# StevenChang5/Canny_Edge

Hardware: AMD Instinct MI355X
Metric: Mpixels/s device-resident Canny (4K gray, frames in HBM, whole pipeline); % HBM roofline on Sobel+NMS in `roofline`; the end-to-end (host->host, PCIe-inclusive) rate is `end_to_end` (higher is better)
Workload: dtype f32+s16; 1 GPU; 128x 3840x2160 gray frames per GPU per step, sigma=1.4, thresholds 50/150, inputs resident in HBM; frames_per_gpu=128, height=2160, width=3840

## Files before the change

### canny_edge_amd/capi.py

```python
from __future__ import annotations

import ctypes as C
import os
import threading
from typing import Optional, Tuple

import numpy as np

_HERE = os.path.dirname(os.path.abspath(__file__))
LIB_PATH = os.environ.get("CANNY_HIP_LIB") or os.path.join(_HERE, "libcanny_hip.so")

OK = 0
STAGE_GAUSSIAN, STAGE_SOBEL_NMS, STAGE_HYST_CLASSIFY, STAGE_HYST_PROPAGATE, STAGE_HYST_FINALIZE, \
    STAGE_SOBEL, STAGE_NMS, STAGE_XY_GRADIENT, STAGE_TO_GRAY = range(9)
STAGE_NAMES = ("gaussian", "sobel_nms", "hyst_classify", "hyst_propagate", "hyst_finalize", "sobel", "nms",
               "xy_gradient", "to_gray")
STAGE_COMPACT = 9

LAYOUT_GRAY8, LAYOUT_BGR8, LAYOUT_RGB8, LAYOUT_BGRA8, LAYOUT_RGBA8 = range(5)
LAYOUT_CHANNELS = {LAYOUT_GRAY8: 1, LAYOUT_BGR8: 3, LAYOUT_RGB8: 3, LAYOUT_BGRA8: 4, LAYOUT_RGBA8: 4}


def layout_of(shape, order: str = "bgr", batch: bool = False) -> int:
    shape = tuple(int(d) for d in shape)
    if order not in ("bgr", "rgb"):
        raise ValueError(f"order must be 'bgr' or 'rgb', not {order!r}")
    nd = len(shape) - (1 if batch else 0)
    if nd == 2:
        return LAYOUT_GRAY8
    if nd == 3 and shape[-1] in (3, 4):
        if shape[-1] == 3:
            return LAYOUT_BGR8 if order == "bgr" else LAYOUT_RGB8
        return LAYOUT_BGRA8 if order == "bgr" else LAYOUT_RGBA8
    raise ValueError(f"expected {'(N, ' if batch else '('}H, W) or {'(N, ' if batch else '('}H, W, 3|4) frames, "
                     f"got shape {shape}")

AUTO_MEDIAN, AUTO_QUANTILE = 1, 2
PIXEL_LDS_TILE, PIXEL_PACKED_I16, PIXEL_F32, PIXEL_F32_FLOOR = 0, 1, 2, 3
WS_DATA, WS_INDEX, WS_CACHE = 0, 1, 2
_AUTO_RULES = {"median": AUTO_MEDIAN, "quantile": AUTO_QUANTILE, AUTO_MEDIAN: AUTO_MEDIAN, AUTO_QUANTILE: AUTO_QUANTILE}


def _rule(rule) -> int:
    if rule not in _AUTO_RULES:
        raise ValueError(f"rule must be 'median', 'quantile', AUTO_MEDIAN or AUTO_QUANTILE, not {rule!r}")
    return _AUTO_RULES[rule]


EXPORTS = (
    "canny_hip_version", "canny_hip_status_string", "canny_hip_device_count", "canny_hip_ctx_create",
    "canny_hip_ctx_destroy", "canny_hip_ctx_set_stream", "canny_hip_ctx_device", "canny_hip_ctx_set_option", "canny_hip_synchronize",
    "canny_hip_last_error", "canny_hip_last_hysteresis_iterations", "canny_hip_malloc", "canny_hip_free",
    "canny_hip_host_alloc", "canny_hip_host_free", "canny_hip_memcpy_h2d", "canny_hip_memcpy_d2h",
    "canny_hip_gaussian_kernel", "canny_hip_gaussian", "canny_hip_xy_gradient", "canny_hip_sobel", "canny_hip_nms",
    "canny_hip_hysteresis", "canny_hip_find_edge_pixels", "canny_hip_canny", "canny_hip_canny_batch",
    "canny_hip_canny_batch_u8", "canny_hip_dev_canny_u8", "canny_hip_canny_multi_gpu", "canny_hip_shard_range", "canny_hip_dev_gaussian", "canny_hip_dev_xy_gradient",
    "canny_hip_dev_sobel", "canny_hip_dev_nms", "canny_hip_dev_sobel_nms", "canny_hip_dev_hysteresis",
    "canny_hip_dev_canny", "canny_hip_dev_canny_stream", "canny_hip_dev_canny_stream_flush", "canny_hip_profile_enable", "canny_hip_profile_reset", "canny_hip_profile_get",
    "canny_hip_selftest_mag_angle", "canny_hip_selftest_sobel_pixel", "canny_hip_selftest_div", "canny_hip_selftest_div_fma",
    "canny_hip_selftest_div_fma_table", "canny_hip_canny_multi_gpu_u8", "canny_hip_multi_gpu_set_option",
    "canny_hip_multi_gpu_release", "canny_hip_device_local_cpus", "canny_hip_selftest_cpulist_count",
    "canny_hip_dev_gaussian_u8", "canny_hip_dev_sobel_nms_u8in", "canny_hip_host_register", "canny_hip_host_unregister",
    "canny_hip_canny_batch_bits", "canny_hip_canny_multi_gpu_bits", "canny_hip_dev_canny_bits",
    "canny_hip_probe_copy", "canny_hip_ctx_get_option", "canny_hip_selftest_expand_bits",
    "canny_hip_selftest_march_order", "canny_hip_to_gray", "canny_hip_dev_to_gray", "canny_hip_dev_gaussian_u8_color",
    "canny_hip_dev_canny_color", "canny_hip_canny_color", "canny_hip_canny_batch_color", "canny_hip_canny_batch_color_u8",
    "canny_hip_canny_batch_color_bits", "canny_hip_auto_thresholds_from_histogram", "canny_hip_dev_canny_thresholds",
    "canny_hip_dev_canny_auto", "canny_hip_canny_batch_thresholds", "canny_hip_canny_batch_auto",
    "canny_hip_dev_canny_points", "canny_hip_dev_points_from_bits", "canny_hip_canny_points",
    "canny_hip_points_from_bits",
    "canny_hip_hough_geometry", "canny_hip_hough_tables", "canny_hip_hough_line_of", "canny_hip_dev_hough_points",
    "canny_hip_dev_hough_bits", "canny_hip_dev_canny_hough", "canny_hip_canny_hough", "canny_hip_hough_profile_get",
    "canny_hip_dev_canny_components", "canny_hip_dev_components_bits", "canny_hip_canny_components",
    "canny_hip_components_from_bits", "canny_hip_components_profile_get",
    "canny_hip_dev_canny_contours", "canny_hip_dev_contours_bits", "canny_hip_canny_contours",
    "canny_hip_contours_from_bits", "canny_hip_contours_profile_get",
    "canny_hip_dev_canny_edt", "canny_hip_dev_edt_bits", "canny_hip_canny_edt", "canny_hip_edt_from_bits",
    "canny_hip_edt_profile_get",
    "canny_hip_hough_segments_from_bits", "canny_hip_dev_hough_segments_bits", "canny_hip_dev_canny_hough_segments",
    "canny_hip_canny_hough_segments", "canny_hip_hough_segments_profile_get",
    "canny_hip_selftest_histogram", "canny_hip_selftest_select", "canny_hip_selftest_workspace",
    "canny_hip_hough_circles_step_of", "canny_hip_hough_circles_from_bits", "canny_hip_dev_hough_circles_bits",
    "canny_hip_dev_canny_hough_circles", "canny_hip_canny_hough_circles", "canny_hip_dev_hough_circles_steps",
    "canny_hip_hough_circles_profile_get",
    "canny_hip_dev_polygons_chains", "canny_hip_dev_canny_polygons", "canny_hip_dev_polygons_bits",
    "canny_hip_canny_polygons", "canny_hip_polygons_from_chains", "canny_hip_polygons_profile_get",
)

_lib: Optional[C.CDLL] = None


class CannyHipError(RuntimeError):
    def __init__(self, status: int, what: str, detail: str = ""):
        self.status = status
        msg = f"{what}: {status_string(status)}"
        if detail:
            msg += f" ({detail})"
        super().__init__(msg)


def load() -> C.CDLL:
    global _lib
    if _lib is not None:
        return _lib
    if not os.path.exists(LIB_PATH):
        raise ImportError(f"{LIB_PATH} is missing: run `python -c 'import __graft_entry__ as g; g.build()'` "
                          "(or `make -C canny_edge_amd/csrc`); there is no CPU fallback")
    os.environ.setdefault("GPU_MAX_HW_QUEUES", "8")
    L = C.CDLL(LIB_PATH)
    i, f, p, sz = C.c_int, C.c_float, C.c_void_p, C.c_size_t
    pp, ip = C.POINTER(C.c_void_p), C.POINTER(C.c_int)
    ull = C.c_ulonglong
    sig = {
        "canny_hip_version": ([], i),
        "canny_hip_status_string": ([i], C.c_char_p),
        "canny_hip_device_count": ([ip], i),
        "canny_hip_ctx_create": ([pp, i], i),
        "canny_hip_ctx_destroy": ([p], None),
        "canny_hip_ctx_set_stream": ([p, p], i),
        "canny_hip_ctx_device": ([p], i),
        "canny_hip_ctx_set_option": ([p, C.c_char_p, i], i),
        "canny_hip_synchronize": ([p], i),
        "canny_hip_last_error": ([p], C.c_char_p),
        "canny_hip_last_hysteresis_iterations": ([p], i),
        "canny_hip_malloc": ([p, pp, sz], i),
        "canny_hip_free": ([p, p], i),
        "canny_hip_host_alloc": ([p, pp, sz], i),
        "canny_hip_host_free": ([p, p], i),
        "canny_hip_host_register": ([p, p, sz], i),
        "canny_hip_host_unregister": ([p, p], i),
        "canny_hip_memcpy_h2d": ([p, p, p, sz], i),
        "canny_hip_memcpy_d2h": ([p, p, p, sz], i),
        "canny_hip_gaussian_kernel": ([f, p, i, ip], i),
        "canny_hip_gaussian": ([p, p, f, i, i, p], i),
        "canny_hip_xy_gradient": ([p, p, i, i, p, p], i),
        "canny_hip_sobel": ([p, p, i, i, p, p], i),
        "canny_hip_nms": ([p, p, p, i, i, p], i),
        "canny_hip_hysteresis": ([p, p, i, i, i, i], i),
        "canny_hip_find_edge_pixels": ([p, p, p, i, i, i, i, i], i),
        "canny_hip_canny": ([p, p, f, i, i, i, i, p], i),
        "canny_hip_canny_batch": ([p, p, i, f, i, i, i, i, p], i),
        "canny_hip_canny_batch_u8": ([p, p, i, f, i, i, i, i, p], i),
        "canny_hip_dev_canny_u8": ([p, p, f, i, i, i, i, i, p], i),
        "canny_hip_dev_canny_bits": ([p, p, f, i, i, i, i, i, p], i),
        "canny_hip_canny_batch_bits": ([p, p, i, f, i, i, i, i, p], i),
        "canny_hip_canny_multi_gpu_bits": ([p, i, f, i, i, i, i, p, i], i),
        "canny_hip_canny_multi_gpu": ([p, i, f, i, i, i, i, p, i], i),
        "canny_hip_canny_multi_gpu_u8": ([p, i, f, i, i, i, i, p, i], i),
        "canny_hip_multi_gpu_set_option": ([C.c_char_p, i], i),
        "canny_hip_multi_gpu_release": ([], i),
        "canny_hip_device_local_cpus": ([i, C.c_char_p, i], i),
        "canny_hip_selftest_cpulist_count": ([C.c_char_p], i),
        "canny_hip_shard_range": ([i, i, i, ip, ip], i),
        "canny_hip_dev_gaussian": ([p, p, f, i, i, i, p], i),
        "canny_hip_dev_xy_gradient": ([p, p, i, i, i, p, p], i),
        "canny_hip_dev_sobel": ([p, p, i, i, i, p, p], i),
        "canny_hip_dev_nms": ([p, p, p, i, i, i, p], i),
        "canny_hip_dev_sobel_nms": ([p, p, i, i, i, p], i),
        "canny_hip_dev_hysteresis": ([p, p, i, i, i, i, i], i),
        "canny_hip_dev_gaussian_u8": ([p, p, f, i, i, i, p], i),
        "canny_hip_dev_sobel_nms_u8in": ([p, p, i, i, i, p], i),
        "canny_hip_dev_canny": ([p, p, f, i, i, i, i, i, p], i),
        "canny_hip_dev_canny_stream": ([p, p, f, i, i, i, i, i, p], i),
        "canny_hip_dev_canny_stream_flush": ([p], i),
        "canny_hip_profile_enable": ([p, i], i),
        "canny_hip_profile_reset": ([p], i),
        "canny_hip_profile_get": ([p, i, C.POINTER(C.c_double), C.POINTER(C.c_long)], i),
        "canny_hip_probe_copy": ([p, p, p, C.c_size_t, i, C.POINTER(C.c_double)], i),
        "canny_hip_ctx_get_option": ([p, C.c_char_p, ip], i),
        "canny_hip_selftest_expand_bits": ([p, i, i, i, p, i], i),
        "canny_hip_selftest_march_order": ([i, i, p], i),
        "canny_hip_selftest_mag_angle": ([p, i, p, p], i),
        "canny_hip_selftest_sobel_pixel": ([p, i, i, p, p], i),
        "canny_hip_selftest_div": ([p, f, C.POINTER(C.c_ulonglong), C.POINTER(C.c_float)], i),
        "canny_hip_selftest_div_fma": ([p, f, f, C.POINTER(C.c_ulonglong), C.POINTER(C.c_float)], i),
        "canny_hip_selftest_div_fma_table": ([i, C.POINTER(C.c_float), C.POINTER(C.c_float)], i),
        "canny_hip_to_gray": ([p, p, i, i, i, p], i),
        "canny_hip_dev_to_gray": ([p, p, i, i, i, i, p], i),
        "canny_hip_dev_gaussian_u8_color": ([p, p, i, f, i, i, i, p], i),
        "canny_hip_dev_canny_color": ([p, p, i, f, i, i, i, i, i, p], i),
        "canny_hip_canny_color": ([p, p, i, f, i, i, i, i, p], i),
        "canny_hip_canny_batch_color": ([p, p, i, i, f, i, i, i, i, p], i),
        "canny_hip_canny_batch_color_u8": ([p, p, i, i, f, i, i, i, i, p], i),
        "canny_hip_canny_batch_color_bits": ([p, p, i, i, f, i, i, i, i, p], i),
        "canny_hip_auto_thresholds_from_histogram": ([p, i, f, f, ip, ip], i),
        "canny_hip_dev_canny_thresholds": ([p, p, f, p, i, i, i, p], i),
        "canny_hip_dev_canny_auto": ([p, p, f, i, f, f, i, i, i, p, p], i),
        "canny_hip_canny_batch_thresholds": ([p, p, i, f, p, i, i, p], i),
        "canny_hip_canny_batch_auto": ([p, p, i, f, i, f, f, i, i, p, p], i),
        "canny_hip_dev_canny_points": ([p, p, f, i, i, i, i, i, p, p, C.c_ulonglong, p], i),
        "canny_hip_dev_points_from_bits": ([p, p, i, i, i, p, C.c_ulonglong, p], i),
        "canny_hip_canny_points": ([p, p, i, f, i, i, i, i, p, C.c_ulonglong, p], i),
        "canny_hip_points_from_bits": ([p, i, i, p, C.c_ulonglong, C.POINTER(C.c_ulonglong)], i),
        "canny_hip_hough_geometry": ([i, i, f, f, f, f, ip, ip], i),
        "canny_hip_hough_tables": ([f, f, f, i, p, p], i),
        "canny_hip_hough_line_of": ([C.c_uint, i, f, f, f, C.POINTER(f), C.POINTER(f)], i),
        "canny_hip_dev_hough_points": ([p, p, p, i, i, i, f, f, i, i, f, f, p, p, p, p, p], i),
        "canny_hip_dev_hough_bits": ([p, p, i, i, i, f, f, i, i, f, f, p, p, p, p, p], i),
        "canny_hip_dev_canny_hough": ([p, p, f, i, i, i, i, i, p, f, f, i, i, f, f, p, p, p, p, p], i),
        "canny_hip_canny_hough": ([p, p, i, f, i, i, i, i, f, f, i, i, f, f, p, p, p, p], i),
        "canny_hip_hough_profile_get": ([p, i, C.POINTER(C.c_double), C.POINTER(C.c_long)], i),
        "canny_hip_dev_canny_components": ([p, p, f, i, i, i, i, i, p, i, p, p, p, C.c_ulonglong, p], i),
        "canny_hip_dev_components_bits": ([p, p, i, i, i, i, p, p, p, C.c_ulonglong, p], i),
        "canny_hip_canny_components": ([p, p, i, f, i, i, i, i, i, p, p, p, C.c_ulonglong, p], i),
        "canny_hip_components_from_bits": ([p, i, i, i, p, p, C.c_ulonglong, C.POINTER(C.c_ulonglong)], i),
        "canny_hip_components_profile_get": ([p, i, C.POINTER(C.c_double), C.POINTER(C.c_long)], i),
        "canny_hip_dev_canny_contours": ([p, p, f, i, i, i, i, i, p, i, p, C.c_ulonglong, p, p, p, C.c_ulonglong, p], i),
        "canny_hip_dev_contours_bits": ([p, p, i, i, i, i, p, C.c_ulonglong, p, p, p, C.c_ulonglong, p], i),
        "canny_hip_canny_contours": ([p, p, i, f, i, i, i, i, i, p, C.c_ulonglong, p, p, p, C.c_ulonglong, p], i),
        "canny_hip_contours_from_bits": ([p, i, i, i, p, C.c_ulonglong, C.POINTER(C.c_ulonglong), p, p, C.c_ulonglong,
                                          C.POINTER(C.c_ulonglong)], i),
        "canny_hip_contours_profile_get": ([p, i, C.POINTER(C.c_double), C.POINTER(C.c_long)], i),
        "canny_hip_dev_canny_edt": ([p, p, f, i, i, i, i, i, p, p, p, p], i),
        "canny_hip_dev_edt_bits": ([p, p, i, i, i, p, p, p], i),
        "canny_hip_canny_edt": ([p, p, i, f, i, i, i, i, p, p, p], i),
        "canny_hip_edt_from_bits": ([p, i, i, p, p, p], i),
        "canny_hip_edt_profile_get": ([p, i, C.POINTER(C.c_double), C.POINTER(C.c_long)], i),
        "canny_hip_hough_segments_from_bits": ([p, i, i, f, f, f, f, p, i, i, i, i, p, i, ip], i),
        "canny_hip_dev_hough_segments_bits": ([p, p, i, i, i, f, f, f, f, p, p, i, i, i, i, p, i, p], i),
        "canny_hip_dev_canny_hough_segments": ([p, p, f, i, i, i, i, i, p, f, f, i, i, f, f, p, p, p, p, p, i, i, i, p, i,
                                                p], i),
        "canny_hip_canny_hough_segments": ([p, p, i, f, i, i, i, i, f, f, i, i, f, f, i, i, i, p, p, p, p, p, i, p], i),
        "canny_hip_hough_segments_profile_get": ([p, i, C.POINTER(C.c_double), C.POINTER(C.c_long)], i),
        "canny_hip_selftest_histogram": ([p, p, i, i, i, i, i, p], i),
        "canny_hip_selftest_select": ([p, p, i, i, f, f, p], i),
        "canny_hip_selftest_workspace": ([p, i, C.POINTER(C.c_char_p), pp, C.POINTER(sz), ip], i),
        "canny_hip_hough_circles_step_of": ([i, i, ip, ip], i),
        "canny_hip_hough_circles_from_bits": ([p, p, p, i, i, i, i, i, i, i, i, i, p, ip, ip, p], i),
        "canny_hip_dev_hough_circles_bits": ([p, p, p, p, i, i, i, i, i, i, i, i, i, i, p, p, p, p], i),
        "canny_hip_dev_canny_hough_circles": ([p, p, f, i, i, i, i, i, p, i, i, i, i, i, i, i, p, p, p, p], i),
        "canny_hip_canny_hough_circles": ([p, p, i, f, i, i, i, i, i, i, i, i, i, i, i, p, p, p], i),
        "canny_hip_dev_hough_circles_steps": ([p, p, p, C.c_size_t, p, p], i),
        "canny_hip_hough_circles_profile_get": ([p, i, C.POINTER(C.c_double), C.POINTER(C.c_long)], i),
        "canny_hip_dev_polygons_chains": ([p, p, i, ull, p, p, ull, i, i, C.c_uint, C.c_uint, p, p, ull, p], i),
        "canny_hip_dev_canny_polygons": ([p, p, f, i, i, i, i, i, p, i, p, ull, p, p, p, ull, p, C.c_uint, C.c_uint, p, p,
                                          ull, p], i),
        "canny_hip_dev_polygons_bits": ([p, p, i, i, i, i, p, ull, p, p, p, ull, p, C.c_uint, C.c_uint, p, p, ull, p], i),
        "canny_hip_canny_polygons": ([p, p, i, f, i, i, i, i, i, p, ull, p, p, p, ull, p, C.c_uint, C.c_uint, p, p, ull,
                                      p], i),
        "canny_hip_polygons_from_chains": ([p, p, ull, ull, i, i, C.c_uint, C.c_uint, p, p, ull, p], i),
        "canny_hip_polygons_profile_get": ([p, i, C.POINTER(C.c_double), C.POINTER(C.c_long)], i),
    }
    for name, (args, res) in sig.items():
        fn = getattr(L, name)
        fn.argtypes = args
        fn.restype = res
    _lib = L
    return L


def status_string(status: int) -> str:
    return load().canny_hip_status_string(status).decode()


def device_count() -> int:
    n = C.c_int(0)
# ... 871 lines not shown
                c[name] = r[:, j]
            out.append(c)
        return out, peaks

    def dev_hough_circles_bits(self, d_bits: int, d_gx: int, d_gy: int, n: int, h: int, w: int, min_radius: int,
                               max_radius: int, cell_shift: int, threshold: int, support_threshold: int, min_dist: int,
                               centres_max: int, d_circles: int, d_counts: int, d_centre_counts: int = 0, d_accum: int = 0):
        v = C.c_void_p
        self._check(self._L.canny_hip_dev_hough_circles_bits(self._h, v(d_bits or None), v(d_gx or None), v(d_gy or None), n,
                                                             h, w, min_radius, max_radius, cell_shift, threshold,
                                                             support_threshold, min_dist, centres_max,
                                                             v(d_circles or None), v(d_counts or None),
                                                             v(d_centre_counts or None), v(d_accum or None)),
                    "dev_hough_circles_bits")

    def dev_canny_hough_circles(self, d_img: int, sigma: float, min_val: int, max_val: int, h: int, w: int, n: int,
                                min_radius: int, max_radius: int, cell_shift: int, threshold: int, support_threshold: int,
                                min_dist: int, centres_max: int, d_circles: int, d_counts: int, d_centre_counts: int = 0,
                                d_accum: int = 0, d_edges: int = 0):
        v = C.c_void_p
        self._check(self._L.canny_hip_dev_canny_hough_circles(self._h, v(d_img or None), sigma, min_val, max_val, h, w, n,
                                                              v(d_edges or None), min_radius, max_radius, cell_shift,
                                                              threshold, support_threshold, min_dist, centres_max,
                                                              v(d_circles or None), v(d_counts or None),
                                                              v(d_centre_counts or None), v(d_accum or None)),
                    "dev_canny_hough_circles")

    def dev_hough_circles_steps(self, d_gx: int, d_gy: int, n: int, d_sx: int, d_sy: int):
        v = C.c_void_p
        self._check(self._L.canny_hip_dev_hough_circles_steps(self._h, v(d_gx or None), v(d_gy or None), n,
                                                              v(d_sx or None), v(d_sy or None)), "dev_hough_circles_steps")

    def hough_circles_profile_get(self, part: int) -> Tuple[float, int]:
        ms, n = C.c_double(0), C.c_long(0)
        self._check(self._L.canny_hip_hough_circles_profile_get(self._h, part, C.byref(ms), C.byref(n)),
                    "hough_circles_profile_get")
        return ms.value, n.value

    def to_gray(self, frame, order: str = "bgr") -> np.ndarray:
        a, lay = _frame(frame, order)
        out = np.empty(a.shape[:2], np.uint8)
        self._check(self._L.canny_hip_to_gray(self._h, _hp(a), lay, a.shape[0], a.shape[1], _hp(out)), "to_gray")
        return out

    def canny_color(self, frame, sigma: float, min_val: int, max_val: int, order: str = "bgr") -> np.ndarray:
        a, lay = _frame(frame, order)
        out = np.empty(a.shape[:2], np.int16)
        self._check(self._L.canny_hip_canny_color(self._h, _hp(a), lay, sigma, min_val, max_val, a.shape[0],
                                                  a.shape[1], _hp(out)), "canny_color")
        return out

    def canny_batch_color(self, imgs, sigma: float, min_val: int, max_val: int, order: str = "bgr",
                          out: Optional[np.ndarray] = None, fmt: str = "s16") -> np.ndarray:
        a, lay = _frame(imgs, order, batch=True)
        if fmt not in ("s16", "u8", "bits"):
            raise ValueError(f"fmt must be 's16', 'u8' or 'bits', not {fmt!r}")
        n, h, w = a.shape[:3]
        dtype = np.int16 if fmt == "s16" else np.uint8
        shape = bits_shape((n, h, w)) if fmt == "bits" else (n, h, w)
        if out is None:
            out = np.empty(shape, dtype)
        elif out.shape != shape or out.dtype != dtype or not out.flags["C_CONTIGUOUS"]:
            raise ValueError(f"out must be a C-contiguous {np.dtype(dtype).name} array of shape {shape}")
        fn = {"s16": self._L.canny_hip_canny_batch_color, "u8": self._L.canny_hip_canny_batch_color_u8,
              "bits": self._L.canny_hip_canny_batch_color_bits}[fmt]
        self._check(fn(self._h, _hp(a), lay, n, sigma, min_val, max_val, h, w, _hp(out)), "canny_batch_color")
        return out

    def selftest_mag_angle(self, lim: int = 1020):
        side = 2 * lim + 1
        mags = np.empty((side, side), np.int16)
        bins = np.empty((side, side), np.uint8)
        self._check(self._L.canny_hip_selftest_mag_angle(self._h, lim, _hp(mags), _hp(bins)), "selftest")
        return mags, bins

    def selftest_sobel_pixel(self, form: int, lim: int = 1020):
        side = 2 * lim + 1
        mags = np.empty((side, side), np.int16)
        bins = np.empty((side, side), np.uint8)
        self._check(self._L.canny_hip_selftest_sobel_pixel(self._h, form, lim, _hp(mags), _hp(bins)),
                    "selftest_sobel_pixel")
        return mags, bins

    def selftest_div(self, divisor: float) -> Tuple[int, float]:
        bad, worst = C.c_ulonglong(0), C.c_float(0.0)
        self._check(self._L.canny_hip_selftest_div(self._h, divisor, C.byref(bad), C.byref(worst)), "selftest_div")
        return bad.value, worst.value

    def selftest_div_fma(self, divisor: float, c: float) -> Tuple[int, float]:
        bad, worst = C.c_ulonglong(0), C.c_float(0.0)
        self._check(self._L.canny_hip_selftest_div_fma(self._h, divisor, c, C.byref(bad), C.byref(worst)),
                    "selftest_div_fma")
        return bad.value, worst.value

    def selftest_histogram(self, d_plane: int, plane_is_u8: bool, kind, h: int, w: int, n: int, d_hist: int):
        self._check(self._L.canny_hip_selftest_histogram(self._h, C.c_void_p(d_plane), int(plane_is_u8), _rule(kind), h,
                                                         w, n, C.c_void_p(d_hist)), "selftest_histogram")

    def selftest_select(self, d_hist: int, n: int, rule, low: float, high: float, d_pairs: int):
        self._check(self._L.canny_hip_selftest_select(self._h, C.c_void_p(d_hist), n, _rule(rule), low, high,
                                                      C.c_void_p(d_pairs)), "selftest_select")

    def selftest_workspaces(self):
        out, index = [], 0
        while True:
            name, ptr, size, kind = C.c_char_p(), C.c_void_p(), C.c_size_t(), C.c_int()
            st = self._L.canny_hip_selftest_workspace(self._h, index, C.byref(name), C.byref(ptr), C.byref(size),
                                                      C.byref(kind))
            if st == 1 and index > 0:
                return out
            self._check(st, "selftest_workspace")
            out.append((name.value.decode(), ptr.value or 0, size.value, kind.value))
            index += 1

    def dev_gaussian(self, d_img: int, sigma: float, h: int, w: int, n: int, d_out: int):
        self._check(self._L.canny_hip_dev_gaussian(self._h, C.c_void_p(d_img), sigma, h, w, n, C.c_void_p(d_out)),
                    "dev_gaussian")

    def dev_xy_gradient(self, d_img: int, h: int, w: int, n: int, d_gx: int, d_gy: int):
        self._check(self._L.canny_hip_dev_xy_gradient(self._h, C.c_void_p(d_img), h, w, n, C.c_void_p(d_gx),
                                                      C.c_void_p(d_gy)), "dev_xy_gradient")

    def dev_sobel(self, d_img: int, h: int, w: int, n: int, d_mag: int, d_ang: int):
        self._check(self._L.canny_hip_dev_sobel(self._h, C.c_void_p(d_img), h, w, n, C.c_void_p(d_mag),
                                                C.c_void_p(d_ang)), "dev_sobel")

    def dev_nms(self, d_mag: int, d_ang: int, h: int, w: int, n: int, d_out: int):
        self._check(self._L.canny_hip_dev_nms(self._h, C.c_void_p(d_mag), C.c_void_p(d_ang), h, w, n,
                                              C.c_void_p(d_out)), "dev_nms")

    def dev_sobel_nms(self, d_smoothed: int, h: int, w: int, n: int, d_out: int):
        self._check(self._L.canny_hip_dev_sobel_nms(self._h, C.c_void_p(d_smoothed), h, w, n, C.c_void_p(d_out)),
                    "dev_sobel_nms")

    def probe_copy(self, d_src: int, d_dst: int, nbytes: int, launches: int = 10) -> float:
        ms = C.c_double(0)
        self._check(self._L.canny_hip_probe_copy(self._h, C.c_void_p(d_src), C.c_void_p(d_dst), nbytes, launches,
                                                 C.byref(ms)), "probe_copy")
        return ms.value

    def dev_gaussian_u8(self, d_img: int, sigma: float, h: int, w: int, n: int, d_out: int):
        self._check(self._L.canny_hip_dev_gaussian_u8(self._h, C.c_void_p(d_img), sigma, h, w, n, C.c_void_p(d_out)),
                    "dev_gaussian_u8")

    def dev_sobel_nms_u8in(self, d_smoothed: int, h: int, w: int, n: int, d_out: int):
        self._check(self._L.canny_hip_dev_sobel_nms_u8in(self._h, C.c_void_p(d_smoothed), h, w, n, C.c_void_p(d_out)),
                    "dev_sobel_nms_u8in")

    def dev_hysteresis(self, d_cand: int, h: int, w: int, n: int, min_val: int, max_val: int):
        self._check(self._L.canny_hip_dev_hysteresis(self._h, C.c_void_p(d_cand), h, w, n, min_val, max_val),
                    "dev_hysteresis")

    def dev_canny(self, d_img: int, sigma: float, min_val: int, max_val: int, h: int, w: int, n: int, d_edges: int):
        self._check(self._L.canny_hip_dev_canny(self._h, C.c_void_p(d_img), sigma, min_val, max_val, h, w, n,
                                                C.c_void_p(d_edges)), "dev_canny")

    def dev_canny_stream(self, d_img: int, sigma: float, min_val: int, max_val: int, h: int, w: int, n: int,
                         d_edges: int):
        self._check(self._L.canny_hip_dev_canny_stream(self._h, C.c_void_p(d_img), sigma, min_val, max_val, h, w, n,
                                                       C.c_void_p(d_edges)), "dev_canny_stream")

    def dev_canny_stream_flush(self):
        self._check(self._L.canny_hip_dev_canny_stream_flush(self._h), "dev_canny_stream_flush")

    def dev_canny_bits(self, d_img: int, sigma: float, min_val: int, max_val: int, h: int, w: int, n: int, d_bits: int):
        self._check(self._L.canny_hip_dev_canny_bits(self._h, C.c_void_p(d_img), sigma, min_val, max_val, h, w, n,
# ... 122 lines not shown
```

### canny_edge_amd/csrc/canny_capi.hip

```cpp
#include "canny_hip.h"
#include "canny_kernels.h"

#include <hip/hip_runtime.h>
#include <sched.h>

#include <algorithm>
#include <atomic>
#include <chrono>
#include <condition_variable>
#include <deque>
#include <memory>
#include <cmath>
#include <cstdint>
#include <cstdio>
#include <cctype>
#include <climits>
#include <cstdlib>
#include <cstring>
#include <mutex>
#include <new>
#include <string>
#include <thread>
#include <vector>
#if defined(__SSE2__)
// ... 209 lines not shown
            }
            run(j);
        }
    }
    void run(const Job &j)
    {
        if (j.copy_bytes) std::memcpy(j.dst, j.bits, j.copy_bytes);
        for (int r = 0; r < (j.copy_bytes ? 0 : j.rows); r++) {
            const uint8_t *src = j.bits + (size_t)r * j.row_bytes;
            const int full = j.width / 8, tail = j.width % 8;
            if (j.to_u8) {
                uint8_t *d = (uint8_t *)j.dst + (size_t)r * j.width;
                for (int b = 0; b < full; b++) std::memcpy(d + 8 * b, lut8_[src[b]], 8);
                if (tail) std::memcpy(d + 8 * full, lut8_[src[full]], tail);
            } else {
                short *d = (short *)j.dst + (size_t)r * j.width;
#if defined(__SSE2__)
                if ((((uintptr_t)d) & 15) == 0) {
                    for (int b = 0; b < full; b++)
                        _mm_stream_si128((__m128i *)(d + 8 * b), _mm_load_si128((const __m128i *)lut16_[src[b]]));
                } else
#endif
                {
                    for (int b = 0; b < full; b++) std::memcpy(d + 8 * b, lut16_[src[b]], 16);
                }
                if (tail) std::memcpy(d + 8 * full, lut16_[src[full]], 2 * tail);
            }
        }
#if defined(__SSE2__)
        _mm_sfence();
#endif
        if (j.left->fetch_sub(1, std::memory_order_acq_rel) == 1) {
            std::lock_guard<std::mutex> lk(mu_);
            cv_done_.notify_all();
        }
    }
    alignas(16) short lut16_[256][8];
    alignas(8) uint8_t lut8_[256][8];
    std::vector<std::thread> threads_;
    std::mutex mu_;
    std::condition_variable cv_job_, cv_done_;
    std::deque<Job> q_;
    bool stop_ = false;
};

struct EventPair {
    hipEvent_t a, b;
};

struct PropLane {
    hipStream_t stream = nullptr;
    uint64_t *S = nullptr;
    const uint64_t *C = nullptr;
    unsigned *sched = nullptr, *flags = nullptr;
    unsigned *host = nullptr, *host_dev = nullptr;
    hipEvent_t event = nullptr;
    HystGeom g{};
    short *edges = nullptr;
    int edge_value = 0;
    int iter = 0;
    unsigned seq = 0;
    bool converged = false;
};

}

struct canny_hip_ctx {
    int device = 0;
    hipStream_t own_stream = nullptr;
    hipStream_t stream = nullptr;
    std::string last_error;
    int last_hyst_iters = 0;
    int gaussian_path = 0;
    int sobel_nms_path = 0;
    int tune_sobel_seg = 0;
    int fuse_classify = 1;
    int smoothed_u8 = 1;
    int last_canny_u8 = 0;
    int gray_rule = 0;
    int fuse_gray = 1;
    int last_fused_gray = 0;
    int hyst_tail = 1;
    int hyst_tail_after = 2;
    bool hyst_iters_async = false;
    int batch_workers = 0;
    int batch_chunk_mb = 0;
    int batch_chunk_frames = 0;
    int batch_pipe_mode = 0;
    int batch_compact = 0;
    int batch_expand_threads = 0;
    std::unique_ptr<ExpandPool> expand_pool;
    struct BatchPipe;
    std::vector<BatchPipe *> batch_pool;

    DevBuf tmp_f32;
    DevBuf smoothed;
    DevBuf edges16;
    DevBuf gray;
    DevBuf hist;
    DevBuf thr;
    DevBuf points;
    DevBuf hough_accum, hough_ws, hough_tab;
    std::vector<float> hough_tab_host;
    float hough_tab_key[3] = {0, 0, 0};
    int hough_tab_n = 0;
    int hough_path = 0;
    int hough_lds_kb = 0;
    DevBuf cc_parent, cc_ws;
    DevBuf ct_ws;
    DevBuf pg_ws, pg_points;
    DevBuf edt_cols, edt_stack;
    DevBuf seg_ws, seg_lines, seg_work;
    DevBuf circ_accum, circ_ws;
    DevBuf plane_s, plane_c, stamps, flags;
    DevBuf io[4];
    std::string ws_name;
    unsigned *host_flags = nullptr;
    unsigned *host_flags_dev = nullptr;
    unsigned publish_seq = 0;
    hipEvent_t flag_event = nullptr;
    int overlap_hysteresis = 0;
    int stream_overlap = 0;
    hipStream_t aux_stream = nullptr;
    hipEvent_t fork_event = nullptr, aux_event = nullptr;
    PropLane pend;
    bool has_pend = false;

    bool prof = false;
    unsigned prof_mask = ~0u;
    unsigned prof_every = 1;
    static constexpr int kProfHough = CANNY_HIP_STAGE_END, kProfComponents = CANNY_HIP_STAGE_END + 3;
    static constexpr int kProfEdt = kProfComponents + CANNY_HIP_CC_PARTS;
    static constexpr int kProfSegments = kProfEdt + CANNY_HIP_EDT_PARTS;
    static constexpr int kProfContours = kProfSegments + CANNY_HIP_SEGMENT_PARTS;
    static constexpr int kProfCircles = kProfContours + CANNY_HIP_CONTOUR_PARTS;
    static constexpr int kProfPolygons = kProfCircles + CANNY_HIP_CIRCLE_PARTS;
    static constexpr int kProfSlots = kProfPolygons + CANNY_HIP_POLYGON_PARTS;
    static constexpr int kProfLastBit = 30;
    static_assert(kProfPolygons == kProfLastBit, "profile_stage_mask has one bit per slot up to the polygon parts");
    unsigned prof_seen[kProfSlots] = {0};
    std::vector<EventPair> pending[kProfSlots];
    std::vector<EventPair> pool;
    double total_ms[kProfSlots] = {0};
    long launches[kProfSlots] = {0};
};

struct canny_hip_ctx::BatchPipe {
    static constexpr int kSlots = 3;
    canny_hip_ctx *sub = nullptr;
    bool owns_sub = false;
    hipStream_t s_h2d = nullptr, s_d2h = nullptr;
    struct Slot {
        DevBuf d_in, d_out, d_out8;
        PinBuf pin_in, pin_out;
        DevBuf d_thr;
        PinBuf pin_thr;
        hipEvent_t ev_h2d = nullptr, ev_comp = nullptr, ev_d2h = nullptr;
        bool d2h_issued = false;
        void *retire_dst = nullptr;
        size_t retire_bytes = 0;
        int retire_frames = 0;
        std::atomic<int> expand_left{0};
    } slot[kSlots];
};

namespace {

int fail(canny_hip_ctx *ctx, hipError_t e, const char *where)
{
    if (ctx) {
        ctx->last_error = std::string(where) + ": " + hipGetErrorString(e);
    }
    (void)hipGetLastError();
    return (e == hipErrorNoDevice || e == hipErrorInvalidDevice) ? CANNY_HIP_ERR_NO_DEVICE : CANNY_HIP_ERR_RUNTIME;
}

#define HIP_TRY(ctx, expr)                                  \
    do {                                                    \
        hipError_t e_ = (expr);                             \
        if (e_ != hipSuccess) return fail((ctx), e_, #expr); \
    } while (0)

int bind(canny_hip_ctx *ctx)
{
    if (!ctx) return CANNY_HIP_ERR_INVALID;
    HIP_TRY(ctx, hipSetDevice(ctx->device));
    return CANNY_HIP_OK;
}

struct StageTimer {
    canny_hip_ctx *ctx;
    int stage;
    EventPair ev{};
    bool on = false;
    hipStream_t stream;
    bool attach;
    StageTimer(canny_hip_ctx *c, int s, hipStream_t on_stream = nullptr, bool attached = false)
// ... 73 lines not shown
    default: return CANNY_HIP_ERR_INVALID;
    }
    const bool bgr = layout == CANNY_HIP_BGR8 || layout == CANNY_HIP_BGRA8;
    ci.rule.k0 = bgr ? w[0] : w[2];
    ci.rule.k1 = w[1];
    ci.rule.k2 = bgr ? w[2] : w[0];
    ci.rule.shift = w[3];
    ci.rule.rnd = 1u << (w[3] - 1);
    return CANNY_HIP_OK;
}

bool gaussian_u8_possible(const canny_hip_ctx *ctx, const GaussTaps &taps, int h, int w)
{
    float min_tap = 1.0f;
    for (int k = 0; k <= 2 * taps.center; k++)
        if (taps.tap[k] > 0.0f && taps.tap[k] < min_tap) min_tap = taps.tap[k];
    return ctx->gaussian_path != 1 && gaussian_march_supported(taps.center, h, w) && min_tap >= 0x1p-48f &&
           gaussian_march_u8_supported(taps) && sobel_nms_u8_input_supported();
}

int dev_gaussian(canny_hip_ctx *ctx, const unsigned char *d_img, float sigma, int h, int w, int n, void *d_out_any,
                 int u8_mode = 0)
{
    short *d_out = (short *)d_out_any;
    GaussTaps taps;
    int rc = make_taps(sigma, taps);
    if (rc) return rc;
    StageTimer tm(ctx, CANNY_HIP_STAGE_GAUSSIAN);
    if (u8_mode) {
        if (!gaussian_u8_possible(ctx, taps, h, w)) return CANNY_HIP_ERR_UNSUPPORTED;
        HIP_TRY(ctx, launch_gaussian_march_u8(d_img, (uint8_t *)d_out_any, h, w, n, taps, ctx->stream));
        return CANNY_HIP_OK;
    }
    float min_tap = 1.0f;
    for (int k = 0; k <= 2 * taps.center; k++)
        if (taps.tap[k] > 0.0f && taps.tap[k] < min_tap) min_tap = taps.tap[k];
    const bool can_march = gaussian_march_supported(taps.center, h, w) && min_tap >= 0x1p-48f;
    if (ctx->gaussian_path == 2 && !can_march) return CANNY_HIP_ERR_UNSUPPORTED;
    if (can_march && ctx->gaussian_path != 1) {
        HIP_TRY(ctx, launch_gaussian_march(d_img, d_out, h, w, n, taps, ctx->stream));
    } else {
        HIP_TRY(ctx, ctx->tmp_f32.ensure(npx(h, w, n) * sizeof(float)));
        HIP_TRY(ctx, launch_gaussian_generic(d_img, (float *)ctx->tmp_f32.p, d_out, h, w, n, taps, ctx->stream));
    }
    return CANNY_HIP_OK;
}

int dev_to_gray(canny_hip_ctx *ctx, const unsigned char *d_src, const ColorIn &ci, int h, int w, int n,
                unsigned char *d_gray)
{
    const size_t px = npx(h, w, n);
    if (ci.ch == 1) {
        if (d_src != d_gray) HIP_TRY(ctx, hipMemcpyAsync(d_gray, d_src, px, hipMemcpyDeviceToDevice, ctx->stream));
        return CANNY_HIP_OK;
    }
    StageTimer tm(ctx, CANNY_HIP_STAGE_TO_GRAY);
    HIP_TRY(ctx, launch_to_gray(d_src, ci.ch, ci.rule, d_gray, px, ctx->stream));
    return CANNY_HIP_OK;
}

bool gaussian_color_fusable(const canny_hip_ctx *ctx, const GaussTaps &taps, const ColorIn &ci, int h, int w)
{
    return ci.ch > 1 && gaussian_u8_possible(ctx, taps, h, w) && gaussian_march_color_supported(taps, w, ci.ch);
}

int dev_gaussian_u8_color(canny_hip_ctx *ctx, const unsigned char *d_src, const ColorIn &ci, float sigma, int h, int w,
                          int n, unsigned char *d_out)
{
    GaussTaps taps;
    int rc = make_taps(sigma, taps);
    if (rc) return rc;
    if (!gaussian_color_fusable(ctx, taps, ci, h, w)) return CANNY_HIP_ERR_UNSUPPORTED;
    StageTimer tm(ctx, CANNY_HIP_STAGE_GAUSSIAN);
    HIP_TRY(ctx, launch_gaussian_march_u8_color(d_src, ci.ch, ci.rule, d_out, h, w, n, taps, ctx->stream));
    return CANNY_HIP_OK;
}

int ensure_hyst(canny_hip_ctx *ctx, const HystGeom &g)
{
    HIP_TRY(ctx, ctx->plane_s.ensure(g.words() * sizeof(uint64_t)));
    HIP_TRY(ctx, ctx->plane_c.ensure(g.words() * sizeof(uint64_t)));
    HIP_TRY(ctx, ctx->stamps.ensure((hyst_sched_words(g) + 4) * sizeof(unsigned)));
    HIP_TRY(ctx, ctx->flags.ensure(4 * sizeof(unsigned)));
    if (!ctx->host_flags) {
        HIP_TRY(ctx, hipHostMalloc((void **)&ctx->host_flags, 8 * sizeof(unsigned), hipHostMallocMapped));
        std::memset(ctx->host_flags, 0, 8 * sizeof(unsigned));
        HIP_TRY(ctx, hipHostGetDevicePointer((void **)&ctx->host_flags_dev, ctx->host_flags, 0));
    }
    if (!ctx->flag_event) HIP_TRY(ctx, hipEventCreateWithFlags(&ctx->flag_event, hipEventDisableTiming));
    return CANNY_HIP_OK;
}

int ensure_aux_stream(canny_hip_ctx *ctx)
{
    if (!ctx->aux_stream) {
        int least = 0, greatest = 0;
        HIP_TRY(ctx, hipDeviceGetStreamPriorityRange(&least, &greatest));
        HIP_TRY(ctx, hipStreamCreateWithPriority(&ctx->aux_stream, hipStreamNonBlocking, greatest));
    }
    if (!ctx->fork_event) HIP_TRY(ctx, hipEventCreateWithFlags(&ctx->fork_event, hipEventDisableTiming));
    if (!ctx->aux_event) HIP_TRY(ctx, hipEventCreateWithFlags(&ctx->aux_event, hipEventDisableTiming));
    return CANNY_HIP_OK;
}

int prepare_hyst(canny_hip_ctx *ctx, const HystGeom &g, bool zero_pad)
{
    HIP_TRY(ctx, launch_hyst_prepare((uint64_t *)ctx->plane_s.p, (uint64_t *)ctx->plane_c.p, g, zero_pad,
                                     (unsigned *)ctx->stamps.p, (unsigned *)ctx->flags.p, ctx->stream));
    return CANNY_HIP_OK;
}

constexpr int kTailMaxTiles = 4096;
constexpr int kSweepChunk = 8;
constexpr int kMaxSweeps = 1 << 22;

int lane_launch_chunk(canny_hip_ctx *ctx, PropLane &L)
{
    {
        StageTimer tm(ctx, CANNY_HIP_STAGE_HYST_PROPAGATE, L.stream);
        for (int k = 0; k < kSweepChunk; k++)
            HIP_TRY(ctx, launch_hyst_propagate(L.S, L.C, L.sched, L.flags, L.iter + k, L.g, L.stream, L.edges,
                                               L.edge_value));
    }
    L.iter += kSweepChunk;
    L.seq = ++ctx->publish_seq;
    HIP_TRY(ctx, launch_hyst_publish(L.flags, L.host_dev, L.seq, L.stream));
    HIP_TRY(ctx, hipEventRecord(L.event, L.stream));
    return CANNY_HIP_OK;
}

int lane_wait(canny_hip_ctx *ctx, PropLane &L)
{
    volatile unsigned *hf = L.host;
    const auto t0 = std::chrono::steady_clock::now();
    unsigned spins = 0;
    while (__atomic_load_n(&hf[2], __ATOMIC_ACQUIRE) != L.seq) {
        __builtin_ia32_pause();
        if ((++spins & 0xfffu) == 0 && std::chrono::steady_clock::now() - t0 > std::chrono::seconds(2)) {
            HIP_TRY(ctx, hipEventSynchronize(L.event));
            if (__atomic_load_n(&hf[2], __ATOMIC_ACQUIRE) != L.seq) return CANNY_HIP_ERR_RUNTIME;
        }
    }
    if (hf[1]) return CANNY_HIP_ERR_DOMAIN;
    L.converged = hf[0] != (unsigned)L.iter;
    if (!L.converged && L.iter >= kMaxSweeps) return CANNY_HIP_ERR_NO_CONVERGE;
    if (L.converged) ctx->last_hyst_iters = std::max(ctx->last_hyst_iters, (int)hf[0] + 1);
    return CANNY_HIP_OK;
}

PropLane main_lane(canny_hip_ctx *ctx, const HystGeom &g, short *edges, int edge_value)
{
    PropLane L;
    L.stream = ctx->stream;
    L.S = (uint64_t *)ctx->plane_s.p;
    L.C = (const uint64_t *)ctx->plane_c.p;
    L.sched = (unsigned *)ctx->stamps.p;
    L.flags = (unsigned *)ctx->flags.p;
    L.host = ctx->host_flags;
    L.host_dev = ctx->host_flags_dev;
    L.event = ctx->flag_event;
    L.g = g;
    L.edges = edges;
    L.edge_value = edge_value;
    return L;
}

// ... 42 lines not shown

int dev_hysteresis(canny_hip_ctx *ctx, short *d_cand, int h, int w, int n, int lo, int hi, const int *pairs = nullptr)
{
    if (pairs) lo = hi = 255;
    if (hysteresis_order_dependent(lo, hi)) return CANNY_HIP_ERR_DOMAIN;
    HystGeom g = make_hyst_geom(h, w, n);
    int rc = finish_pending(ctx);
    if (rc || (rc = ensure_hyst(ctx, g))) return rc;
    if ((rc = prepare_hyst(ctx, g, false))) return rc;
    {
        StageTimer tm(ctx, CANNY_HIP_STAGE_HYST_CLASSIFY);
        HIP_TRY(ctx, launch_hyst_classify(d_cand, (uint64_t *)ctx->plane_s.p, (uint64_t *)ctx->plane_c.p, g, lo, hi,
                                          (unsigned *)ctx->flags.p + 1, ctx->stream, pairs));
    }
    return propagate_and_finalize(ctx, g, d_cand, hi);
}

int dev_sobel_nms(canny_hip_ctx *ctx, const short *d_smoothed, int h, int w, int n, short *d_out)
{
    if (ctx->sobel_nms_path != 1 && sobel_nms_march_supported(h, w)) {
        StageTimer tm(ctx, CANNY_HIP_STAGE_SOBEL_NMS, nullptr, true);
        HIP_TRY(ctx, launch_sobel_nms_march(d_smoothed, d_out, h, w, n, ctx->stream, ctx->tune_sobel_seg,
                                            tm.launch_events()));
    } else {
        StageTimer tm(ctx, CANNY_HIP_STAGE_SOBEL_NMS);
        HIP_TRY(ctx, launch_sobel_nms(d_smoothed, d_out, h, w, n, true, ctx->stream));
    }
    return CANNY_HIP_OK;
}

int dev_canny(canny_hip_ctx *ctx, const unsigned char *d_img, float sigma, int lo, int hi, int h, int w, int n,
              short *d_edges, const ColorIn *color = nullptr, const ThrSpec *thr = nullptr)
{
    if (h < 2 || w < 2) return CANNY_HIP_ERR_UNSUPPORTED;
    if (thr) lo = hi = 255;
    if (hysteresis_order_dependent(lo, hi)) return CANNY_HIP_ERR_DOMAIN;
    int rc = finish_pending(ctx);
    if (rc) return rc;
    HIP_TRY(ctx, ctx->smoothed.ensure(npx(h, w, n) * sizeof(short)));
    short *sm = (short *)ctx->smoothed.p;
    const bool fused = ctx->fuse_classify && ctx->sobel_nms_path != 1 && sobel_nms_classify_supported(h, w, lo);
    int sm_u8 = 0;
    if (fused && ctx->smoothed_u8) {
        GaussTaps taps;
        if ((rc = make_taps(sigma, taps))) return rc;
        if (gaussian_u8_possible(ctx, taps, h, w)) sm_u8 = ctx->smoothed_u8;
    }
    ctx->last_canny_u8 = sm_u8;
    if (color && color->ch > 1) {
        GaussTaps taps;
        if ((rc = make_taps(sigma, taps))) return rc;
        const bool fuse = sm_u8 && color->fuse && gaussian_color_fusable(ctx, taps, *color, h, w);
        ctx->last_fused_gray = fuse;
        if (fuse) {
            StageTimer tm(ctx, CANNY_HIP_STAGE_GAUSSIAN);
            HIP_TRY(ctx, launch_gaussian_march_u8_color(d_img, color->ch, color->rule, (uint8_t *)sm, h, w, n, taps,
                                                        ctx->stream));
        } else {
            HIP_TRY(ctx, ctx->gray.ensure(npx(h, w, n)));
            if ((rc = dev_to_gray(ctx, d_img, *color, h, w, n, (unsigned char *)ctx->gray.p))) return rc;
            if ((rc = dev_gaussian(ctx, (const unsigned char *)ctx->gray.p, sigma, h, w, n, sm, sm_u8))) return rc;
        }
    } else {
        if (color) ctx->last_fused_gray = 0;
        if ((rc = dev_gaussian(ctx, d_img, sigma, h, w, n, sm, sm_u8))) return rc;
    }
    const int *pairs = thr ? thr->pairs : nullptr;
    if (thr && thr->rule) {
        int *out = thr->out;
        if (!out) {
            HIP_TRY(ctx, ctx->thr.ensure((size_t)n * 2 * sizeof(int)));
            out = (int *)ctx->thr.p;
        }
        HIP_TRY(ctx, ctx->hist.ensure((size_t)n * kHistBins * sizeof(uint32_t)));
        uint32_t *hist = (uint32_t *)ctx->hist.p;
        StageTimer tm(ctx, CANNY_HIP_STAGE_HYST_CLASSIFY);
        HIP_TRY(ctx, hipMemsetAsync(hist, 0, (size_t)n * kHistBins * sizeof(uint32_t), ctx->stream));
        HIP_TRY(ctx, thr->rule == kAutoMedian ? launch_hist_intensity(sm, sm_u8 != 0, hist, h, w, n, ctx->stream)
                                              : launch_hist_gradient(sm, sm_u8 != 0, hist, h, w, n, ctx->stream));
        HIP_TRY(ctx, launch_thr_select(hist, n, thr->rule, thr->low, thr->high, out, ctx->stream));
        pairs = out;
    }
    auto fused_sobel = [&](const short *smp, short *edges, uint64_t *S, uint64_t *C, const HystGeom &gg, int ev,
                           const LaunchEvents &le, const int *pp) -> hipError_t {
        return sm_u8 ? launch_sobel_nms_classify_march_u8in((const uint8_t *)smp, edges, S, C, gg, lo, hi, ev,
                                                            ctx->stream, ctx->tune_sobel_seg, le, pp)
                     : launch_sobel_nms_classify_march(smp, edges, S, C, gg, lo, hi, ev, ctx->stream,
                                                       ctx->tune_sobel_seg, le, pp);
    };
    if (fused) {
        HystGeom g = make_hyst_geom(h, w, n);
        if ((rc = ensure_hyst(ctx, g))) return rc;
        uint64_t *S = (uint64_t *)ctx->plane_s.p, *C = (uint64_t *)ctx->plane_c.p;
        const int edge_value = 255 >= hi ? 255 : 0;
        if (ctx->overlap_hysteresis && n >= 16) {
            if ((rc = ensure_aux_stream(ctx))) return rc;
            const int nA = n / 2, nB = n - nA;
            const HystGeom gA = make_hyst_geom(h, w, nA), gB = make_hyst_geom(h, w, nB);
            const size_t px_a = npx(h, w, nA);
            HIP_TRY(ctx, launch_hyst_prepare(S, C, g, true, (unsigned *)ctx->stamps.p,
                                             (unsigned *)ctx->flags.p, ctx->stream, 2));
            PropLane A = main_lane(ctx, gA, d_edges, edge_value), B = main_lane(ctx, gB, d_edges + px_a, edge_value);
            A.stream = ctx->aux_stream;
            A.event = ctx->aux_event;
            B.S += gA.words();
            B.C += gA.words();
            B.sched += hyst_sched_words(gA);
            B.flags += 2;
            B.host += 4;
            B.host_dev += 4;
            {
                StageTimer tm(ctx, CANNY_HIP_STAGE_SOBEL_NMS, nullptr, true);
                HIP_TRY(ctx, fused_sobel(sm, d_edges, A.S, (uint64_t *)A.C, gA, edge_value, tm.launch_events(), pairs));
            }
            HIP_TRY(ctx, hipEventRecord(ctx->fork_event, ctx->stream));
            HIP_TRY(ctx, hipStreamWaitEvent(ctx->aux_stream, ctx->fork_event, 0));
            ctx->last_hyst_iters = 0;
            if ((rc = lane_launch_chunk(ctx, A))) return rc;
            {
                StageTimer tm(ctx, CANNY_HIP_STAGE_SOBEL_NMS, nullptr, true);
                const short *smB = sm_u8 ? (const short *)((const uint8_t *)sm + px_a) : sm + px_a;
                HIP_TRY(ctx, fused_sobel(smB, d_edges + px_a, B.S, (uint64_t *)B.C, gB, edge_value, tm.launch_events(),
                                         pairs ? pairs + 2 * (size_t)nA : nullptr));
            }
            if ((rc = lane_launch_chunk(ctx, B))) return rc;
            for (PropLane *L : {&A, &B}) {
                if ((rc = lane_wait(ctx, *L))) return rc;
                while (!L->converged) {
                    if ((rc = lane_launch_chunk(ctx, *L)) || (rc = lane_wait(ctx, *L))) return rc;
                }
            }
            HIP_TRY(ctx, hipStreamWaitEvent(ctx->stream, A.event, 0));
            return CANNY_HIP_OK;
        }
        if ((rc = prepare_hyst(ctx, g, true))) return rc;
        {
            StageTimer tm(ctx, CANNY_HIP_STAGE_SOBEL_NMS, nullptr, true);
            HIP_TRY(ctx, fused_sobel(sm, d_edges, S, C, g, edge_value, tm.launch_events(), pairs));
        }
        if (ctx->hyst_tail && g.tiles_x * g.tiles_y <= kTailMaxTiles) {
            StageTimer tm(ctx, CANNY_HIP_STAGE_HYST_PROPAGATE);
            unsigned *sched = (unsigned *)ctx->stamps.p, *flags = (unsigned *)ctx->flags.p;
            const int wide = ctx->hyst_tail_after;
            for (int k = 0; k < wide; k++)
                HIP_TRY(ctx, launch_hyst_propagate(S, C, sched, flags, k, g, ctx->stream, d_edges, edge_value,
                                                   true));
            HIP_TRY(ctx, launch_hyst_tail(S, C, sched, flags, wide, g, ctx->stream, d_edges, edge_value));
            ctx->hyst_iters_async = true;
            return CANNY_HIP_OK;
        }
        ctx->hyst_iters_async = false;
        return run_propagation(ctx, g, false, []() -> int { return CANNY_HIP_OK; }, d_edges, edge_value);
    }
    if ((rc = dev_sobel_nms(ctx, sm, h, w, n, d_edges))) return rc;
    return dev_hysteresis(ctx, d_edges, h, w, n, lo, hi, pairs);
}

int finish_pending(canny_hip_ctx *ctx)
{
    if (!ctx->has_pend) return CANNY_HIP_OK;
    ctx->has_pend = false;
    PropLane &L = ctx->pend;
    int rc;
    if ((rc = lane_wait(ctx, L))) return rc;
    while (!L.converged)
        if ((rc = lane_launch_chunk(ctx, L)) || (rc = lane_wait(ctx, L))) return rc;
    if (L.stream != ctx->stream) HIP_TRY(ctx, hipStreamWaitEvent(ctx->stream, L.event, 0));
    return CANNY_HIP_OK;
}

int dev_canny_stream(canny_hip_ctx *ctx, const unsigned char *d_img, float sigma, int lo, int hi, int h, int w, int n,
                     short *d_edges)
{
    if (h < 2 || w < 2) return CANNY_HIP_ERR_UNSUPPORTED;
    if (hysteresis_order_dependent(lo, hi)) return CANNY_HIP_ERR_DOMAIN;
    if (!(ctx->fuse_classify && ctx->sobel_nms_path != 1 && sobel_nms_classify_supported(h, w, lo)) ||
        (ctx->hyst_tail && make_hyst_geom(h, w, n).tiles_x * make_hyst_geom(h, w, n).tiles_y <= kTailMaxTiles)) {
        int rc = finish_pending(ctx);
        return rc ? rc : dev_canny(ctx, d_img, sigma, lo, hi, h, w, n, d_edges);
    }
    HIP_TRY(ctx, ctx->smoothed.ensure(npx(h, w, n) * sizeof(short)));
    short *sm = (short *)ctx->smoothed.p;
    int sm_u8 = 0;
    if (ctx->smoothed_u8) {
        GaussTaps taps;
        int rt = make_taps(sigma, taps);
        if (rt) return rt;
        if (gaussian_u8_possible(ctx, taps, h, w)) sm_u8 = ctx->smoothed_u8;
    }
    ctx->last_canny_u8 = sm_u8;
    int rc = dev_gaussian(ctx, d_img, sigma, h, w, n, sm, sm_u8);
    if (rc) return rc;
    if ((rc = finish_pending(ctx))) return rc;
    HystGeom g = make_hyst_geom(h, w, n);
    if ((rc = ensure_hyst(ctx, g)) || (ctx->stream_overlap && (rc = ensure_aux_stream(ctx)))) return rc;
    const int edge_value = 255 >= hi ? 255 : 0;
    if ((rc = prepare_hyst(ctx, g, true))) return rc;
    {
        StageTimer tm(ctx, CANNY_HIP_STAGE_SOBEL_NMS, nullptr, true);
        if (sm_u8)
            HIP_TRY(ctx, launch_sobel_nms_classify_march_u8in((const uint8_t *)sm, d_edges, (uint64_t *)ctx->plane_s.p,
                                                              (uint64_t *)ctx->plane_c.p, g, lo, hi, edge_value,
                                                              ctx->stream, ctx->tune_sobel_seg, tm.launch_events()));
        else
            HIP_TRY(ctx, launch_sobel_nms_classify_march(sm, d_edges, (uint64_t *)ctx->plane_s.p,
                                                         (uint64_t *)ctx->plane_c.p, g, lo, hi, edge_value, ctx->stream,
                                                         ctx->tune_sobel_seg, tm.launch_events()));
    }
    ctx->pend = main_lane(ctx, g, d_edges, edge_value);
    if (ctx->stream_overlap) {
        HIP_TRY(ctx, hipEventRecord(ctx->fork_event, ctx->stream));
        HIP_TRY(ctx, hipStreamWaitEvent(ctx->aux_stream, ctx->fork_event, 0));
        ctx->pend.stream = ctx->aux_stream;
        ctx->pend.event = ctx->aux_event;
    }
    ctx->last_hyst_iters = 0;
    ctx->hyst_iters_async = false;
    if ((rc = lane_launch_chunk(ctx, ctx->pend))) return rc;
    ctx->has_pend = true;
    return CANNY_HIP_OK;
}

int h2d(canny_hip_ctx *ctx, DevBuf &b, const void *src, size_t bytes)
{
    HIP_TRY(ctx, b.ensure(bytes));
    HIP_TRY(ctx, hipMemcpyAsync(b.p, src, bytes, hipMemcpyHostToDevice, ctx->stream));
    return CANNY_HIP_OK;
}
int d2h_sync(canny_hip_ctx *ctx, void *dst, const void *src, size_t bytes)
// ... 596 lines not shown
        sl.d_out8.release();
        sl.pin_in.release();
        sl.pin_out.release();
        sl.d_thr.release();
        sl.pin_thr.release();
        for (hipEvent_t e : {sl.ev_h2d, sl.ev_comp, sl.ev_d2h})
            if (e) (void)hipEventDestroy(e);
    }
    if (w->s_h2d) (void)hipStreamDestroy(w->s_h2d);
    if (w->s_d2h) (void)hipStreamDestroy(w->s_d2h);
    if (w->owns_sub) canny_hip_ctx_destroy(w->sub);
    delete w;
}

int create_batch_pipe(canny_hip_ctx *ctx, bool first, canny_hip_ctx::BatchPipe **out)
{
    auto *w = new (std::nothrow) canny_hip_ctx::BatchPipe();
    if (!w) return CANNY_HIP_ERR_RUNTIME;
    int st = CANNY_HIP_OK;
    if (first) {
        w->sub = ctx;
    } else {
        st = canny_hip_ctx_create(&w->sub, ctx->device);
        w->owns_sub = st == CANNY_HIP_OK;
    }
    hipError_t e = hipSuccess;
    if (!st) {
        for (auto &sl : w->slot)
            for (hipEvent_t *ev : {&sl.ev_h2d, &sl.ev_comp, &sl.ev_d2h})
                if (e == hipSuccess) e = hipEventCreateWithFlags(ev, hipEventDisableTiming);
        if (e != hipSuccess) st = fail(ctx, e, "batch pipeline events");
    }
    if (st) {
        destroy_batch_pipe(w);
        return st;
    }
    *out = w;
    return CANNY_HIP_OK;
}

int ensure_copy_streams(canny_hip_ctx *ctx, canny_hip_ctx::BatchPipe &w)
{
    if (!w.s_h2d) HIP_TRY(ctx, hipStreamCreateWithFlags(&w.s_h2d, hipStreamNonBlocking));
    if (!w.s_d2h) HIP_TRY(ctx, hipStreamCreateWithFlags(&w.s_d2h, hipStreamNonBlocking));
    return CANNY_HIP_OK;
}

struct WsEntry {
    std::string name;
    const DevBuf *buf;
    int kind;
};

void collect_workspaces(const canny_hip_ctx *c, const std::string &prefix, std::vector<WsEntry> &v)
{
    const int D = CANNY_HIP_WS_DATA, I = CANNY_HIP_WS_INDEX;
    auto add = [&](const char *name, const DevBuf &b, int kind) { v.push_back({prefix + name, &b, kind}); };
    add("tmp_f32", c->tmp_f32, D);
    add("smoothed", c->smoothed, D);
    add("edges16", c->edges16, D);
    add("gray", c->gray, D);
    add("hist", c->hist, D);
    add("thr", c->thr, D);
    add("points", c->points, I);
    add("hough_accum", c->hough_accum, D);
    add("hough_ws", c->hough_ws, I);
    add("hough_tab", c->hough_tab, CANNY_HIP_WS_CACHE);
    add("cc_parent", c->cc_parent, I);
    add("cc_ws", c->cc_ws, I);
    add("ct_ws", c->ct_ws, I);
    add("pg_ws", c->pg_ws, I);
    add("pg_points", c->pg_points, I);
    add("edt_cols", c->edt_cols, I);
    add("edt_stack", c->edt_stack, I);
    add("seg_ws", c->seg_ws, I);
    add("seg_lines", c->seg_lines, I);
    add("seg_work", c->seg_work, D);
    add("circ_accum", c->circ_accum, D);
    add("circ_ws", c->circ_ws, I);
    add("plane_s", c->plane_s, D);
    add("plane_c", c->plane_c, D);
    add("stamps", c->stamps, I);
    add("flags", c->flags, D);
    for (int k = 0; k < 4; k++) add(("io" + std::to_string(k)).c_str(), c->io[k], I);
    for (size_t p = 0; p < c->batch_pool.size(); p++) {
        const canny_hip_ctx::BatchPipe *w = c->batch_pool[p];
        if (!w) continue;
        const std::string pipe = prefix + "pipe" + std::to_string(p) + ".";
        for (int s = 0; s < canny_hip_ctx::BatchPipe::kSlots; s++) {
            const std::string slot = pipe + "slot" + std::to_string(s) + ".";
            v.push_back({slot + "d_in", &w->slot[s].d_in, D});
            v.push_back({slot + "d_out", &w->slot[s].d_out, D});
            v.push_back({slot + "d_out8", &w->slot[s].d_out8, D});
            v.push_back({slot + "d_thr", &w->slot[s].d_thr, D});
        }
        if (w->owns_sub && w->sub) collect_workspaces(w->sub, pipe, v);
    }
}

}

extern "C" {

int canny_hip_version(void) { return CANNY_HIP_VERSION; }

const char *canny_hip_status_string(int status)
{
    switch (status) {
    case CANNY_HIP_OK: return "ok";
    case CANNY_HIP_ERR_INVALID: return "invalid argument";
    case CANNY_HIP_ERR_UNSUPPORTED: return "unsupported size or window";
    case CANNY_HIP_ERR_NO_DEVICE: return "no usable HIP device (there is no CPU fallback)";
    case CANNY_HIP_ERR_RUNTIME: return "HIP runtime error";
    case CANNY_HIP_ERR_DOMAIN: return "input outside the documented numeric domain";
    case CANNY_HIP_ERR_NO_CONVERGE: return "hysteresis propagation did not converge";
    default: return "unknown status";
    }
}

int canny_hip_device_count(int *count)
{
    if (!count) return CANNY_HIP_ERR_INVALID;
    int n = 0;
    hipError_t e = hipGetDeviceCount(&n);
    if (e != hipSuccess) {
        (void)hipGetLastError();
        *count = 0;
        return CANNY_HIP_ERR_NO_DEVICE;
    }
    *count = n;
    return CANNY_HIP_OK;
}

int canny_hip_ctx_create(canny_hip_ctx **out, int device)
{
    if (!out) return CANNY_HIP_ERR_INVALID;
    *out = nullptr;
    int n = 0;
    if (hipGetDeviceCount(&n) != hipSuccess || n < 1) {
        (void)hipGetLastError();
        return CANNY_HIP_ERR_NO_DEVICE;
    }
    if (device < 0 || device >= n) return CANNY_HIP_ERR_INVALID;
    canny_hip_ctx *ctx = new (std::nothrow) canny_hip_ctx();
    if (!ctx) return CANNY_HIP_ERR_RUNTIME;
    ctx->device = device;
    if (hipSetDevice(device) != hipSuccess ||
        hipStreamCreateWithFlags(&ctx->own_stream, hipStreamNonBlocking) != hipSuccess) {
        (void)hipGetLastError();
        delete ctx;
        return CANNY_HIP_ERR_NO_DEVICE;
    }
    ctx->stream = ctx->own_stream;
    *out = ctx;
    return CANNY_HIP_OK;
}

void canny_hip_ctx_destroy(canny_hip_ctx *ctx)
{
    if (!ctx) return;
    (void)hipSetDevice(ctx->device);
    (void)finish_pending(ctx);
    ctx->expand_pool.reset();
    for (auto *w : ctx->batch_pool) destroy_batch_pipe(w);
    ctx->batch_pool.clear();
    (void)hipSetDevice(ctx->device);
    if (ctx->aux_stream) (void)hipStreamSynchronize(ctx->aux_stream);
    (void)hipStreamSynchronize(ctx->stream);
    ctx->tmp_f32.release();
    ctx->smoothed.release();
    ctx->plane_s.release();
    ctx->plane_c.release();
    ctx->edges16.release();
    ctx->hist.release();
    ctx->thr.release();
    ctx->points.release();
    ctx->hough_accum.release();
    ctx->hough_ws.release();
    ctx->hough_tab.release();
    ctx->seg_ws.release();
    ctx->seg_lines.release();
    ctx->seg_work.release();
    ctx->circ_accum.release();
    ctx->circ_ws.release();
    ctx->cc_parent.release();
    ctx->cc_ws.release();
    ctx->ct_ws.release();
    ctx->pg_ws.release();
    ctx->pg_points.release();
    ctx->edt_cols.release();
    ctx->edt_stack.release();
    ctx->stamps.release();
    ctx->flags.release();
    for (auto &b : ctx->io) b.release();
    if (ctx->host_flags) (void)hipHostFree(ctx->host_flags);
    if (ctx->flag_event) (void)hipEventDestroy(ctx->flag_event);
    if (ctx->fork_event) (void)hipEventDestroy(ctx->fork_event);
    if (ctx->aux_event) (void)hipEventDestroy(ctx->aux_event);
    if (ctx->aux_stream) (void)hipStreamDestroy(ctx->aux_stream);
    for (auto &v : ctx->pending)
        for (auto &e : v) {
            (void)hipEventDestroy(e.a);
            (void)hipEventDestroy(e.b);
        }
    for (auto &e : ctx->pool) {
        (void)hipEventDestroy(e.a);
        (void)hipEventDestroy(e.b);
    }
    if (ctx->own_stream) (void)hipStreamDestroy(ctx->own_stream);
    delete ctx;
}

int canny_hip_ctx_set_stream(canny_hip_ctx *ctx, void *hip_stream)
{
    int rc = bind(ctx);
    if (rc || (rc = finish_pending(ctx))) return rc;
    ctx->stream = hip_stream ? (hipStream_t)hip_stream : ctx->own_stream;
    return CANNY_HIP_OK;
}

int canny_hip_ctx_device(const canny_hip_ctx *ctx) { return ctx ? ctx->device : -1; }

int canny_hip_ctx_get_option(const canny_hip_ctx *ctx, const char *name, int *value)
{
    if (!ctx || !name || !value) return CANNY_HIP_ERR_INVALID;
    if (!std::strcmp(name, "smoothed_u8")) *value = ctx->smoothed_u8;
    else if (!std::strcmp(name, "last_canny_smoothed_u8")) *value = ctx->last_canny_u8;
    else if (!std::strcmp(name, "gray_rule")) *value = ctx->gray_rule;
    else if (!std::strcmp(name, "fuse_gray")) *value = ctx->fuse_gray;
    else if (!std::strcmp(name, "last_canny_fused_gray")) *value = ctx->last_fused_gray;
    else if (!std::strcmp(name, "fuse_classify")) *value = ctx->fuse_classify;
    else if (!std::strcmp(name, "hysteresis_tail")) *value = ctx->hyst_tail;
    else if (!std::strcmp(name, "gaussian_path")) *value = ctx->gaussian_path;
    else if (!std::strcmp(name, "sobel_nms_path")) *value = ctx->sobel_nms_path;
    else if (!std::strcmp(name, "tune_batch_compact")) *value = ctx->batch_compact;
    else if (!std::strcmp(name, "hough_path")) *value = ctx->hough_path;
    else if (!std::strcmp(name, "tune_hough_lds_kb")) *value = ctx->hough_lds_kb;
    else if (!std::strcmp(name, "batch_expand_threads")) *value = ctx->expand_pool ? ctx->expand_pool->size() : 0;
    else return CANNY_HIP_ERR_INVALID;
    return CANNY_HIP_OK;
}

int canny_hip_ctx_set_option(canny_hip_ctx *ctx, const char *name, int value)
{
    if (!ctx || !name || value < 0) return CANNY_HIP_ERR_INVALID;
    if (!std::strcmp(name, "gaussian_path") && value <= 2) ctx->gaussian_path = value;
    else if (!std::strcmp(name, "sobel_nms_path") && value <= 2) ctx->sobel_nms_path = value;
    else if (!std::strcmp(name, "tune_sobel_seg") && value <= 4096) ctx->tune_sobel_seg = value;
    else if (!std::strcmp(name, "fuse_classify") && value <= 1) ctx->fuse_classify = value;
    else if (!std::strcmp(name, "smoothed_u8") && value <= 1) ctx->smoothed_u8 = value;
    else if (!std::strcmp(name, "gray_rule") && value <= 1) ctx->gray_rule = value;
    else if (!std::strcmp(name, "fuse_gray") && value <= 1) ctx->fuse_gray = value;
    else if (!std::strcmp(name, "hysteresis_tail") && value <= 1) ctx->hyst_tail = value;
    else if (!std::strcmp(name, "tune_hyst_tail_after") && value >= 1 && value <= 4) ctx->hyst_tail_after = value;
    else if (!std::strcmp(name, "overlap_hysteresis") && value <= 1) ctx->overlap_hysteresis = value;
    else if (!std::strcmp(name, "tune_batch_workers") && value <= 16) ctx->batch_workers = value;
    else if (!std::strcmp(name, "tune_batch_chunk_mb") && value <= 1024) ctx->batch_chunk_mb = value;
    else if (!std::strcmp(name, "tune_batch_chunk_frames") && value <= 65535) ctx->batch_chunk_frames = value;
    else if (!std::strcmp(name, "tune_batch_pipe_mode") && value <= 2) ctx->batch_pipe_mode = value;
    else if (!std::strcmp(name, "tune_batch_compact") && value <= 1) ctx->batch_compact = value;
    else if (!std::strcmp(name, "hough_path") && value <= 2) ctx->hough_path = value;
    else if (!std::strcmp(name, "tune_hough_lds_kb") && value <= kHoughLdsMax / 1024) ctx->hough_lds_kb = value;
    else if (!std::strcmp(name, "tune_batch_expand_threads") && value <= 64) {
        if (value != ctx->batch_expand_threads) ctx->expand_pool.reset();
        ctx->batch_expand_threads = value;
    }
    else if (!std::strcmp(name, "stream_overlap") && value <= 1) {
        int rc = bind(ctx);
        if (rc || (rc = finish_pending(ctx))) return rc;
        ctx->stream_overlap = value;
    } else if (!std::strcmp(name, "profile_sample_interval") && value >= 1) {
        ctx->prof_every = (unsigned)value;
        for (auto &n : ctx->prof_seen) n = 0;
    } else if (!std::strcmp(name, "profile_stage_mask")) ctx->prof_mask = value ? (unsigned)value : ~0u;
    else if (!std::strcmp(name, "tune_sobel_px") && value <= 1) sobel_nms_set_px_variant(value);
    else if (!std::strcmp(name, "tune_sobel_variant") && value <= 2) sobel_nms_set_arith_variant(value);
    else if (!std::strcmp(name, "tune_plane_stores") && value <= 1) sobel_nms_set_plane_store_variant(value);
    else if (!std::strcmp(name, "gaussian_fma_div") && value <= 1) gaussian_set_fma_div(value != 0);
    else if (!std::strcmp(name, "tune_finalize_mode") && value <= 1) hyst_set_finalize_mode(value);
    else if (!std::strcmp(name, "tune_gaussian_variant") && value <= 4) gaussian_set_march_variant(value);
    else if (!std::strcmp(name, "tune_gaussian_seg") && value <= 8192) gaussian_set_seg_target(value);
    else return CANNY_HIP_ERR_INVALID;
    return CANNY_HIP_OK;
}

int canny_hip_synchronize(canny_hip_ctx *ctx)
{
    int rc = bind(ctx);
    if (rc || (rc = finish_pending(ctx))) return rc;
    HIP_TRY(ctx, hipStreamSynchronize(ctx->stream));
    return CANNY_HIP_OK;
}

const char *canny_hip_last_error(const canny_hip_ctx *ctx) { return ctx ? ctx->last_error.c_str() : ""; }
int canny_hip_last_hysteresis_iterations(canny_hip_ctx *ctx)
{
    if (!ctx) return 0;
    if (ctx->hyst_iters_async && ctx->flags.p) {
        unsigned last = 0;
        if (hipSetDevice(ctx->device) == hipSuccess &&
            hipMemcpyAsync(&last, ctx->flags.p, sizeof last, hipMemcpyDeviceToHost, ctx->stream) == hipSuccess &&
            hipStreamSynchronize(ctx->stream) == hipSuccess)
            ctx->last_hyst_iters = (int)last + 1;
        else
            (void)hipGetLastError();
        ctx->hyst_iters_async = false;
    }
    return ctx->last_hyst_iters;
}

int canny_hip_malloc(canny_hip_ctx *ctx, void **dev_ptr, size_t bytes)
{
    int rc = bind(ctx);
    if (rc) return rc;
    if (!dev_ptr) return CANNY_HIP_ERR_INVALID;
    HIP_TRY(ctx, hipMalloc(dev_ptr, bytes ? bytes : 1));
    return CANNY_HIP_OK;
}
int canny_hip_free(canny_hip_ctx *ctx, void *dev_ptr)
{
    int rc = bind(ctx);
    if (rc) return rc;
    HIP_TRY(ctx, hipFree(dev_ptr));
    return CANNY_HIP_OK;
}
int canny_hip_host_alloc(canny_hip_ctx *ctx, void **host_ptr, size_t bytes)
{
    int rc = bind(ctx);
    if (rc) return rc;
    if (!host_ptr) return CANNY_HIP_ERR_INVALID;
    hipError_t e = numa_host_malloc(ctx->device, host_ptr, bytes);
    HIP_TRY(ctx, e);
    return CANNY_HIP_OK;
}
int canny_hip_host_free(canny_hip_ctx *ctx, void *host_ptr)
{
    int rc = bind(ctx);
// ... 2139 lines not shown
    double total = 0.0;
    hipError_t e = hipSuccess;
    for (int k = 0; k < launches && e == hipSuccess; k++) {
        e = launch_probe_copy(d_src, d_dst, nbytes, ctx->stream, LaunchEvents{a, b});
        if (e == hipSuccess) e = hipEventSynchronize(b);
        float ms = 0.0f;
        if (e == hipSuccess) e = hipEventElapsedTime(&ms, a, b);
        total += ms;
    }
    (void)hipEventDestroy(a);
    (void)hipEventDestroy(b);
    HIP_TRY(ctx, e);
    *avg_ms = total / launches;
    return CANNY_HIP_OK;
}

int canny_hip_selftest_march_order(int n_segs, int n_strips, int *out_pairs)
{
    if (!out_pairs || n_segs < 1 || n_strips < 1 || (long long)n_segs * n_strips > (1 << 24)) return CANNY_HIP_ERR_INVALID;
    for (int k = 0; k < n_segs * n_strips; k++) {
        const MarchCell c = march_cell_of(k, n_segs, n_strips);
        out_pairs[2 * k] = c.seg;
        out_pairs[2 * k + 1] = c.strip;
    }
    return CANNY_HIP_OK;
}

int canny_hip_selftest_expand_bits(const unsigned char *bits, int height, int width, int to_u8, void *out, int n_threads)
{
    if (!bits || !out || height < 1 || width < 1 || n_threads < 1 || n_threads > 64) return CANNY_HIP_ERR_INVALID;
    ExpandPool pool(n_threads);
    constexpr int kBlockRows = 128;
    const int row_bytes = (width + 7) / 8, blocks = (height + kBlockRows - 1) / kBlockRows;
    std::atomic<int> left{blocks};
    for (int b = 0; b < blocks; b++) {
        ExpandPool::Job job;
        const int r0 = b * kBlockRows;
        job.bits = bits + (size_t)r0 * row_bytes;
        job.dst = (unsigned char *)out + (size_t)r0 * width * (to_u8 ? 1 : sizeof(short));
        job.rows = std::min(kBlockRows, height - r0);
        job.width = width;
        job.row_bytes = row_bytes;
        job.to_u8 = to_u8 != 0;
        job.left = &left;
        pool.submit(job);
    }
    pool.wait(left);
    return CANNY_HIP_OK;
}

int canny_hip_selftest_mag_angle(canny_hip_ctx *ctx, int lim, short *magnitudes, unsigned char *bins)
{
    int rc = bind(ctx);
    if (rc) return rc;
    if (!magnitudes || !bins || lim < 0 || lim > 1020) return CANNY_HIP_ERR_INVALID;
    size_t total = (size_t)(2 * lim + 1) * (2 * lim + 1);
    HIP_TRY(ctx, ctx->io[0].ensure(total * 2));
    HIP_TRY(ctx, ctx->io[1].ensure(total));
    HIP_TRY(ctx, launch_selftest_mag_angle(lim, (int16_t *)ctx->io[0].p, (uint8_t *)ctx->io[1].p, ctx->stream));
    HIP_TRY(ctx, hipMemcpyAsync(magnitudes, ctx->io[0].p, total * 2, hipMemcpyDeviceToHost, ctx->stream));
    return d2h_sync(ctx, bins, ctx->io[1].p, total);
}

int canny_hip_selftest_sobel_pixel(canny_hip_ctx *ctx, int form, int lim, short *magnitudes, unsigned char *bins)
{
    int rc = bind(ctx);
    if (rc) return rc;
    if (!magnitudes || !bins || lim < 0 || lim > 1020 || form < CANNY_HIP_PIXEL_LDS_TILE ||
        form > CANNY_HIP_PIXEL_F32_FLOOR)
        return CANNY_HIP_ERR_INVALID;
    size_t total = (size_t)(2 * lim + 1) * (2 * lim + 1);
    HIP_TRY(ctx, ctx->io[0].ensure(total * 2));
    HIP_TRY(ctx, ctx->io[1].ensure(total));
    int16_t *d_mags = (int16_t *)ctx->io[0].p;
    uint8_t *d_bins = (uint8_t *)ctx->io[1].p;
    if (form == CANNY_HIP_PIXEL_LDS_TILE)
        HIP_TRY(ctx, launch_selftest_mag_angle(lim, d_mags, d_bins, ctx->stream));
    else
        HIP_TRY(ctx, launch_selftest_sobel_pixel(form, lim, d_mags, d_bins, ctx->stream));
    HIP_TRY(ctx, hipMemcpyAsync(magnitudes, d_mags, total * 2, hipMemcpyDeviceToHost, ctx->stream));
    return d2h_sync(ctx, bins, d_bins, total);
}

static int selftest_div_common(canny_hip_ctx *ctx, float divisor, int use_fma, float c,
                               unsigned long long *mismatches, float *largest_mismatching_dividend)
{
    int rc = bind(ctx);
    if (rc) return rc;
    if (!mismatches || !largest_mismatching_dividend || !(divisor > 0.0f) || !std::isfinite(divisor))
        return CANNY_HIP_ERR_INVALID;
    HIP_TRY(ctx, ctx->io[0].ensure(2 * sizeof(unsigned long long)));
    HIP_TRY(ctx, hipMemsetAsync(ctx->io[0].p, 0, 2 * sizeof(unsigned long long), ctx->stream));
    const unsigned last = 0x43800000u;
    HIP_TRY(ctx, launch_selftest_div(divisor, use_fma, c, 0u, last, (unsigned long long *)ctx->io[0].p, ctx->stream));
    unsigned long long res[2] = {0, 0};
    if ((rc = d2h_sync(ctx, res, ctx->io[0].p, sizeof(res)))) return rc;
    *mismatches = res[0];
    unsigned bits = (unsigned)res[1];
    std::memcpy(largest_mismatching_dividend, &bits, sizeof(float));
    return CANNY_HIP_OK;
}

int canny_hip_selftest_div(canny_hip_ctx *ctx, float divisor, unsigned long long *mismatches,
                           float *largest_mismatching_dividend)
{
    return selftest_div_common(ctx, divisor, 0, 0.0f, mismatches, largest_mismatching_dividend);
}

int canny_hip_selftest_div_fma_table(int index, float *divisor, float *c)
{
    const unsigned(*table)[2] = nullptr;
    const int n = gaussian_fma_div_table(&table);
    if (index < 0 || index >= n || !divisor || !c) return CANNY_HIP_ERR_INVALID;
    std::memcpy(divisor, &table[index][0], sizeof(float));
    std::memcpy(c, &table[index][1], sizeof(float));
    return CANNY_HIP_OK;
}

int canny_hip_selftest_div_fma(canny_hip_ctx *ctx, float divisor, float c, unsigned long long *mismatches,
                               float *largest_mismatching_dividend)
{
    return selftest_div_common(ctx, divisor, 1, c, mismatches, largest_mismatching_dividend);
}

int canny_hip_selftest_histogram(canny_hip_ctx *ctx, const void *d_plane, int plane_is_u8, int kind, int height, int width,
                                 int n_frames, unsigned int *d_hist)
{
    int rc = bind(ctx);
    if (rc) return rc;
    if (!d_plane || !d_hist || (kind != kAutoMedian && kind != kAutoQuantile)) return CANNY_HIP_ERR_INVALID;
    if ((rc = check_dims(height, width, n_frames))) return rc;
    HIP_TRY(ctx, hipMemsetAsync(d_hist, 0, (size_t)n_frames * kHistBins * sizeof(uint32_t), ctx->stream));
    HIP_TRY(ctx, kind == kAutoMedian
                     ? launch_hist_intensity(d_plane, plane_is_u8 != 0, d_hist, height, width, n_frames, ctx->stream)
                     : launch_hist_gradient(d_plane, plane_is_u8 != 0, d_hist, height, width, n_frames, ctx->stream));
    return CANNY_HIP_OK;
}

int canny_hip_selftest_select(canny_hip_ctx *ctx, const unsigned int *d_hist, int n_frames, int rule, float low, float high,
                              int *d_pairs)
{
    int rc = bind(ctx);
    if (rc) return rc;
    if (!d_hist || !d_pairs || !auto_params_valid(rule, low, high)) return CANNY_HIP_ERR_INVALID;
    if ((rc = check_dims(1, 1, n_frames))) return rc;
    HIP_TRY(ctx, launch_thr_select(d_hist, n_frames, rule, low, high, d_pairs, ctx->stream));
    return CANNY_HIP_OK;
}

int canny_hip_selftest_workspace(canny_hip_ctx *ctx, int index, const char **name, void **d_ptr, size_t *bytes, int *kind)
{
    int rc = bind(ctx);
    if (rc) return rc;
    if (index < 0 || !name || !d_ptr || !bytes || !kind) return CANNY_HIP_ERR_INVALID;
    HIP_TRY(ctx, hipStreamSynchronize(ctx->stream));
    if (ctx->has_pend) return CANNY_HIP_ERR_INVALID;
    std::vector<WsEntry> all;
    collect_workspaces(ctx, "", all);
    if ((size_t)index >= all.size()) return CANNY_HIP_ERR_INVALID;
    ctx->ws_name = all[(size_t)index].name;
    *name = ctx->ws_name.c_str();
    *d_ptr = all[(size_t)index].buf->p;
    *bytes = all[(size_t)index].buf->bytes;
    *kind = all[(size_t)index].kind;
    return CANNY_HIP_OK;
}
// ... 3 lines not shown
```

### canny_edge_amd/csrc/canny_kernels.h

```cpp
#pragma once

#include <hip/hip_runtime.h>
#include <stddef.h>
#include <stdint.h>

namespace canny {

constexpr int kMaxCenter = 64;
constexpr int kMaxWindow = 2 * kMaxCenter + 1;
constexpr int kTile = 64;

struct GaussTaps {
    int center;
    float tap[kMaxWindow];
};

struct MarchCell {
    int seg, strip;
};
__host__ __device__ inline MarchCell march_cell_of(int k, int n_segs, int n_strips)
{
    MarchCell c;
#ifdef CANNY_MARCH_ROW_MAJOR
    n_segs = 0;
// ... 26 lines not shown
    int height, width, n_frames;
    int tiles_x, tiles_y;
    __host__ __device__ size_t words() const { return (size_t)n_frames * tiles_x * tiles_y * kTile; }
    __host__ __device__ int tiles() const { return n_frames * tiles_x * tiles_y; }
};
inline HystGeom make_hyst_geom(int height, int width, int n_frames)
{
    HystGeom g;
    g.height = height;
    g.width = width;
    g.n_frames = n_frames;
    g.tiles_x = (width + kTile - 1) / kTile;
    g.tiles_y = (height + kTile - 1) / kTile;
    return g;
}

hipError_t launch_gaussian_generic(const uint8_t *img, float *tmp, int16_t *out, int height, int width,
                                   int n_frames, const GaussTaps &taps, hipStream_t stream);
bool gaussian_march_supported(int center, int height, int width);
hipError_t launch_gaussian_march(const uint8_t *img, int16_t *out, int height, int width, int n_frames,
                                 const GaussTaps &taps, hipStream_t stream);

bool gaussian_march_u8_supported(const GaussTaps &taps);
hipError_t launch_gaussian_march_u8(const uint8_t *img, uint8_t *out, int height, int width, int n_frames,
                                    const GaussTaps &taps, hipStream_t stream);

int gaussian_fma_div_table(const unsigned (**table)[2]);
void gaussian_set_fma_div(bool on);
void gaussian_set_march_variant(int v);
void gaussian_set_seg_target(int rows);

struct GrayRule {
    uint32_t k0, k1, k2, rnd, shift;
};

template <int CH>
__device__ __forceinline__ uint32_t gray4(const uint32_t *w, const GrayRule &r)
{
    static_assert(CH == 3 || CH == 4, "interleaved 3- or 4-byte pixels");
    uint32_t out = 0u;
#pragma unroll
    for (int p = 0; p < 4; p++) {
        uint32_t c[3];
#pragma unroll
        for (int k = 0; k < 3; k++) {
            const int i = CH * p + k;
            c[k] = (w[i >> 2] >> (8 * (i & 3))) & 0xffu;
        }
        const uint32_t g = __umul24(c[0], r.k0) + __umul24(c[1], r.k1) + __umul24(c[2], r.k2) + r.rnd;
        out |= (g >> r.shift) << (8 * p);
    }
    return out;
}

hipError_t launch_to_gray(const uint8_t *src, int ch, const GrayRule &rule, uint8_t *gray, size_t n_px,
                          hipStream_t stream);

bool gaussian_march_color_supported(const GaussTaps &taps, int width, int ch);
hipError_t launch_gaussian_march_u8_color(const uint8_t *src, int ch, const GrayRule &rule, uint8_t *out, int height,
                                          int width, int n_frames, const GaussTaps &taps, hipStream_t stream);

hipError_t launch_xy_gradient(const int16_t *img, int16_t *gx, int16_t *gy, int height, int width, int n_frames,
                              hipStream_t stream);
hipError_t launch_sobel(const int16_t *img, int16_t *mag, int16_t *angle, int height, int width, int n_frames,
                        hipStream_t stream);
hipError_t launch_nms(const int16_t *mag, const int16_t *angle, int16_t *out, int height, int width, int n_frames,
                      hipStream_t stream);
hipError_t launch_sobel_nms(const int16_t *smoothed, int16_t *out, int height, int width, int n_frames,
                            bool domain8, hipStream_t stream);
bool sobel_nms_march_supported(int height, int width);
void sobel_nms_set_px_variant(int v);
void sobel_nms_set_arith_variant(int v);
void sobel_nms_set_plane_store_variant(int v);
struct LaunchEvents {
    hipEvent_t start = nullptr, stop = nullptr;
};
hipError_t launch_sobel_nms_march(const int16_t *smoothed, int16_t *out, int height, int width, int n_frames,
                                  hipStream_t stream, int tune_seg = 0, const LaunchEvents &ev = {});

bool sobel_nms_classify_supported(int height, int width, int min_val);
hipError_t launch_sobel_nms_classify_march(const int16_t *smoothed, int16_t *edges, uint64_t *strong, uint64_t *conn,
                                           const HystGeom &g, int min_val, int max_val, int edge_value,
                                           hipStream_t stream, int tune_seg = 0, const LaunchEvents &ev = {},
                                           const int *pairs = nullptr);

bool sobel_nms_u8_input_supported();
hipError_t launch_sobel_nms_march_u8in(const uint8_t *smoothed, int16_t *out, int height, int width, int n_frames,
                                       hipStream_t stream, int tune_seg = 0, const LaunchEvents &ev = {});
hipError_t launch_sobel_nms_classify_march_u8in(const uint8_t *smoothed, int16_t *edges, uint64_t *strong,
                                                uint64_t *conn, const HystGeom &g, int min_val, int max_val,
                                                int edge_value, hipStream_t stream, int tune_seg = 0,
                                                const LaunchEvents &ev = {}, const int *pairs = nullptr);

__host__ __device__ inline void clamp_thresholds(int &lo, int &hi)
{
    lo = lo < 1 ? 1 : (lo > 255 ? 255 : lo);
    hi = hi < lo ? lo : (hi > 255 ? 255 : hi);
}

constexpr int kAutoMedian = 1, kAutoQuantile = 2;
constexpr int kHistBins = 257;

template <class Cum>
__host__ __device__ inline int hist_quantile(const Cum &cum, double q)
{
    const double t = ceil(q * (double)cum(kHistBins - 1));
    const unsigned long long need = t < 1.0 ? 1ull : (unsigned long long)t;
    int a = 0, b = kHistBins;
    while (a < b) {
        const int m = (a + b) >> 1;
        if (cum(m) >= need)
            b = m;
        else
            a = m + 1;
    }
    return a;
}

template <class Cum>
__host__ __device__ inline void auto_thresholds(const Cum &cum, int rule, double low, double high, int &lo, int &hi)
{
    if (rule == kAutoMedian) {
        const double m = (double)hist_quantile(cum, 0.5);
        lo = (int)floor(fmin(low * m, 256.0));
        hi = (int)floor(fmin(high * m, 256.0));
    } else {
        lo = hist_quantile(cum, low);
        hi = hist_quantile(cum, high);
    }
    clamp_thresholds(lo, hi);
}

hipError_t launch_hist_intensity(const void *plane, bool in_u8, uint32_t *hist, int height, int width, int n_frames,
                                 hipStream_t stream);
hipError_t launch_hist_gradient(const void *plane, bool in_u8, uint32_t *hist, int height, int width, int n_frames,
                                hipStream_t stream);
hipError_t launch_thr_select(const uint32_t *hist, int n_frames, int rule, double low, double high, int *pairs,
                             hipStream_t stream);

hipError_t launch_hyst_classify(const int16_t *cand, uint64_t *strong, uint64_t *conn, const HystGeom &g, int min_val,
                                int max_val, unsigned *domain_flag, hipStream_t stream, const int *pairs = nullptr);
inline size_t hyst_sched_words(const HystGeom &g) { return 5 * (size_t)g.tiles() + 4 + 4 * (size_t)g.n_frames; }
hipError_t launch_hyst_prepare(uint64_t *strong, uint64_t *conn, const HystGeom &g, bool zero_pad, unsigned *sched,
                               unsigned *flags, hipStream_t stream, int n_lanes = 1);
hipError_t launch_hyst_propagate(uint64_t *strong, const uint64_t *conn, unsigned *sched, unsigned *last_change,
                                 int iter, const HystGeom &g, hipStream_t stream, int16_t *edges = nullptr,
                                 int edge_value = 0, bool frame_queues = false);
hipError_t launch_hyst_tail(uint64_t *strong, const uint64_t *conn, unsigned *sched, unsigned *last_change,
                            int first_iter, const HystGeom &g, hipStream_t stream, int16_t *edges = nullptr,
                            int edge_value = 0);
hipError_t launch_edges_to_u8(const int16_t *edges, uint8_t *out, size_t n, hipStream_t stream);
hipError_t launch_edges_to_bits(const int16_t *edges, uint8_t *bits, int height, int width, int n_frames,
                                hipStream_t stream);
hipError_t launch_hyst_publish(const unsigned *flags, unsigned *host_flags_dev, unsigned seq, hipStream_t stream);
hipError_t launch_hyst_finalize(int16_t *cand, const uint64_t *strong, const HystGeom &g, int edge_value,
                                hipStream_t stream);
void hyst_set_finalize_mode(int mode);
hipError_t launch_fep_classify(const int16_t *cand, const uint8_t *visited, uint64_t *strong, uint64_t *conn,
                               const HystGeom &g, int start, int min_val, hipStream_t stream);
hipError_t launch_fep_finalize(int16_t *cand, uint8_t *visited, const uint64_t *strong, const HystGeom &g, int start,
                               int min_val, hipStream_t stream);

__host__ __device__ inline size_t hyst_word_index(const HystGeom &g, int f, int y, int wx)
{
    return ((((size_t)f * g.tiles_y + (y >> 6)) * g.tiles_x + wx) << 6) + (y & 63);
}
#ifdef __HIPCC__
template <bool BITS>
__device__ __forceinline__ uint64_t row_word(const void *__restrict__ src, const HystGeom &g, int row_bytes, int f,
                                             int y, int k)
{
    const int left = g.width - (k << 6);
    const uint64_t mask = left >= 64 ? ~0ull : ((1ull << left) - 1ull);
    if constexpr (!BITS) {
        return static_cast<const uint64_t *>(src)[hyst_word_index(g, f, y, k)] & mask;
    } else {
        const uint8_t *row = static_cast<const uint8_t *>(src) + ((size_t)f * g.height + y) * (size_t)row_bytes +
                             (size_t)k * 8;
        const int nb = min(8, row_bytes - k * 8);
        uint64_t w = 0;
        for (int j = 0; j < nb; j++) w |= (uint64_t)(__brev((unsigned)row[j]) >> 24) << (8 * j);
        return w & mask;
    }
}
#endif
hipError_t launch_points_count(const uint64_t *strong, const uint8_t *bits, const HystGeom &g, uint32_t *row_counts,
                               hipStream_t stream);
hipError_t launch_points_scan(uint32_t *rows, unsigned long long *frame_totals, unsigned long long *offsets, int height,
                              int n_frames, hipStream_t stream);
hipError_t launch_points_scatter(const uint64_t *strong, const uint8_t *bits, const HystGeom &g,
                                 const uint32_t *row_offsets, const unsigned long long *offsets, uint32_t *points,
                                 unsigned long long capacity, hipStream_t stream);

struct HoughGeom {
    int numangle, numrho;
    float rho, theta, min_theta;
};
constexpr int kHoughMaxLines = 4096;
constexpr int kHoughLdsMax = 160 * 1024;
inline size_t hough_accum_bytes(const HoughGeom &hg, int n_frames)
{
    return (size_t)n_frames * (hg.numangle + 2) * (size_t)(hg.numrho + 2) * sizeof(int);
}
#ifdef __HIPCC__
__device__ __forceinline__ int vote_r(int x, int y, float c, float s, int half)
{
    return (int)rintf(__fadd_rn(__fmul_rn((float)x, c), __fmul_rn((float)y, s))) + half;
}
#endif
int hough_lds_rows(const HoughGeom &hg, int budget_bytes);
hipError_t launch_hough_vote(const uint64_t *strong, const uint8_t *bits, const uint32_t *points,
                             const unsigned long long *offsets, const HystGeom &g, const HoughGeom &hg, const float *tab,
                             int *accum, int lds_rows, hipStream_t stream);
hipError_t launch_hough_peaks(const int *accum, int n_frames, const HoughGeom &hg, int threshold, int *counts,
                              unsigned *hist, int hist_bins, hipStream_t stream);
hipError_t launch_hough_select(const int *accum, int n_frames, const HoughGeom &hg, int threshold, int lines_max,
                               const int *counts, const unsigned *hist, int hist_bins, unsigned *ties, unsigned *cut,
                               unsigned long long *cand, float *lines, int *votes, unsigned *bases, hipStream_t stream);

struct CircleGeom {
    int min_radius, max_radius, cell_shift, aw, ah;
};
constexpr int kCircleMaxRadius = 1024;
constexpr int kCircleRecord = 6;
inline size_t circles_accum_bytes(const CircleGeom &cg, int n_frames)
{
    return (size_t)n_frames * (cg.ah + 2) * (size_t)(cg.aw + 2) * sizeof(int);
}
hipError_t launch_circles_vote(const uint64_t *strong, const uint8_t *bits, const HystGeom &g, const void *smoothed,
                               bool smoothed_u8, const int16_t *gx, const int16_t *gy, const CircleGeom &cg, int *accum,
// ... 84 lines not shown
```

### canny_edge_amd/csrc/canny_kernels.hip

```cpp
#include "canny_kernels.h"

#include <hip/hip_ext.h>

namespace canny {

__device__ __forceinline__ uint64_t shfl_up_u64(uint64_t v)
{
    unsigned lo = (unsigned)v, hi = (unsigned)(v >> 32);
    lo = __shfl_up(lo, 1);
    hi = __shfl_up(hi, 1);
    return ((uint64_t)hi << 32) | lo;
}
__device__ __forceinline__ uint64_t shfl_down_u64(uint64_t v)
{
    unsigned lo = (unsigned)v, hi = (unsigned)(v >> 32);
    lo = __shfl_down(lo, 1);
    hi = __shfl_down(hi, 1);
    return ((uint64_t)hi << 32) | lo;
}

__device__ __forceinline__ uint64_t readlane_u64(uint64_t v, int uniform_lane)
{
    const unsigned lo = (unsigned)__builtin_amdgcn_readlane((int)(unsigned)v, uniform_lane);
    const unsigned hi = (unsigned)__builtin_amdgcn_readlane((int)(unsigned)(v >> 32), uniform_lane);
// ... 666 lines not shown
        if (lane == 0) up = su;
        if (lane == 63) dn = sd;
        uint64_t d = up | s | dn;
        uint64_t d_from_left = quirk ? (up | s | (dn & ~1ull)) : d;
        uint64_t nb = d | (d_from_left << 1) | (d >> 1) | in_left | in_right;
        uint64_t gsel = s | (c & nb);
        if (!__any(gsel != s)) break;
        s = fill_runs(c, gsel);
    }

    const uint64_t chg = s ^ s0;
    const uint64_t rows_changed = __ballot(chg != 0);
    if (rows_changed != 0) {
        strong[base + lane] = s;
        if (edges) {
            const int f = t / tpf;
            const int cols = min(kTile, g.width - tx * kTile), rows = min(kTile, g.height - ty * kTile);
            int16_t *const tile0 = edges + ((size_t)f * g.height + (size_t)ty * kTile) * g.width + tx * kTile;
            if (__popcll(rows_changed) <= 16) {
                for (uint64_t m = rows_changed; m != 0; m &= m - 1) {
                    const int r = __builtin_ctzll(m);
                    const uint64_t word = readlane_u64(chg, r);
                    if (((word >> lane) & 1ull) != 0 && lane < cols && r < rows)
                        tile0[(size_t)r * g.width + lane] = (int16_t)edge_value;
                }
            } else if (lane < rows) {
                int16_t *const rowp = tile0 + (size_t)lane * g.width;
                for (uint64_t m = chg; m != 0; m &= m - 1) {
                    const int b = __builtin_ctzll(m);
                    if (b < cols) rowp[b] = (int16_t)edge_value;
                }
            }
        }
        const uint64_t top64 = readlane_u64(chg, 0);
        const uint64_t bot = readlane_u64(chg, 63);
        const bool anyL = __any((chg & 1ull) != 0), anyR = __any((chg >> 63) != 0);
        const int dy = (lane == 0 || lane == 4 || lane == 5) ? -1 : ((lane == 1 || lane == 6 || lane == 7) ? 1 : 0);
        const int dx = (lane == 2 || lane == 4 || lane == 6) ? -1 : ((lane == 3 || lane == 5 || lane == 7) ? 1 : 0);
        const uint64_t facing = dy < 0 ? top64 : bot;
        const bool hit = dy == 0 ? (dx < 0 ? anyL : anyR)
                                 : (dx == 0 ? facing != 0 : (dx < 0 ? (facing & 1ull) != 0 : (facing >> 63) != 0));
        const bool there = (dy >= 0 || hasU) && (dy <= 0 || hasD) && (dx >= 0 || hasL) && (dx <= 0 || hasR);
        const bool want = lane < 8 && hit && there;
        push_tiles(want, t + dy * g.tiles_x + dx);
    }
}

__device__ __forceinline__ void note_push(unsigned *last_change, unsigned nxt)
{
    if (__hip_atomic_load(last_change, __ATOMIC_RELAXED, __HIP_MEMORY_SCOPE_AGENT) < nxt) atomicMax(last_change, nxt);
}

__device__ __forceinline__ void process_tile(int t, int lane, uint64_t *__restrict__ strong, const HystSched &sch,
                                             unsigned *__restrict__ last_change, int iter, const HystGeom &g,
                                             int16_t *__restrict__ edges, int edge_value, uint64_t c,
                                             const TileIn &in, bool to_frame = false)
{
    const unsigned nxt = (unsigned)iter + 1u;
    unsigned *q = (nxt & 1u) ? sch.queue1 : sch.queue0;
    unsigned *cnt = sch.count + nxt % 3u;
    if (to_frame) {
        const int tpf = g.tiles_x * g.tiles_y;
        const int f = t / tpf;
        q = ((nxt & 1u) ? sch.fq1 : sch.fq0) + (size_t)f * tpf;
        cnt = sch.fcount + 4 * (size_t)f + nxt % 3u;
    }
    process_tile_with(t, lane, strong, iter, g, edges, edge_value, c, in, [&](bool want, int nb) {
        push_neighbours(want, lane, sch.stamp, (unsigned)nb, (unsigned)nb, nxt, q, cnt);
        if (__any(want) && lane == 0) note_push(last_change, nxt);
    });
}

__device__ __forceinline__ void propagate_tile(int t, int lane, uint64_t *__restrict__ strong,
                                               const uint64_t *__restrict__ conn, const HystSched &sch,
                                               unsigned *__restrict__ last_change, int iter, const HystGeom &g,
                                               int16_t *__restrict__ edges, int edge_value, uint64_t c,
                                               bool to_frame = false)
{
    if (!__any(c != 0)) return;
    const TileIn in = load_tile(t, lane, strong, g, c);
    process_tile(t, lane, strong, sch, last_change, iter, g, edges, edge_value, c, in, to_frame);
}

__global__ __launch_bounds__(256) void hyst_propagate_kernel(uint64_t *__restrict__ strong,
                                                             const uint64_t *__restrict__ conn,
                                                             unsigned *__restrict__ sched_words,
                                                             unsigned *__restrict__ last_change, int iter, HystGeom g,
                                                             int16_t *__restrict__ edges, int edge_value,
                                                             int frame_groups)
{
    const int lane = threadIdx.x & 63;
    const int wave = __builtin_amdgcn_readfirstlane(blockIdx.x * 4 + (threadIdx.x >> 6));
    const int n_waves = gridDim.x * 4;
    const int tiles = g.tiles();
    const HystSched sch = make_sched(sched_words, tiles);
    if (wave == 0 && lane == 0) sch.count[(iter + 2) % 3] = 0;
    if (iter == 0) {
        for (int t0 = wave * kSweep0Tiles; t0 < tiles; t0 += n_waves * kSweep0Tiles) {
            uint64_t c[kSweep0Tiles];
#pragma unroll
            for (int k = 0; k < kSweep0Tiles; k++)
                c[k] = (t0 + k < tiles) ? conn[(size_t)(t0 + k) * kTile + lane] : 0ull;
#pragma unroll
            for (int k = 0; k < kSweep0Tiles; k++)
                propagate_tile(t0 + k, lane, strong, conn, sch, last_change, iter, g, edges, edge_value, c[k],
                               frame_groups > 0);
        }
        return;
    }
    if (frame_groups > 0) {
        const int tpf = g.tiles_x * g.tiles_y;
        const int f = (int)blockIdx.x / frame_groups, part = (int)blockIdx.x - f * frame_groups;
        unsigned *const fcount = sch.fcount + 4 * (size_t)f;
        if (part == 0 && threadIdx.x == 0) fcount[(iter + 2) % 3] = 0;
        const unsigned n = min(__hip_atomic_load(fcount + iter % 3, __ATOMIC_RELAXED, __HIP_MEMORY_SCOPE_AGENT),
                               (unsigned)tpf);
        const unsigned *q = ((iter & 1) ? sch.fq1 : sch.fq0) + (size_t)f * tpf;
        const unsigned w = (unsigned)__builtin_amdgcn_readfirstlane(part * 4 + (int)(threadIdx.x >> 6));
        for (unsigned i = w; i < n; i += (unsigned)frame_groups * 4u) {
            const int t = (int)q[i];
            propagate_tile(t, lane, strong, conn, sch, last_change, iter, g, edges, edge_value,
                           conn[(size_t)t * kTile + lane], true);
        }
        return;
    }
    const unsigned n = __hip_atomic_load(sch.count + iter % 3, __ATOMIC_RELAXED, __HIP_MEMORY_SCOPE_AGENT);
    const unsigned *q = (iter & 1) ? sch.queue1 : sch.queue0;
    for (unsigned i = (unsigned)wave; i < n; i += (unsigned)n_waves) {
        const int t = (int)q[i];
        propagate_tile(t, lane, strong, conn, sch, last_change, iter, g, edges, edge_value,
                       conn[(size_t)t * kTile + lane]);
    }
}

constexpr int kTailTiles = 4096;
__global__ __launch_bounds__(1024) void hyst_tail_kernel(uint64_t *__restrict__ strong, const uint64_t *__restrict__ conn,
                                                         unsigned *__restrict__ sched_words,
                                                         unsigned *__restrict__ last_change, int first_iter, HystGeom g,
                                                         int16_t *__restrict__ edges, int edge_value)
{
    __shared__ unsigned s_queue[2][kTailTiles];
    __shared__ unsigned s_stamp[kTailTiles];
    __shared__ unsigned s_count[2];
    __shared__ unsigned s_last;
    const int lane = threadIdx.x & 63;
    const int wave = __builtin_amdgcn_readfirstlane(threadIdx.x >> 6), n_waves = blockDim.x >> 6;
    const int f = blockIdx.x;
    const int tpf = g.tiles_x * g.tiles_y;
    const int t_base = f * tpf;
    const HystSched sch = make_sched(sched_words, g.tiles());
    int cur = first_iter & 1;
    {
        const unsigned n0 = __hip_atomic_load(sch.fcount + 4 * (size_t)f + first_iter % 3, __ATOMIC_RELAXED,
                                              __HIP_MEMORY_SCOPE_AGENT);
        const unsigned *q0 = (cur ? sch.fq1 : sch.fq0) + (size_t)t_base;
        for (unsigned i = threadIdx.x; i < n0; i += blockDim.x)
            s_queue[cur][i] = __hip_atomic_load(q0 + i, __ATOMIC_RELAXED, __HIP_MEMORY_SCOPE_AGENT) - (unsigned)t_base;
        for (int i = threadIdx.x; i < tpf; i += blockDim.x) s_stamp[i] = 0;
        if (threadIdx.x == 0) {
            s_count[cur] = n0;
            s_count[cur ^ 1] = 0;
            s_last = 0;
        }
    }
    unsigned pushed = 0;
    for (int iter = first_iter;; iter++, cur ^= 1) {
        __syncthreads();
        const unsigned n = s_count[cur];
        __syncthreads();
        if (n == 0) break;
        if (threadIdx.x == 0) s_count[cur] = 0;
        unsigned *const q_next = s_queue[cur ^ 1];
        unsigned *const n_next = &s_count[cur ^ 1];
        const unsigned nxt = (unsigned)iter + 1u;
        for (unsigned i = (unsigned)wave; i < n; i += (unsigned)n_waves) {
            const int t = t_base + (int)s_queue[cur][i];
            const uint64_t c = conn[(size_t)t * kTile + lane];
            const TileIn in = load_tile(t, lane, strong, g);
            if (!__any(c != 0)) continue;
            process_tile_with(t, lane, strong, iter, g, edges, edge_value, c, in, [&](bool want, int nb) {
                const unsigned loc = (unsigned)(nb - t_base);
                push_neighbours(want, lane, s_stamp, loc, loc, nxt, q_next, n_next);
                if (__any(want)) pushed = nxt;
            });
        }
    }
    if (lane == 0 && pushed != 0) atomicMax(&s_last, pushed);
    __syncthreads();
    if (threadIdx.x == 0 && s_last != 0) atomicMax(last_change, s_last);
}

__global__ __launch_bounds__(256) void hyst_finalize_kernel(int16_t *__restrict__ cand,
                                                            const uint64_t *__restrict__ strong, HystGeom g,
                                                            int edge_value)
{
    const size_t plane = (size_t)g.height * g.width;
    const size_t total = plane * g.n_frames;
    const size_t stride = (size_t)gridDim.x * blockDim.x;
    for (size_t i = (size_t)blockIdx.x * blockDim.x + threadIdx.x; i < total; i += stride) {
        size_t f = i / plane, p = i - f * plane;
        int y = (int)(p / (size_t)g.width), x = (int)(p - (size_t)y * g.width);
// ... 117 lines not shown
        unsigned cbits = 0, sbits = 0;
        if (inside[k]) {
            const uint4 v = px4[k];
            const uint32_t w[4] = {v.x, v.y, v.z, v.w};
            if (fast) {
                const uint32_t r[4] = {__builtin_amdgcn_perm(w[2], w[0], 0x05040100u),
                                       __builtin_amdgcn_perm(w[2], w[0], 0x07060302u),
                                       __builtin_amdgcn_perm(w[3], w[1], 0x05040100u),
                                       __builtin_amdgcn_perm(w[3], w[1], 0x07060302u)};
                uint32_t dc[4], ds[4];
#pragma unroll
                for (int k = 0; k < 4; k++) {
                    const uint32_t a = pk_sub_sat_i16(r[k], lo2);
                    const uint32_t b = pk_sub_sat_i16(r[k], hi2);
                    dc[k] = a & 0x80008000u;
                    ds[k] = (a | b) & 0x80008000u;
                }
                const uint32_t xc = (dc[0] >> 3) | (dc[1] >> 2) | (dc[2] >> 1) | dc[3];
                const uint32_t xs = (ds[0] >> 3) | (ds[1] >> 2) | (ds[2] >> 1) | ds[3];
                cbits = (((xc >> 12) & 0xfu) | ((xc >> 24) & 0xf0u)) ^ 0xffu;
                sbits = (((xs >> 12) & 0xfu) | ((xs >> 24) & 0xf0u)) ^ 0xffu;
                if (lo <= 0 && cbits != 0xffu) atomicOr(domain_flag, 1u);
            } else {
                bool below = false;
#pragma unroll
                for (int e = 0; e < 8; e++) {
                    const int px = (e & 1) ? ((int)w[e >> 1] >> 16) : (int)(short)(w[e >> 1] & 0xffffu);
                    const bool c = px >= lo;
                    cbits |= (unsigned)c << e;
                    sbits |= (unsigned)(c && px >= hi) << e;
                    below |= px < lo;
                }
                if (lo <= 0 && below) atomicOr(domain_flag, 1u);
            }
        }
        conn[i] = (uint8_t)cbits;
        strong[i] = (uint8_t)sbits;
    }
}

__global__ __launch_bounds__(256) void hyst_finalize8_kernel(int16_t *__restrict__ cand,
                                                             const uint8_t *__restrict__ strong, HystGeom g,
                                                             int edge_value)
{
    const uint32_t ev = (uint32_t)(uint16_t)edge_value;
#pragma unroll
    for (int k = 0; k < kPatchItems; k++) {
        int f, y, x0;
        size_t i;
        if (!patch_coords(g, k, i, f, y, x0)) continue;
        const unsigned b = strong[i];
        const uint32_t t = b | (b << 15);
        uint4 v;
        v.x = __umul24(t & 0x00010001u, ev);
        v.y = __umul24((t >> 2) & 0x00010001u, ev);
        v.z = __umul24((t >> 4) & 0x00010001u, ev);
        v.w = __umul24((t >> 6) & 0x00010001u, ev);
        __builtin_memcpy(cand + ((size_t)f * g.height + y) * g.width + x0, &v, 16);
    }
}

hipError_t launch_hyst_classify(const int16_t *cand, uint64_t *strong, uint64_t *conn, const HystGeom &g, int min_val,
                                int max_val, unsigned *domain_flag, hipStream_t stream, const int *pairs)
{
    size_t n_words = (size_t)g.n_frames * g.tiles_y * kTile * g.tiles_x;
    const dim3 grid8((g.tiles_x + 1) / 2, g.tiles_y, g.n_frames), grid(grid_for(n_words * 64, 256));
    if (g.width % 8 == 0 && pairs)
        hipLaunchKernelGGL(hyst_classify8_kernel<true>, grid8, dim3(256), 0, stream, cand, (uint8_t *)strong,
                           (uint8_t *)conn, g, min_val, max_val, domain_flag, pairs);
    else if (g.width % 8 == 0)
        hipLaunchKernelGGL(hyst_classify8_kernel<false>, grid8, dim3(256), 0, stream, cand, (uint8_t *)strong,
                           (uint8_t *)conn, g, min_val, max_val, domain_flag, pairs);
    else if (pairs)
        hipLaunchKernelGGL(hyst_classify_kernel<true>, grid, dim3(256), 0, stream, cand, strong, conn, g, min_val,
                           max_val, domain_flag, pairs);
    else
        hipLaunchKernelGGL(hyst_classify_kernel<false>, grid, dim3(256), 0, stream, cand, strong, conn, g, min_val,
                           max_val, domain_flag, pairs);
    return hipGetLastError();
}
__global__ __launch_bounds__(256) void hyst_prepare_kernel(uint64_t *__restrict__ strong, uint64_t *__restrict__ conn,
                                                           HystGeom g, int pad_waves, unsigned *__restrict__ sched,
                                                           unsigned n_sched, unsigned *__restrict__ flags,
                                                           int n_flags)
{
    const int lane = (int)(threadIdx.x & 63);
    const int wave = (int)blockIdx.x * 4 + (int)(threadIdx.x >> 6);
    if (wave < pad_waves) {
        const int per_frame = g.tiles_x + g.tiles_y;
        const int f = wave / per_frame, k = wave - f * per_frame;
        const int tx = k < g.tiles_x ? k : g.tiles_x - 1;
        const int ty = k < g.tiles_x ? g.tiles_y - 1 : k - g.tiles_x;
        const size_t w = ((((size_t)f * g.tiles_y + ty) * g.tiles_x + tx) << 6) + lane;
        const int y = ty * kTile + lane;
        const int valid_px = min(kTile, g.width - tx * kTile);
        if (y >= g.height) {
            strong[w] = 0;
            conn[w] = 0;
        } else if (valid_px < kTile) {
            uint8_t *sb = (uint8_t *)(strong + w), *cb = (uint8_t *)(conn + w);
            for (int b = valid_px / 8; b < 8; b++) sb[b] = cb[b] = 0;
        }
        return;
    }
    const size_t i0 = ((size_t)(wave - pad_waves) * 64 + lane) * 4;
    for (int j = 0; j < 4; j++)
        if (i0 + j < n_sched) sched[i0 + j] = 0u;
    if (wave == pad_waves && lane < n_flags) flags[lane] = 0u;
}

hipError_t launch_hyst_prepare(uint64_t *strong, uint64_t *conn, const HystGeom &g, bool zero_pad, unsigned *sched,
                               unsigned *flags, hipStream_t stream, int n_lanes)
{
    if (n_lanes < 1 || n_lanes > 16) return hipErrorInvalidValue;
    const bool pad = zero_pad && (g.height % kTile != 0 || g.width % kTile != 0);
    const long long pad_waves = pad ? (long long)(g.tiles_x + g.tiles_y) * g.n_frames : 0;
    const size_t n_sched = 5 * (size_t)g.tiles() + 4 * (size_t)n_lanes + 4 * (size_t)g.n_frames;
    const long long waves = pad_waves + (long long)((n_sched + 255) / 256);
    if (pad_waves > 0x3fffffffLL || n_sched > 0xffffffffull) return hipErrorInvalidValue;
    hipLaunchKernelGGL(hyst_prepare_kernel, dim3((unsigned)((waves + 3) / 4)), dim3(256), 0, stream, strong, conn, g,
                       (int)pad_waves, sched, (unsigned)n_sched, flags, 2 * n_lanes);
    return hipGetLastError();
}

__global__ __launch_bounds__(256) void edges_to_u8_kernel(const int16_t *__restrict__ in, uint8_t *__restrict__ out,
                                                          size_t n)
{
    const size_t groups = n / 16;
    const size_t stride = (size_t)gridDim.x * blockDim.x;
    const bool aligned = (((uintptr_t)in | (uintptr_t)out) & 15u) == 0;
    for (size_t g = (size_t)blockIdx.x * blockDim.x + threadIdx.x; g < groups; g += stride) {
        if (aligned) {
            const uint4 a = *reinterpret_cast<const uint4 *>(in + g * 16);
            const uint4 b = *reinterpret_cast<const uint4 *>(in + g * 16 + 8);
            uint4 r;
            r.x = __builtin_amdgcn_perm(a.y, a.x, 0x06040200u);
            r.y = __builtin_amdgcn_perm(a.w, a.z, 0x06040200u);
            r.z = __builtin_amdgcn_perm(b.y, b.x, 0x06040200u);
            r.w = __builtin_amdgcn_perm(b.w, b.z, 0x06040200u);
            *reinterpret_cast<uint4 *>(out + g * 16) = r;
        } else {
            for (int k = 0; k < 16; k++) out[g * 16 + k] = (uint8_t)in[g * 16 + k];
        }
    }
    if (blockIdx.x == 0 && threadIdx.x < n % 16) out[groups * 16 + threadIdx.x] = (uint8_t)in[groups * 16 + threadIdx.x];
}

hipError_t launch_edges_to_u8(const int16_t *edges, uint8_t *out, size_t n, hipStream_t stream)
{
    if (n == 0) return hipSuccess;
    hipLaunchKernelGGL(edges_to_u8_kernel, dim3(grid_for(n / 16 + 1, 256)), dim3(256), 0, stream, edges, out, n);
    return hipGetLastError();
}

__global__ __launch_bounds__(256) void edges_to_bits_kernel(const int16_t *__restrict__ in, uint8_t *__restrict__ out,
                                                            int width, int row_bytes, size_t n_bytes, int vec_ok)
{
    const size_t stride = (size_t)gridDim.x * blockDim.x;
    for (size_t b = (size_t)blockIdx.x * blockDim.x + threadIdx.x; b < n_bytes; b += stride) {
        const size_t row = b / (size_t)row_bytes;
        const int xb = (int)(b - row * (size_t)row_bytes);
        const int16_t *px = in + row * (size_t)width + (size_t)xb * 8;
        unsigned byte = 0;
        if (vec_ok) {
            const uint4 v = *reinterpret_cast<const uint4 *>(px);
            const unsigned d[4] = {v.x, v.y, v.z, v.w};
#pragma unroll
            for (int k = 0; k < 4; k++)
                byte |= (((d[k] & 0xffffu) != 0 ? 2u : 0u) | ((d[k] >> 16) != 0 ? 1u : 0u)) << (6 - 2 * k);
        } else {
            const int left = width - xb * 8;
#pragma unroll
            for (int k = 0; k < 8; k++)
                if (k < left && px[k] != 0) byte |= 0x80u >> k;
        }
        out[b] = (uint8_t)byte;
    }
}

hipError_t launch_edges_to_bits(const int16_t *edges, uint8_t *bits, int height, int width, int n_frames,
                                hipStream_t stream)
{
    const int row_bytes = (width + 7) / 8;
    const size_t n_bytes = (size_t)n_frames * (size_t)height * (size_t)row_bytes;
    if (n_bytes == 0) return hipSuccess;
    const int vec_ok = (width % 8 == 0) && (((uintptr_t)edges & 15u) == 0);
    hipLaunchKernelGGL(edges_to_bits_kernel, dim3(grid_for(n_bytes, 256)), dim3(256), 0, stream, edges, bits, width,
                       row_bytes, n_bytes, vec_ok);
    return hipGetLastError();
}

__global__ void hyst_publish_kernel(const unsigned *__restrict__ flags, unsigned *host, unsigned seq)
{
    __hip_atomic_store(&host[0], flags[0], __ATOMIC_RELAXED, __HIP_MEMORY_SCOPE_SYSTEM);
    __hip_atomic_store(&host[1], flags[1], __ATOMIC_RELAXED, __HIP_MEMORY_SCOPE_SYSTEM);
    __hip_atomic_store(&host[2], seq, __ATOMIC_RELEASE, __HIP_MEMORY_SCOPE_SYSTEM);
}

hipError_t launch_hyst_publish(const unsigned *flags, unsigned *host_flags_dev, unsigned seq, hipStream_t stream)
{
    hipLaunchKernelGGL(hyst_publish_kernel, dim3(1), dim3(1), 0, stream, flags, host_flags_dev, seq);
    return hipGetLastError();
}

hipError_t launch_hyst_tail(uint64_t *strong, const uint64_t *conn, unsigned *sched, unsigned *last_change,
                            int first_iter, const HystGeom &g, hipStream_t stream, int16_t *edges, int edge_value)
{
    if (g.n_frames < 1 || first_iter < 1 || g.tiles_x * g.tiles_y > kTailTiles) return hipErrorInvalidValue;
    const int tpf = g.tiles_x * g.tiles_y;
    const unsigned threads = tpf >= 256 ? 1024u : (tpf >= 64 ? 512u : 256u);
    hipLaunchKernelGGL(hyst_tail_kernel, dim3((unsigned)g.n_frames), dim3(threads), 0, stream, strong, conn, sched,
                       last_change, first_iter, g, edges, edge_value);
    return hipGetLastError();
}

hipError_t launch_hyst_propagate(uint64_t *strong, const uint64_t *conn, unsigned *stamp, unsigned *last_change,
                                 int iter, const HystGeom &g, hipStream_t stream, int16_t *edges, int edge_value,
                                 bool frame_queues)
{
    if (frame_queues && (g.n_frames < 1 || g.tiles_x * g.tiles_y > kTailTiles)) return hipErrorInvalidValue;
    unsigned blocks = (unsigned)((g.tiles() + 4 * kSweep0Tiles - 1) / (4 * kSweep0Tiles));
    int frame_groups = frame_queues ? 1 : 0;
    if (iter > 0) {
        const unsigned want = (unsigned)((g.tiles() + 15) / 16);
        blocks = want < 8u ? 8u : (want > 1024u ? 1024u : want);
        if (frame_queues) {
            frame_groups = (int)(blocks / (unsigned)g.n_frames);
            if (frame_groups < 1) frame_groups = 1;
            blocks = (unsigned)frame_groups * (unsigned)g.n_frames;
        }
    }
    hipLaunchKernelGGL(hyst_propagate_kernel, dim3(blocks), dim3(256), 0, stream, strong, conn, stamp, last_change,
                       iter, g, edges, edge_value, frame_groups);
    return hipGetLastError();
}
__global__ __launch_bounds__(256) void hyst_finalize_rows_kernel(int16_t *__restrict__ cand,
                                                                 const uint8_t *__restrict__ strong, HystGeom g,
                                                                 int edge_value, int groups_per_row)
{
    const uint32_t ev = (uint32_t)(uint16_t)edge_value;
    const int chunk = (int)blockIdx.x * 4 + (int)(threadIdx.x >> 6);
    const int gx = chunk * 64 + (int)(threadIdx.x & 63);
    if (gx >= groups_per_row) return;
    const int f = (int)blockIdx.z;
    const int x0 = gx * 8;
    const size_t tile_col = ((size_t)f * g.tiles_y) * g.tiles_x + (gx >> 3);
    unsigned b[4];
#pragma unroll
    for (int k = 0; k < 4; k++) {
        const int y = (int)blockIdx.y * 4 + k;
        b[k] = 0;
        if (y < g.height)
            b[k] = strong[((tile_col + (size_t)(y >> 6) * g.tiles_x) << 9) + (size_t)(y & 63) * 8 + (gx & 7)];
    }
#pragma unroll
    for (int k = 0; k < 4; k++) {
        const int y = (int)blockIdx.y * 4 + k;
        if (y >= g.height) break;
        const uint32_t t = b[k] | (b[k] << 15);
        uint4 v;
        v.x = __umul24(t & 0x00010001u, ev);
        v.y = __umul24((t >> 2) & 0x00010001u, ev);
        v.z = __umul24((t >> 4) & 0x00010001u, ev);
        v.w = __umul24((t >> 6) & 0x00010001u, ev);
        __builtin_memcpy(cand + ((size_t)f * g.height + y) * g.width + x0, &v, 16);
    }
}

static int finalize_mode = 0;
void hyst_set_finalize_mode(int m) { finalize_mode = m; }

hipError_t launch_hyst_finalize(int16_t *cand, const uint64_t *strong, const HystGeom &g, int edge_value,
                                hipStream_t stream)
{
    size_t total = (size_t)g.n_frames * g.height * g.width;
    if (g.width % 8 == 0 && finalize_mode != 1) {
        const int groups = g.width / 8;
        hipLaunchKernelGGL(hyst_finalize_rows_kernel, dim3((groups + 255) / 256, (g.height + 3) / 4, g.n_frames),
                           dim3(256), 0, stream, cand, (const uint8_t *)strong, g, edge_value, groups);
    } else if (g.width % 8 == 0)
        hipLaunchKernelGGL(hyst_finalize8_kernel, dim3((g.tiles_x + 1) / 2, g.tiles_y, g.n_frames), dim3(256), 0, stream, cand,
                           (const uint8_t *)strong, g, edge_value);
    else
        hipLaunchKernelGGL(hyst_finalize_kernel, dim3(grid_for(total, 256)), dim3(256), 0, stream, cand, strong, g,
                           edge_value);
    return hipGetLastError();
}
hipError_t launch_fep_classify(const int16_t *cand, const uint8_t *visited, uint64_t *strong, uint64_t *conn,
                               const HystGeom &g, int start, int min_val, hipStream_t stream)
{
    size_t n_words = (size_t)g.tiles_y * kTile * g.tiles_x;
    hipLaunchKernelGGL(fep_classify_kernel, dim3(grid_for(n_words * 64, 256)), dim3(256), 0, stream, cand, visited,
                       strong, conn, g, start, min_val);
    return hipGetLastError();
}
hipError_t launch_fep_finalize(int16_t *cand, uint8_t *visited, const uint64_t *strong, const HystGeom &g, int start,
                               int min_val, hipStream_t stream)
{
    size_t total = (size_t)g.height * g.width;
    hipLaunchKernelGGL(fep_finalize_kernel, dim3(grid_for(total, 256)), dim3(256), 0, stream, cand, visited, strong, g,
                       start, min_val);
    return hipGetLastError();
}

__global__ __launch_bounds__(256) void selftest_mag_angle_kernel(int lim, int16_t *__restrict__ mags,
                                                                 uint8_t *__restrict__ bins)
{
    const int side = 2 * lim + 1;
    const size_t total = (size_t)side * side;
    const size_t stride = (size_t)gridDim.x * blockDim.x;
    for (size_t i = (size_t)blockIdx.x * blockDim.x + threadIdx.x; i < total; i += stride) {
        int gy = (int)(i / side) - lim, gx = (int)(i % side) - lim;
        mags[i] = (int16_t)magnitude_d8(gx, gy);
        bins[i] = (uint8_t)angle_bin_d8(gx, gy);
    }
}
// ... 30 lines not shown
```

### canny_edge_amd/csrc/canny_sobel_nms_march.hip

```cpp
#include "canny_kernels.h"

#include <hip/hip_ext.h>

#include <type_traits>

namespace canny {

namespace {

typedef short s16x2 __attribute__((ext_vector_type(2)));

__device__ __forceinline__ s16x2 as_v(uint32_t u) { return __builtin_bit_cast(s16x2, u); }
__device__ __forceinline__ uint32_t as_u(s16x2 v) { return __builtin_bit_cast(uint32_t, v); }
__device__ __forceinline__ uint32_t pk_add(uint32_t a, uint32_t b) { return as_u(as_v(a) + as_v(b)); }
__device__ __forceinline__ uint32_t pk_sub(uint32_t a, uint32_t b) { return as_u(as_v(a) - as_v(b)); }
__device__ __forceinline__ uint32_t pk_mad2(uint32_t a, uint32_t b)
{
    uint32_t r;
    const uint32_t two = 0x00020002u;
    asm("v_pk_mad_i16 %0, %1, %2, %3" : "=v"(r) : "v"(a), "s"(two), "v"(b));
    return r;
}

__device__ __forceinline__ uint32_t from_left(uint32_t v)
{
    return (uint32_t)__builtin_amdgcn_mov_dpp((int)v, 0x138 , 0xf, 0xf, true);
}
__device__ __forceinline__ uint32_t from_right(uint32_t v)
{
    return (uint32_t)__builtin_amdgcn_mov_dpp((int)v, 0x130 , 0xf, 0xf, true);
}
__device__ __forceinline__ void keep_gt_hi(uint32_t &pair, int a, int b, int zero)
{
    asm("v_cmp_gt_i32 vcc, %1, %2\n\t"
        "s_nop 1\n\t"
        "v_cndmask_b32_sdwa %0, %3, %1, vcc dst_sel:WORD_1 dst_unused:UNUSED_PRESERVE src0_sel:DWORD src1_sel:DWORD"
        : "+v"(pair)
        : "v"(a), "v"(b), "v"(zero)
        : "vcc");
}

__device__ __forceinline__ void push_gt2(unsigned &cbits, unsigned &sbits, int a, int b, int c)
{
    unsigned long long m;
    asm("v_cmp_gt_i32 vcc, %3, %4\n\t"
        "v_cmp_gt_i32 %2, %3, %5\n\t"
        "s_nop 0\n\t"
        "v_addc_co_u32 %0, vcc, %0, %0, vcc\n\t"
        "v_addc_co_u32 %1, %2, %1, %1, %2"
        : "+v"(cbits), "+v"(sbits), "=&s"(m)
        : "v"(a), "v"(b), "s"(c)
        : "vcc");
}

template <int NP>
struct SnmCfg {
    static constexpr int PX = 2 * NP;
    static constexpr int SW = 62 * PX;
};
constexpr int SNM_STAGE_ROWS = 64;
constexpr int SNM_WPB = 4;

template <int N>
using IC = std::integral_constant<int, N>;
#ifndef FLT_WAVES
#define FLT_WAVES 4
#endif
#ifndef FLT_GROUP
#define FLT_GROUP 2
#endif
#ifndef FLT_EARLY_RELOAD
#define FLT_EARLY_RELOAD 1
#endif
#ifndef FLT_DEFER_STORE
#define FLT_DEFER_STORE 1
#endif
#ifndef FLT_CARRIERS
#define FLT_CARRIERS 1
#endif
#define FLT_SCHED_FENCE() __builtin_amdgcn_sched_barrier(0)

struct StripJob {
    const int16_t *fin;
    const uint8_t *fin8;
    int16_t *fout;
    int H, W, ybeg, yend, x0, lane;
    uint8_t *pconn, *pstrong;
    int tiles_x, lo1, hi1;
    int edge_value;
};

__device__ __forceinline__ int max_u16(int a, int b)
{
    int r;
    asm("v_max_u16 %0, %1, %2" : "=v"(r) : "v"(a), "v"(b));
    return r;
}

template <int NP>
__device__ __forceinline__ void store_row(int16_t *dst, const uint32_t (&outp)[NP])
{
    __builtin_memcpy(dst, outp, 4 * NP);
}

__device__ __forceinline__ int pk_pixel_mag(float fx, float fy, float &Ah, float &nh)
{
    Ah = __fmaf_rn(fx, fx, 0.5f);
    nh = __fmaf_rn(fy, fy, Ah);
    return (int)__builtin_amdgcn_sqrtf(nh);
}
__device__ __forceinline__ void pk_pixel_disc(float fx, float fy, float Ah, float nh, float &P, float &Q)
{
    P = __fmul_rn(fx, fy);
    Q = __fmaf_rn(nh, -0.5f, Ah);
}
__device__ __forceinline__ int pk_nms_select(float P, float Q, int n0, int n45, int n90, int n135)
{
    const bool v_ge0 = P <= Q;
    const bool u_ge0 = P > -Q;
    const int na = v_ge0 ? n0 : n45;
    const int nb = v_ge0 ? n135 : n90;
    return u_ge0 ? na : nb;
}

template <bool COL_EDGE, bool ROW_EDGE, bool PLANES, int NP, bool LDS_PLANES, bool IN_U8 = false>
__device__ __forceinline__ void march_strip(const StripJob &jb, uint8_t *stage_mem, const uint4 *edge_lut = nullptr)
{
    static_assert(!IN_U8 || NP == 4, "the u8 input form exists for 8 pixels per lane only");
    constexpr int PX = 2 * NP;
    const int H = jb.H, W = jb.W, x0 = jb.x0, ybeg = jb.ybeg, yend = jb.yend;
    const bool full8 = x0 >= 0 && x0 + PX - 1 < W;
    const bool owner = jb.lane >= 1 && jb.lane <= 62 && x0 < W;

    uint32_t fix_l = 0, fix_r[NP] = {};
    unsigned oob = 0;
    if (COL_EDGE) {
        fix_l = (x0 == 0) ? 0x0000ffffu : 0u;
#pragma unroll
        for (int i = 0; i < NP; i++) {
            if (x0 + 2 * i == W - 1) fix_r[i] |= 0x0000ffffu;
            if (x0 + 2 * i + 1 == W - 1) fix_r[i] |= 0xffff0000u;
        }
#pragma unroll
        for (int e = 0; e < PX; e++)
            if (x0 + e < 0 || x0 + e >= W) oob |= 1u << e;
    }

    auto load_row = [&](int r, uint32_t (&p)[NP]) {
#pragma unroll
        for (int i = 0; i < NP; i++) p[i] = 0u;
        if (ROW_EDGE && (r < 0 || r >= H)) return;
        if (IN_U8) {
            const uint8_t *src8 = jb.fin8 + (size_t)r * W + x0;
            if (!COL_EDGE || full8) {
                __builtin_memcpy(p, src8, 8);
            } else if (x0 + PX - 1 >= 0 && x0 < W) {
#pragma unroll
                for (int e = 0; e < PX; e++) {
                    int x = x0 + e;
                    if (x >= 0 && x < W) p[e >> 2] |= (uint32_t)src8[e] << (8 * (e & 3));
                }
            }
            return;
        }
        const int16_t *src = jb.fin + (size_t)r * W + x0;
        if (!COL_EDGE || full8) {
            __builtin_memcpy(p, src, 4 * NP);
        } else {
            if (x0 + PX - 1 >= 0 && x0 < W) {
#pragma unroll
                for (int e = 0; e < PX; e++) {
                    int x = x0 + e;
                    if (x >= 0 && x < W) p[e >> 1] |= (uint32_t)(uint16_t)src[e] << (16 * (e & 1));
                }
            }
        }
    };

    int skip = PLANES ? jb.lo1 : 0;
    asm volatile("" : "+v"(skip));
    uint32_t d[3][NP], t[3][NP];
    int M[3][PX + 2];
    float cP[3][PX], cQ[3][PX];
#pragma unroll
    for (int a = 0; a < 3; a++) {
#pragma unroll
        for (int i = 0; i < NP; i++) d[a][i] = t[a][i] = 0u;
#pragma unroll
        for (int e = 0; e < PX + 2; e++) M[a][e] = skip;
#pragma unroll
        for (int e = 0; e < PX; e++) cP[a][e] = cQ[a][e] = 0.0f;
    }

    constexpr bool STAGE = LDS_PLANES && PLANES && NP == 4;
    constexpr unsigned kStagePitch = 72, kStageRows = SNM_STAGE_ROWS, kStagePlane = kStageRows * kStagePitch;
    uint8_t *const stage = stage_mem;
    unsigned stage_col = 0;
    int st_o = 0, st_e = 0, st_w0 = 0;
    if (STAGE) {
        const int strip_b0 = (x0 - (jb.lane - 1) * PX) >> 3;
        const int nb = COL_EDGE ? max(0, min(62, (W >> 3) - strip_b0)) : 62;
        st_o = strip_b0 & 7;
        st_w0 = strip_b0 >> 3;
        st_e = st_o + nb;
        stage_col = jb.lane == 0 ? 71u : (unsigned)(st_o + jb.lane - 1);
    }
    auto stage_flush_segment = [&]() {
        const int y = ybeg + jb.lane;
        const bool row_ok = y < yend;
        const unsigned lrow = (unsigned)jb.lane * kStagePitch;
        const unsigned grow = (unsigned)(y >> 6) * (unsigned)jb.tiles_x * 512u + (unsigned)(y & 63) * 8u;
        __builtin_amdgcn_fence(__ATOMIC_ACQ_REL, "wavefront");
        const int wf0 = (st_o + 7) >> 3, wf1 = st_e >> 3;
        for (int k = wf0; k < wf1; k++) {
            if (row_ok) {
                const unsigned g = grow + (unsigned)(st_w0 + k) * 512u;
                *reinterpret_cast<uint64_t *>(jb.pconn + g) = *reinterpret_cast<const uint64_t *>(stage + lrow + 8 * k);
                *reinterpret_cast<uint64_t *>(jb.pstrong + g) =
                    *reinterpret_cast<const uint64_t *>(stage + kStagePlane + lrow + 8 * k);
            }
        }
        auto leftover = [&](int i) {
            if (!row_ok) return;
            const unsigned g = grow + (unsigned)(st_w0 + (i >> 3)) * 512u + (unsigned)(i & 7);
            if (!COL_EDGE) {
                *reinterpret_cast<uint16_t *>(jb.pconn + g) = *reinterpret_cast<const uint16_t *>(stage + lrow + i);
                *reinterpret_cast<uint16_t *>(jb.pstrong + g) =
                    *reinterpret_cast<const uint16_t *>(stage + kStagePlane + lrow + i);
            } else {
                jb.pconn[g] = stage[lrow + i];
                jb.pstrong[g] = stage[kStagePlane + lrow + i];
            }
        };
        constexpr int kStep = COL_EDGE ? 1 : 2;
        const int head_end = min(8 * wf0, st_e), tail_beg = max(8 * wf1, head_end);
        for (int i = st_o; i < head_end; i += kStep) leftover(i);
        for (int i = tail_beg; i < st_e; i += kStep) leftover(i);
        __builtin_amdgcn_fence(__ATOMIC_ACQ_REL, "wavefront");
    };

    constexpr bool DEFER = FLT_DEFER_STORE != 0;
    uint32_t pend[NP] = {};
    auto park = [&](const uint32_t (&outp)[NP]) {
#pragma unroll
        for (int q = 0; q < NP; q++) pend[q] = outp[q];
    };
    constexpr bool PARKS = DEFER && ((PLANES && STAGE) || (!PLANES && !COL_EDGE));
    auto store_pending = [&](int y) {
        if (PARKS && y >= ybeg && y < yend) {
            if (owner) store_row<NP>(jb.fout + (size_t)y * W + x0, pend);
        }
    };

    auto step = [&](auto ph, int r, const uint32_t (&praw)[NP]) {
        constexpr int PH = decltype(ph)::value;
        uint32_t p[NP];
        if (IN_U8) {
            p[0] = __builtin_amdgcn_perm(praw[0], praw[0], 0x0c010c00u);
            p[1] = __builtin_amdgcn_perm(praw[0], praw[0], 0x0c030c02u);
            p[NP > 2 ? 2 : 0] = __builtin_amdgcn_perm(praw[1], praw[1], 0x0c010c00u);
            p[NP > 2 ? 3 : 1] = __builtin_amdgcn_perm(praw[1], praw[1], 0x0c030c02u);
        } else {
#pragma unroll
            for (int i = 0; i < NP; i++) p[i] = praw[i];
        }
        if (DEFER) {
#pragma unroll
            for (int i = 0; i < NP; i++) asm volatile("" : "+v"(p[i]));
            __builtin_amdgcn_sched_barrier(0);
            store_pending(r - 3);
            __builtin_amdgcn_sched_barrier(0);
        }
        constexpr int k2 = PH % 3, k1 = (PH + 2) % 3, k0 = (PH + 1) % 3;
        constexpr int m2 = PH % 3, m1 = (PH + 2) % 3, m0 = (PH + 1) % 3;

        {
            const uint32_t lp = from_left(p[NP - 1]), rp = from_right(p[0]);
            uint32_t sh[NP + 1];
            sh[0] = __builtin_amdgcn_alignbit(p[0], lp, 16);
#pragma unroll
            for (int i = 1; i < NP; i++) sh[i] = __builtin_amdgcn_alignbit(p[i], p[i - 1], 16);
            sh[NP] = __builtin_amdgcn_alignbit(rp, p[NP - 1], 16);
#pragma unroll
            for (int i = 0; i < NP; i++) {
                d[k2][i] = pk_sub(sh[i + 1], sh[i]);
                t[k2][i] = pk_mad2(p[i], pk_add(sh[i], sh[i + 1]));
            }
            if (COL_EDGE) {
                d[k2][0] = pk_sub(d[k2][0], p[0] & fix_l);
#pragma unroll
                for (int i = 0; i < NP; i++) d[k2][i] = pk_add(d[k2][i], p[i] & fix_r[i]);
            }
        }

        const int y1 = r - 1;
        if (!ROW_EDGE || (y1 >= 0 && y1 < H)) {
            uint32_t gy[NP];
            if (ROW_EDGE && (y1 == 0 || y1 == H - 1)) {
#pragma unroll
                for (int i = 0; i < NP; i++) {
                    const uint32_t tu = (y1 == 0) ? t[k1][i] : t[k0][i];
                    const uint32_t td = (y1 == H - 1) ? t[k1][i] : t[k2][i];
                    gy[i] = pk_sub(td, tu);
                }
            } else {
#pragma unroll
                for (int i = 0; i < NP; i++) gy[i] = pk_sub(t[k2][i], t[k0][i]);
            }
#pragma unroll
            for (int i = 0; i < NP; i++) {
                const uint32_t gx = pk_add(pk_mad2(d[k1][i], d[k0][i]), d[k2][i]);
#pragma unroll
                for (int hf = 0; hf < 2; hf++) {
                    const int e = 2 * i + hf;
                    const float fx = hf ? (float)((int)gx >> 16) : (float)(int)(short)(gx & 0xffffu);
                    const float fy = hf ? (float)((int)gy[i] >> 16) : (float)(int)(short)(gy[i] & 0xffffu);
                    float Ah, nh;
                    const int mag = pk_pixel_mag(fx, fy, Ah, nh);
                    M[m2][e + 1] = PLANES ? max_u16(mag, skip) : mag;
                    pk_pixel_disc(fx, fy, Ah, nh, cP[m2][e], cQ[m2][e]);
// ... 170 lines not shown
    auto inside = [&](int e) { return in_m[e]; };

    uint32_t lane_off = (uint32_t)x0;
    auto load_row = [&](int r, uint32_t (&p)[NP]) {
#pragma unroll
        for (int i = 0; i < NP; i++) p[i] = 0u;
        if (ROW_EDGE && (r < 0 || r >= H)) return;
        if (IN_U8) {
            if (!COL_EDGE) {
                asm volatile("" : "+v"(lane_off));
                __builtin_memcpy(p, jb.fin8 + (size_t)r * W + lane_off, 8);
                return;
            }
            const uint8_t *src8 = jb.fin8 + (size_t)r * W + x0;
            if (!COL_EDGE || full8) {
                __builtin_memcpy(p, src8, 8);
            } else if (x0 + PX - 1 >= 0 && x0 < W) {
#pragma unroll
                for (int e = 0; e < PX; e++) {
                    int x = x0 + e;
                    if (x >= 0 && x < W) p[e >> 2] |= (uint32_t)src8[e] << (8 * (e & 3));
                }
            }
            return;
        }
        if (!COL_EDGE) {
            asm volatile("" : "+v"(lane_off));
            __builtin_memcpy(p, reinterpret_cast<const char *>(jb.fin + (size_t)r * W) + 2 * lane_off, 4 * NP);
            return;
        }
        const int16_t *src = jb.fin + (size_t)r * W + x0;
        if (!COL_EDGE || full8) {
            __builtin_memcpy(p, src, 4 * NP);
        } else if (x0 + PX - 1 >= 0 && x0 < W) {
#pragma unroll
            for (int e = 0; e < PX; e++) {
                int x = x0 + e;
                if (x >= 0 && x < W) p[e >> 1] |= (uint32_t)(uint16_t)src[e] << (16 * (e & 1));
            }
        }
    };

    int skip = PLANES ? jb.lo1 : 0;
    int hi1v = PLANES ? jb.hi1 : 0;
    asm volatile("" : "+v"(skip), "+v"(hi1v));

    float F[3][PX];
    int M[3][PX + 2];
    int cz[3][PX];
#if FLT_CARRIERS != 1
    int cy[3][PX];
#endif
#pragma unroll
    for (int a = 0; a < 3; a++) {
#pragma unroll
        for (int e = 0; e < PX; e++) {
            F[a][e] = 0.0f;
            cz[a][e] = 0;
        }
#pragma unroll
        for (int e = 0; e < PX + 2; e++) M[a][e] = skip;
    }

    constexpr bool STAGE = LDS_PLANES && PLANES;
    constexpr unsigned kStagePitch = 72, kStageRows = SNM_STAGE_ROWS, kStagePlane = kStageRows * kStagePitch;
    uint8_t *const stage = stage_mem;
    unsigned stage_col = 0;
    int st_o = 0, st_e = 0, st_w0 = 0;
    if (STAGE) {
        const int strip_b0 = (x0 - (jb.lane - 1) * PX) >> 3;
        const int nb = COL_EDGE ? max(0, min(62, (W >> 3) - strip_b0)) : 62;
        st_o = strip_b0 & 7;
        st_w0 = strip_b0 >> 3;
        st_e = st_o + nb;
        stage_col = jb.lane == 0 ? 71u : (unsigned)(st_o + jb.lane - 1);
    }
    auto stage_flush_segment = [&]() {
        const int y = ybeg + jb.lane;
        const bool row_ok = y < yend;
        const unsigned lrow = (unsigned)jb.lane * kStagePitch;
        const unsigned grow = (unsigned)(y >> 6) * (unsigned)jb.tiles_x * 512u + (unsigned)(y & 63) * 8u;
        __builtin_amdgcn_fence(__ATOMIC_ACQ_REL, "wavefront");
        const int wf0 = (st_o + 7) >> 3, wf1 = st_e >> 3;
        for (int k = wf0; k < wf1; k++) {
            if (row_ok) {
                const unsigned g = grow + (unsigned)(st_w0 + k) * 512u;
                *reinterpret_cast<uint64_t *>(jb.pconn + g) = *reinterpret_cast<const uint64_t *>(stage + lrow + 8 * k);
                *reinterpret_cast<uint64_t *>(jb.pstrong + g) =
                    *reinterpret_cast<const uint64_t *>(stage + kStagePlane + lrow + 8 * k);
            }
        }
        auto leftover = [&](int i) {
            if (!row_ok) return;
            const unsigned g = grow + (unsigned)(st_w0 + (i >> 3)) * 512u + (unsigned)(i & 7);
            if (!COL_EDGE) {
                *reinterpret_cast<uint16_t *>(jb.pconn + g) = *reinterpret_cast<const uint16_t *>(stage + lrow + i);
                *reinterpret_cast<uint16_t *>(jb.pstrong + g) =
                    *reinterpret_cast<const uint16_t *>(stage + kStagePlane + lrow + i);
            } else {
                jb.pconn[g] = stage[lrow + i];
                jb.pstrong[g] = stage[kStagePlane + lrow + i];
            }
        };
        constexpr int kStep = COL_EDGE ? 1 : 2;
        const int head_end = min(8 * wf0, st_e), tail_beg = max(8 * wf1, head_end);
        for (int i = st_o; i < head_end; i += kStep) leftover(i);
        for (int i = tail_beg; i < st_e; i += kStep) leftover(i);
        __builtin_amdgcn_fence(__ATOMIC_ACQ_REL, "wavefront");
    };

    constexpr bool DEFER = FLT_DEFER_STORE != 0;
    uint32_t pend[NP] = {};
    auto park = [&](const uint32_t (&outp)[NP]) {
#pragma unroll
        for (int q = 0; q < NP; q++) pend[q] = outp[q];
    };
    constexpr bool PARKS = DEFER && ((PLANES && STAGE) || (!PLANES && !COL_EDGE));
    auto store_pending = [&](int y) {
        if (PARKS && y >= ybeg && y < yend) {
            if (!COL_EDGE) {
                asm volatile("" : "+v"(lane_off));
                if (owner)
                    store_row<NP>(reinterpret_cast<int16_t *>(reinterpret_cast<char *>(jb.fout + (size_t)y * W) +
                                                              2 * lane_off), pend);
            } else if (owner) {
                store_row<NP>(jb.fout + (size_t)y * W + x0, pend);
            }
        }
    };

    auto step = [&](auto ph, int r, uint32_t (&praw)[NP]) {
        constexpr int PH = decltype(ph)::value;
        constexpr int k2 = PH % 3, k1 = (PH + 2) % 3, k0 = (PH + 1) % 3;
        constexpr int m2 = PH % 3, m1 = (PH + 2) % 3, m0 = (PH + 1) % 3;

#pragma unroll
        for (int e = 0; e < PX; e++) {
            const uint32_t w = IN_U8 ? praw[e >> 2] >> (8 * (e & 3)) : praw[e >> 1] >> (16 * (e & 1));
            F[k2][e] = (float)(w & 0xffu);
        }
        if (DEFER) {
#pragma unroll
            for (int e = 0; e < PX; e++) asm volatile("" : "+v"(F[k2][e]));
            FLT_SCHED_FENCE();
            store_pending(r - 3);
            FLT_SCHED_FENCE();
        }
        if (FLT_EARLY_RELOAD) {
#pragma unroll
            for (int e = 0; e < PX; e++) asm volatile("" : "+v"(F[k2][e]));
            load_row(r + 3, praw);
            FLT_SCHED_FENCE();
        }

        const int y1 = r - 1;
        if (!ROW_EDGE || (y1 >= 0 && y1 < H)) {
            float a[PX], b[PX];
#pragma unroll
            for (int e = 0; e < PX; e++) {
                a[e] = __fadd_rn(__fmaf_rn(2.0f, F[k1][e], F[k0][e]), F[k2][e]);
                const float up = (ROW_EDGE && y1 == 0) ? F[k1][e] : F[k0][e];
                const float dn = (ROW_EDGE && y1 == H - 1) ? F[k1][e] : F[k2][e];
                b[e] = __fsub_rn(dn, up);
            }
            const float a_l = f_from_left(a[PX - 1]), a_r = f_from_right(a[0]);
            const float b_l = f_from_left(b[PX - 1]), b_r = f_from_right(b[0]);
            FLT_SCHED_FENCE();
#pragma unroll
            for (int e = 0; e < PX; e++) {
                if (e && e % FLT_GROUP == 0) FLT_SCHED_FENCE();
                const float al = e ? a[e - 1] : a_l, ar = e < PX - 1 ? a[e + 1] : a_r;
                const float bl = e ? b[e - 1] : b_l, br = e < PX - 1 ? b[e + 1] : b_r;
                float gx = __fsub_rn(ar, al);
                if (COL_EDGE) {
                    if (e == 0) gx = __fmaf_rn(-fix_l, a[0], gx);
                    gx = __fadd_rn(gx, __int_as_float(__float_as_int(a[e]) & (inside(e) ^ inside(e + 1))));
                }
                const float gy = __fadd_rn(__fmaf_rn(2.0f, b[e], bl), br);
                float Ah, nh;
                int m = f_pixel_mag_word(gx, gy, Ah, nh);
                if (COL_EDGE) m &= inside(e);
                M[m2][e + 1] = f_pixel_mag_store<PLANES>(m, skip);
                float qm, qp;
                f_pixel_bin_signs(gx, gy, Ah, nh, qm, qp);
#if FLT_CARRIERS == 1
                cz[m2][e] = f_pixel_carrier(qm, qp);
                asm volatile("" : "+v"(cz[m2][e]));
#else
                cz[m2][e] = __float_as_int(qm);
                cy[m2][e] = __float_as_int(qp);
// ... 74 lines not shown
                for (int i = 0; i < NP; i++) outp[i] = (uint32_t)keep[2 * i] | ((uint32_t)keep[2 * i + 1] << 16);
                int16_t *dst = jb.fout + (size_t)y2 * W + x0;
                if (!COL_EDGE || full8) {
                    store_row<NP>(dst, outp);
                } else {
#pragma unroll
                    for (int e = 0; e < PX; e++)
                        if (x0 + e < W) dst[e] = (int16_t)keep[e];
                }
            }
        }
    };

    const int rfirst = ybeg - 2;
    const int rlast = rfirst + 3 * ((yend + 1 - rfirst + 3) / 3) - 1;
    uint32_t pa[NP], pb[NP], pc[NP];
    load_row(rfirst, pa);
    load_row(rfirst + 1, pb);
    if (FLT_EARLY_RELOAD) {
        load_row(rfirst + 2, pc);
        for (int r = rfirst; r <= rlast; r += 3) {
            step(IC<0>{}, r, pa);
            step(IC<1>{}, r + 1, pb);
            step(IC<2>{}, r + 2, pc);
        }
    } else {
        for (int r = rfirst; r <= rlast; r += 3) {
            load_row(r + 2, pc);
            step(IC<0>{}, r, pa);
            load_row(r + 3, pa);
            step(IC<1>{}, r + 1, pb);
            load_row(r + 4, pb);
            step(IC<2>{}, r + 2, pc);
        }
    }
    store_pending(rlast - 2);
    if (STAGE) stage_flush_segment();
}

__global__ __launch_bounds__(256) void selftest_sobel_pixel_kernel(int form, int lim, int16_t *__restrict__ mags,
                                                                   uint8_t *__restrict__ bins)
{
    const int side = 2 * lim + 1;
    const size_t total = (size_t)side * side;
    const size_t stride = (size_t)gridDim.x * blockDim.x;
    int skip = 0;
    asm volatile("" : "+v"(skip));
    for (size_t i = (size_t)blockIdx.x * blockDim.x + threadIdx.x; i < total; i += stride) {
        const float gx = (float)((int)(i % side) - lim), gy = (float)((int)(i / side) - lim);
        float Ah, nh;
        int mag, bin;
        if (form == 1) {
            mag = pk_pixel_mag(gx, gy, Ah, nh);
            float P, Q;
            pk_pixel_disc(gx, gy, Ah, nh, P, Q);
            bin = pk_nms_select(P, Q, 0, 45, 90, 135);
        } else {
            const int m = f_pixel_mag_word(gx, gy, Ah, nh);
            mag = form == 3 ? f_pixel_mag_store<true>(m, skip) : f_pixel_mag_store<false>(m, skip);
            float qm, qp;
            f_pixel_bin_signs(gx, gy, Ah, nh, qm, qp);
            bin = f_nms_select(f_pixel_carrier(qm, qp), 0, 45, 90, 135);
        }
        mags[i] = (int16_t)((mag >> 16) ? -1 : mag);
        bins[i] = (uint8_t)bin;
    }
}

}

hipError_t launch_selftest_sobel_pixel(int form, int lim, int16_t *mags, uint8_t *bins, hipStream_t stream)
{
    if (form < 1 || form > 3 || lim < 0 || lim > 1020) return hipErrorInvalidValue;
    const size_t total = (size_t)(2 * lim + 1) * (2 * lim + 1);
    hipLaunchKernelGGL(selftest_sobel_pixel_kernel, dim3((unsigned)((total + 255) / 256)), dim3(256), 0, stream, form,
                       lim, mags, bins);
    return hipGetLastError();
}

struct PlaneArgs {
    uint8_t *conn, *strong;
    int tiles_x, tiles_y, lo1, hi1, edge_value;
    const int *thr;
};

template <bool PLANES, int NP, bool LDS_PLANES, bool IN_U8 = false, bool FLT = false, bool THR = false>
__global__ __launch_bounds__(SNM_WPB * 64) __attribute__((amdgpu_waves_per_eu(FLT ? FLT_WAVES : 1)))
void sobel_nms_march_kernel(const void *__restrict__ in,
                                                                       int16_t *__restrict__ out, int H, int W,
                                                                       int n_strips, int n_segs, int seg_rows,
                                                                       int total_waves, PlaneArgs pl)
{
    __shared__ __attribute__((aligned(8))) uint8_t stage_lds[LDS_PLANES ? SNM_WPB * 2 * SNM_STAGE_ROWS * 72 : 8];
    uint8_t *stage_mem = stage_lds + (LDS_PLANES ? (threadIdx.x >> 6) * (2 * SNM_STAGE_ROWS * 72) : 0);
    __shared__ uint4 edge_lut[LDS_PLANES ? 256 : 1];
    if (LDS_PLANES) {
        static_assert(SNM_WPB * 64 == 256, "one table entry per thread");
        const unsigned b = threadIdx.x, ev = (unsigned)pl.edge_value;
        uint4 v;
        v.x = ((b >> 0) & 1u) * ev | (((b >> 1) & 1u) * ev) << 16;
        v.y = ((b >> 2) & 1u) * ev | (((b >> 3) & 1u) * ev) << 16;
        v.z = ((b >> 4) & 1u) * ev | (((b >> 5) & 1u) * ev) << 16;
        v.w = ((b >> 6) & 1u) * ev | (((b >> 7) & 1u) * ev) << 16;
        edge_lut[b] = v;
        __syncthreads();
    }
    unsigned bid = blockIdx.x;
    {
        const unsigned q = gridDim.x / 8u, r = gridDim.x % 8u, xcd = bid % 8u;
        bid = (xcd < r ? xcd * (q + 1u) : r * (q + 1u) + (xcd - r) * q) + bid / 8u;
    }
    const int wave = __builtin_amdgcn_readfirstlane(bid * SNM_WPB + (threadIdx.x >> 6));
    if (wave >= total_waves) return;
    const int f = wave / (n_strips * n_segs);
    const MarchCell cell = march_cell_of(wave - f * (n_strips * n_segs), n_segs, n_strips);
    const int s = cell.strip, g = cell.seg;
    StripJob jb;
    jb.lane = threadIdx.x & 63;
    jb.H = H;
    jb.W = W;
    jb.ybeg = g * seg_rows;
    jb.yend = min(H, jb.ybeg + seg_rows);
    jb.x0 = s * SnmCfg<NP>::SW + (jb.lane - 1) * SnmCfg<NP>::PX;
    jb.fin = (const int16_t *)in + (size_t)f * H * W;
    jb.fin8 = (const uint8_t *)in + (size_t)f * H * W;
    jb.fout = out + (size_t)f * H * W;
    if (PLANES) {
        jb.edge_value = pl.edge_value;
        const size_t frame_bytes = (size_t)pl.tiles_y * pl.tiles_x * 512;
        jb.pconn = pl.conn + (size_t)f * frame_bytes;
        jb.pstrong = pl.strong + (size_t)f * frame_bytes;
        jb.tiles_x = pl.tiles_x;
        if constexpr (THR) {
            int lo = pl.thr[2 * f], hi = pl.thr[2 * f + 1];
            clamp_thresholds(lo, hi);
            jb.lo1 = lo - 1;
            jb.hi1 = hi - 1;
        } else {
            jb.lo1 = pl.lo1;
            jb.hi1 = pl.hi1;
        }
    }
    const bool col_edge = (s == 0) || ((s + 1) * SnmCfg<NP>::SW + SnmCfg<NP>::PX >= W);
    const bool row_edge = (jb.ybeg < 2) || (jb.yend + (FLT && FLT_EARLY_RELOAD ? 6 : 5) >= H);
    if constexpr (FLT) {
        static_assert(NP == 4, "the f32 variant processes 8 pixels per lane");
#ifdef PROBE_VARIANT
        fmarch_strip<(PROBE_VARIANT & 1) != 0, (PROBE_VARIANT & 2) != 0, PLANES, LDS_PLANES, IN_U8>(jb, stage_mem, edge_lut);
        return;
#endif
        if (col_edge) {
            if (row_edge)
                fmarch_strip<true, true, PLANES, LDS_PLANES, IN_U8>(jb, stage_mem, edge_lut);
            else
                fmarch_strip<true, false, PLANES, LDS_PLANES, IN_U8>(jb, stage_mem, edge_lut);
        } else {
            if (row_edge)
                fmarch_strip<false, true, PLANES, LDS_PLANES, IN_U8>(jb, stage_mem, edge_lut);
            else
                fmarch_strip<false, false, PLANES, LDS_PLANES, IN_U8>(jb, stage_mem, edge_lut);
        }
    } else if (col_edge) {
        if (row_edge)
            march_strip<true, true, PLANES, NP, LDS_PLANES, IN_U8>(jb, stage_mem, edge_lut);
        else
            march_strip<true, false, PLANES, NP, LDS_PLANES, IN_U8>(jb, stage_mem, edge_lut);
    } else {
        if (row_edge)
            march_strip<false, true, PLANES, NP, LDS_PLANES, IN_U8>(jb, stage_mem, edge_lut);
        else
            march_strip<false, false, PLANES, NP, LDS_PLANES, IN_U8>(jb, stage_mem, edge_lut);
    }
}

bool sobel_nms_march_supported(int height, int width) { return height >= 2 && width >= 2; }

static int px_variant = 0;
void sobel_nms_set_px_variant(int v) { px_variant = v; }
static int arith_variant = 0;
void sobel_nms_set_arith_variant(int v) { arith_variant = v; }
static int plane_store_variant = 0;
void sobel_nms_set_plane_store_variant(int v) { plane_store_variant = v; }

template <class K, class... A>
static void launch_timed(K kernel, dim3 grid, dim3 block, hipStream_t stream, const LaunchEvents &ev, A... args)
{
    if (ev.start && ev.stop)
        hipExtLaunchKernelGGL(kernel, grid, block, 0, stream, ev.start, ev.stop, 0, args...);
    else
        hipLaunchKernelGGL(kernel, grid, block, 0, stream, args...);
}

template <bool THR = false>
static hipError_t launch_march(const void *smoothed, int16_t *out, const PlaneArgs *planes, int height, int width,
                               int n_frames, hipStream_t stream, int tune_seg, const LaunchEvents &ev,
                               bool in_u8 = false)
{
    const int np = px_variant == 1 ? 2 : 4;
    if (in_u8 && !(np == 4 && (!planes || plane_store_variant == 0))) return hipErrorNotSupported;
    const int sw = 62 * 2 * np;
    int n_strips = (width + sw - 1) / sw;
    int seg = 64;
    while (seg > 32 && (long long)n_frames * n_strips * ((height + seg - 1) / seg) < 16384) seg >>= 1;
    while (seg > 8 && (long long)n_frames * n_strips * ((height + seg - 1) / seg) < 2048) seg >>= 1;
    if (tune_seg >= 8) seg = tune_seg;
    if (planes && np == 4 && plane_store_variant == 0 && seg > SNM_STAGE_ROWS) seg = SNM_STAGE_ROWS;
    int n_segs = (height + seg - 1) / seg;
    long long waves = (long long)n_frames * n_strips * n_segs;
    if (waves > 0x7fffffffLL) return hipErrorInvalidValue;
    unsigned blocks = (unsigned)((waves + SNM_WPB - 1) / SNM_WPB);
    const PlaneArgs pl = planes ? *planes : PlaneArgs{};
    const dim3 grid(blocks), block(SNM_WPB * 64);
    const bool use_f32 = arith_variant == 2 || (arith_variant == 0 && planes != nullptr);
    if (use_f32 && np == 4) {
        const bool lds = planes && plane_store_variant == 0;
#define CANNY_FLT_LAUNCH(P, L, U)                                                                                      \
    launch_timed(sobel_nms_march_kernel<P, 4, L, U, true, P && THR>, grid, block, stream, ev, smoothed, out, height,   \
                 width, n_strips, n_segs, seg, (int)waves, pl)
        if (planes && lds && in_u8) CANNY_FLT_LAUNCH(true, true, true);
        else if (planes && lds) CANNY_FLT_LAUNCH(true, true, false);
        else if (planes) CANNY_FLT_LAUNCH(true, false, false);
        else if (in_u8) CANNY_FLT_LAUNCH(false, false, true);
        else CANNY_FLT_LAUNCH(false, false, false);
#undef CANNY_FLT_LAUNCH
        return hipGetLastError();
    }
    if (in_u8 && planes)
        launch_timed(sobel_nms_march_kernel<true, 4, true, true, false, THR>, grid, block, stream, ev, smoothed, out, height, width,
                     n_strips, n_segs, seg, (int)waves, pl);
    else if (in_u8)
        launch_timed(sobel_nms_march_kernel<false, 4, false, true>, grid, block, stream, ev, smoothed, out, height,
                     width, n_strips, n_segs, seg, (int)waves, pl);
    else if (planes && np == 4 && plane_store_variant == 0)
        launch_timed(sobel_nms_march_kernel<true, 4, true, false, false, THR>, grid, block, stream, ev, smoothed, out, height, width,
                     n_strips, n_segs, seg, (int)waves, pl);
    else if (planes && np == 4)
        launch_timed(sobel_nms_march_kernel<true, 4, false, false, false, THR>, grid, block, stream, ev, smoothed, out, height, width,
                     n_strips, n_segs, seg, (int)waves, pl);
    else if (planes)
        launch_timed(sobel_nms_march_kernel<true, 2, false, false, false, THR>, grid, block, stream, ev, smoothed, out, height, width,
                     n_strips, n_segs, seg, (int)waves, pl);
    else if (np == 4)
        launch_timed(sobel_nms_march_kernel<false, 4, false>, grid, block, stream, ev, smoothed, out, height, width,
                     n_strips, n_segs, seg, (int)waves, pl);
    else
        launch_timed(sobel_nms_march_kernel<false, 2, false>, grid, block, stream, ev, smoothed, out, height, width,
                     n_strips, n_segs, seg, (int)waves, pl);
    return hipGetLastError();
}

hipError_t launch_sobel_nms_march(const int16_t *smoothed, int16_t *out, int height, int width, int n_frames,
                                  hipStream_t stream, int tune_seg, const LaunchEvents &ev)
{
    return launch_march(smoothed, out, nullptr, height, width, n_frames, stream, tune_seg, ev);
}

bool sobel_nms_classify_supported(int height, int width, int min_val)
{
    return sobel_nms_march_supported(height, width) && width % 8 == 0 && min_val >= 1;
}

bool sobel_nms_u8_input_supported() { return px_variant == 0 && plane_store_variant == 0; }

hipError_t launch_sobel_nms_march_u8in(const uint8_t *smoothed, int16_t *out, int height, int width, int n_frames,
                                       hipStream_t stream, int tune_seg, const LaunchEvents &ev)
{
    return launch_march(smoothed, out, nullptr, height, width, n_frames, stream, tune_seg, ev, true);
}

static hipError_t classify_march_any(const void *smoothed, bool in_u8, int16_t *edges, uint64_t *strong, uint64_t *conn,
                                     const HystGeom &g, int min_val, int max_val, int edge_value, hipStream_t stream,
                                     int tune_seg, const LaunchEvents &ev, const int *pairs);

hipError_t launch_sobel_nms_classify_march(const int16_t *smoothed, int16_t *edges, uint64_t *strong, uint64_t *conn,
                                           const HystGeom &g, int min_val, int max_val, int edge_value,
                                           hipStream_t stream, int tune_seg, const LaunchEvents &ev, const int *pairs)
{
    return classify_march_any(smoothed, false, edges, strong, conn, g, min_val, max_val, edge_value, stream, tune_seg, ev,
                              pairs);
}

hipError_t launch_sobel_nms_classify_march_u8in(const uint8_t *smoothed, int16_t *edges, uint64_t *strong,
                                                uint64_t *conn, const HystGeom &g, int min_val, int max_val,
                                                int edge_value, hipStream_t stream, int tune_seg,
                                                const LaunchEvents &ev, const int *pairs)
{
    return classify_march_any(smoothed, true, edges, strong, conn, g, min_val, max_val, edge_value, stream, tune_seg, ev,
                              pairs);
}

static hipError_t classify_march_any(const void *smoothed, bool in_u8, int16_t *edges, uint64_t *strong, uint64_t *conn,
                                     const HystGeom &g, int min_val, int max_val, int edge_value, hipStream_t stream,
                                     int tune_seg, const LaunchEvents &ev, const int *pairs)
{
    if (pairs) min_val = max_val = 255;
    if (!sobel_nms_classify_supported(g.height, g.width, min_val)) return hipErrorNotSupported;
    if (edge_value < 0 || edge_value > 32767) return hipErrorInvalidValue;
    const int lo = min_val > 4096 ? 4096 : min_val;
    const int hi = max_val > 4096 ? 4096 : max_val;
    PlaneArgs pl;
    pl.conn = (uint8_t *)conn;
    pl.strong = (uint8_t *)strong;
    pl.tiles_x = g.tiles_x;
    pl.tiles_y = g.tiles_y;
    pl.lo1 = lo - 1;
    pl.hi1 = (hi > lo ? hi : lo) - 1;
    pl.edge_value = edge_value;
    pl.thr = pairs;
    if (pairs) {
        if (edge_value != 255) return hipErrorInvalidValue;
        return launch_march<true>(smoothed, edges, &pl, g.height, g.width, g.n_frames, stream, tune_seg, ev, in_u8);
    }
    return launch_march(smoothed, edges, &pl, g.height, g.width, g.n_frames, stream, tune_seg, ev, in_u8);
}

}
```

### include/canny_hip.h

```cpp
#ifndef CANNY_HIP_H
#define CANNY_HIP_H

#include <stddef.h>

#ifdef __cplusplus
extern "C" {
#endif

#define CANNY_HIP_VERSION 1201
#define CANNY_HIP_MAX_WINDOW 129

typedef struct canny_hip_ctx canny_hip_ctx;

enum canny_hip_status {
    CANNY_HIP_OK = 0,
    CANNY_HIP_ERR_INVALID = 1,
    CANNY_HIP_ERR_UNSUPPORTED = 2,
    CANNY_HIP_ERR_NO_DEVICE = 3,
    CANNY_HIP_ERR_RUNTIME = 4,
    CANNY_HIP_ERR_DOMAIN = 5,
    CANNY_HIP_ERR_NO_CONVERGE = 6
};

enum canny_hip_stage {
    CANNY_HIP_STAGE_GAUSSIAN = 0,
    CANNY_HIP_STAGE_SOBEL_NMS = 1,
    CANNY_HIP_STAGE_HYST_CLASSIFY = 2,
    CANNY_HIP_STAGE_HYST_PROPAGATE = 3,
    CANNY_HIP_STAGE_HYST_FINALIZE = 4,
    CANNY_HIP_STAGE_SOBEL = 5,
    CANNY_HIP_STAGE_NMS = 6,
    CANNY_HIP_STAGE_XY_GRADIENT = 7,
    CANNY_HIP_STAGE_TO_GRAY = 8,
    CANNY_HIP_STAGE_COUNT = 9,
    CANNY_HIP_STAGE_COMPACT = 9,
    CANNY_HIP_STAGE_END = 10
};

enum canny_hip_layout {
    CANNY_HIP_GRAY8 = 0,
    CANNY_HIP_BGR8 = 1,
    CANNY_HIP_RGB8 = 2,
    CANNY_HIP_BGRA8 = 3,
    CANNY_HIP_RGBA8 = 4
};

int canny_hip_version(void);
const char *canny_hip_status_string(int status);
int canny_hip_device_count(int *count);

int canny_hip_ctx_create(canny_hip_ctx **ctx, int device);
void canny_hip_ctx_destroy(canny_hip_ctx *ctx);
int canny_hip_ctx_set_stream(canny_hip_ctx *ctx, void *hip_stream);
int canny_hip_ctx_device(const canny_hip_ctx *ctx);
int canny_hip_ctx_set_option(canny_hip_ctx *ctx, const char *name, int value);
int canny_hip_ctx_get_option(const canny_hip_ctx *ctx, const char *name, int *value);
int canny_hip_synchronize(canny_hip_ctx *ctx);
const char *canny_hip_last_error(const canny_hip_ctx *ctx);
int canny_hip_last_hysteresis_iterations(canny_hip_ctx *ctx);

int canny_hip_malloc(canny_hip_ctx *ctx, void **dev_ptr, size_t bytes);
int canny_hip_free(canny_hip_ctx *ctx, void *dev_ptr);
int canny_hip_host_alloc(canny_hip_ctx *ctx, void **host_ptr, size_t bytes);
int canny_hip_host_free(canny_hip_ctx *ctx, void *host_ptr);
int canny_hip_host_register(canny_hip_ctx *ctx, void *host_ptr, size_t bytes);
int canny_hip_host_unregister(canny_hip_ctx *ctx, void *host_ptr);
int canny_hip_memcpy_h2d(canny_hip_ctx *ctx, void *dev_dst, const void *host_src, size_t bytes);
int canny_hip_memcpy_d2h(canny_hip_ctx *ctx, void *host_dst, const void *dev_src, size_t bytes);

int canny_hip_gaussian_kernel(float sigma, float *taps, int cap, int *window);
int canny_hip_gaussian(canny_hip_ctx *ctx, const unsigned char *img, float sigma, int height, int width,
                       short *result);
int canny_hip_xy_gradient(canny_hip_ctx *ctx, const short *img, int height, int width, short *grad_x,
                          short *grad_y);
int canny_hip_sobel(canny_hip_ctx *ctx, const short *img, int height, int width, short *magnitude,
                    short *angle);
int canny_hip_nms(canny_hip_ctx *ctx, const short *magnitude, const short *angle, int height, int width,
                  short *result);
int canny_hip_hysteresis(canny_hip_ctx *ctx, short *edge_candidates, int height, int width, int min_val,
                         int max_val);
int canny_hip_find_edge_pixels(canny_hip_ctx *ctx, short *edge_candidates, unsigned char *visited, int start,
                               int min_val, int max_val, int height, int width);
int canny_hip_canny(canny_hip_ctx *ctx, const unsigned char *img, float sigma, int min_val, int max_val,
                    int height, int width, short *edges);
int canny_hip_canny_batch(canny_hip_ctx *ctx, const unsigned char *imgs, int n_frames, float sigma, int min_val,
                          int max_val, int height, int width, short *edges);
int canny_hip_canny_batch_u8(canny_hip_ctx *ctx, const unsigned char *imgs, int n_frames, float sigma, int min_val,
                             int max_val, int height, int width, unsigned char *edges);
int canny_hip_canny_batch_bits(canny_hip_ctx *ctx, const unsigned char *imgs, int n_frames, float sigma, int min_val,
                               int max_val, int height, int width, unsigned char *bits);
int canny_hip_canny_multi_gpu(const unsigned char *imgs, int n_frames, float sigma, int min_val, int max_val,
                              int height, int width, short *edges, int n_devices);
// ... 215 lines not shown
    CANNY_HIP_POLYGON_PART_SCAN = 1,
    CANNY_HIP_POLYGON_PART_EMIT = 2,
    CANNY_HIP_POLYGON_PARTS = 3
};
int canny_hip_dev_polygons_chains(canny_hip_ctx *ctx, const unsigned long long *d_offsets, int n_frames,
                                  unsigned long long capacity, const unsigned long long *d_chain_offsets,
                                  const int *d_points, unsigned long long point_capacity, int width, int height,
                                  unsigned epsilon_q8, unsigned ratio_q16, unsigned long long *d_vertex_offsets,
                                  int *d_vertices, unsigned long long vertex_capacity, long long *d_measures);
int canny_hip_dev_canny_polygons(canny_hip_ctx *ctx, const unsigned char *d_img, float sigma, int min_val, int max_val,
                                 int height, int width, int n_frames, short *d_edges, int min_area, int *d_stats,
                                 unsigned long long capacity, unsigned long long *d_offsets,
                                 unsigned long long *d_chain_offsets, int *d_points, unsigned long long point_capacity,
                                 unsigned long long *d_point_offsets, unsigned epsilon_q8, unsigned ratio_q16,
                                 unsigned long long *d_vertex_offsets, int *d_vertices, unsigned long long vertex_capacity,
                                 long long *d_measures);
int canny_hip_dev_polygons_bits(canny_hip_ctx *ctx, const unsigned char *d_bits, int height, int width, int n_frames,
                                int min_area, int *d_stats, unsigned long long capacity, unsigned long long *d_offsets,
                                unsigned long long *d_chain_offsets, int *d_points, unsigned long long point_capacity,
                                unsigned long long *d_point_offsets, unsigned epsilon_q8, unsigned ratio_q16,
                                unsigned long long *d_vertex_offsets, int *d_vertices, unsigned long long vertex_capacity,
                                long long *d_measures);
int canny_hip_canny_polygons(canny_hip_ctx *ctx, const unsigned char *imgs, int n_frames, float sigma, int min_val,
                             int max_val, int height, int width, int min_area, int *stats, unsigned long long capacity,
                             unsigned long long *offsets, unsigned long long *chain_offsets, int *points,
                             unsigned long long point_capacity, unsigned long long *point_offsets, unsigned epsilon_q8,
                             unsigned ratio_q16, unsigned long long *vertex_offsets, int *vertices,
                             unsigned long long vertex_capacity, long long *measures);
int canny_hip_polygons_from_chains(const unsigned long long *chain_offsets, const int *points,
                                   unsigned long long n_records, unsigned long long point_capacity, int width, int height,
                                   unsigned epsilon_q8, unsigned ratio_q16, unsigned long long *vertex_offsets,
                                   int *vertices, unsigned long long vertex_capacity, long long *measures);

#define CANNY_HIP_EDT_NONE 0x7FFFFFFF
enum canny_hip_edt_part {
    CANNY_HIP_EDT_PART_ROWS = 0,
    CANNY_HIP_EDT_PART_COLUMNS = 1,
    CANNY_HIP_EDT_PARTS = 2
};
int canny_hip_dev_canny_edt(canny_hip_ctx *ctx, const unsigned char *d_img, float sigma, int min_val, int max_val,
                            int height, int width, int n_frames, short *d_edges, int *d_dist2, float *d_dist,
                            int *d_nearest);
int canny_hip_dev_edt_bits(canny_hip_ctx *ctx, const unsigned char *d_bits, int height, int width, int n_frames,
                           int *d_dist2, float *d_dist, int *d_nearest);
int canny_hip_canny_edt(canny_hip_ctx *ctx, const unsigned char *imgs, int n_frames, float sigma, int min_val, int max_val,
                        int height, int width, int *dist2, float *dist, int *nearest);
int canny_hip_edt_from_bits(const unsigned char *bits, int height, int width, int *dist2, float *dist, int *nearest);

int canny_hip_profile_enable(canny_hip_ctx *ctx, int on);
int canny_hip_profile_reset(canny_hip_ctx *ctx);
int canny_hip_profile_get(canny_hip_ctx *ctx, int stage, double *total_ms, long *launches);
int canny_hip_hough_profile_get(canny_hip_ctx *ctx, int part, double *total_ms, long *launches);
int canny_hip_components_profile_get(canny_hip_ctx *ctx, int part, double *total_ms, long *launches);
int canny_hip_edt_profile_get(canny_hip_ctx *ctx, int part, double *total_ms, long *launches);
int canny_hip_hough_segments_profile_get(canny_hip_ctx *ctx, int part, double *total_ms, long *launches);

int canny_hip_contours_profile_get(canny_hip_ctx *ctx, int part, double *total_ms, long *launches);
int canny_hip_hough_circles_profile_get(canny_hip_ctx *ctx, int part, double *total_ms, long *launches);
int canny_hip_polygons_profile_get(canny_hip_ctx *ctx, int part, double *total_ms, long *launches);

int canny_hip_selftest_mag_angle(canny_hip_ctx *ctx, int lim, short *magnitudes, unsigned char *bins);
enum canny_hip_pixel_form {
    CANNY_HIP_PIXEL_LDS_TILE = 0,
    CANNY_HIP_PIXEL_PACKED_I16 = 1,
    CANNY_HIP_PIXEL_F32 = 2,
    CANNY_HIP_PIXEL_F32_FLOOR = 3
};
int canny_hip_selftest_sobel_pixel(canny_hip_ctx *ctx, int form, int lim, short *magnitudes, unsigned char *bins);
int canny_hip_probe_copy(canny_hip_ctx *ctx, const void *d_src, void *d_dst, size_t nbytes, int launches,
                         double *avg_ms);

int canny_hip_selftest_div(canny_hip_ctx *ctx, float divisor, unsigned long long *mismatches,
                           float *largest_mismatching_dividend);
int canny_hip_selftest_div_fma(canny_hip_ctx *ctx, float divisor, float c, unsigned long long *mismatches,
                               float *largest_mismatching_dividend);
int canny_hip_selftest_div_fma_table(int index, float *divisor, float *c);
int canny_hip_selftest_expand_bits(const unsigned char *bits, int height, int width, int to_u8, void *out, int n_threads);
int canny_hip_selftest_march_order(int n_segs, int n_strips, int *out_pairs);
int canny_hip_selftest_cpulist_count(const char *text);
int canny_hip_selftest_histogram(canny_hip_ctx *ctx, const void *d_plane, int plane_is_u8, int kind, int height, int width,
                                 int n_frames, unsigned int *d_hist);
int canny_hip_selftest_select(canny_hip_ctx *ctx, const unsigned int *d_hist, int n_frames, int rule, float low, float high,
                              int *d_pairs);
enum canny_hip_workspace_kind { CANNY_HIP_WS_DATA = 0, CANNY_HIP_WS_INDEX = 1, CANNY_HIP_WS_CACHE = 2 };
int canny_hip_selftest_workspace(canny_hip_ctx *ctx, int index, const char **name, void **d_ptr, size_t *bytes, int *kind);

#ifdef __cplusplus
}
#endif
#endif
```

Measured before the change: 582,700 Mpixels/s.

## Emit per-tile hysteresis flags from Sobel/NMS to build sweep-0 work lists

The fused Sobel+NMS+classify kernel now writes per-tile flags (strong and weak present) into a small buffer, and hysteresis prepare uses them to build per-frame tile lists. Propagate iteration 0 then visits only the listed tiles instead of scanning every tile's planes. This is meant to cut the full-plane sweep at the start of hysteresis, at the cost of extra ballots and flag stores in the march kernel and an extra prepare launch on the tail route. It also caps SGPRs on the propagate kernel and adds a selftest plus tuning options.

```diff
diff --git a/canny_edge_amd/capi.py b/canny_edge_amd/capi.py
--- a/canny_edge_amd/capi.py
+++ b/canny_edge_amd/capi.py
@@ -57,7 +57,8 @@
     "canny_hip_canny_batch_u8", "canny_hip_dev_canny_u8", "canny_hip_canny_multi_gpu", "canny_hip_shard_range", "canny_hip_dev_gaussian", "canny_hip_dev_xy_gradient",
     "canny_hip_dev_sobel", "canny_hip_dev_nms", "canny_hip_dev_sobel_nms", "canny_hip_dev_hysteresis",
     "canny_hip_dev_canny", "canny_hip_dev_canny_stream", "canny_hip_dev_canny_stream_flush", "canny_hip_profile_enable", "canny_hip_profile_reset", "canny_hip_profile_get",
-    "canny_hip_selftest_mag_angle", "canny_hip_selftest_sobel_pixel", "canny_hip_selftest_div", "canny_hip_selftest_div_fma",
+    "canny_hip_selftest_mag_angle", "canny_hip_selftest_sobel_pixel", "canny_hip_selftest_sweep0_lists",
+    "canny_hip_selftest_div", "canny_hip_selftest_div_fma",
     "canny_hip_selftest_div_fma_table", "canny_hip_canny_multi_gpu_u8", "canny_hip_multi_gpu_set_option",
     "canny_hip_multi_gpu_release", "canny_hip_device_local_cpus", "canny_hip_selftest_cpulist_count",
     "canny_hip_dev_gaussian_u8", "canny_hip_dev_sobel_nms_u8in", "canny_hip_host_register", "canny_hip_host_unregister",
@@ -172,6 +173,7 @@
         "canny_hip_selftest_march_order": ([i, i, p], i),
         "canny_hip_selftest_mag_angle": ([p, i, p, p], i),
         "canny_hip_selftest_sobel_pixel": ([p, i, i, p, p], i),
+        "canny_hip_selftest_sweep0_lists": ([p, p, C.c_float, i, i, i, i, i, p, p], i),
         "canny_hip_selftest_div": ([p, f, C.POINTER(C.c_ulonglong), C.POINTER(C.c_float)], i),
         "canny_hip_selftest_div_fma": ([p, f, f, C.POINTER(C.c_ulonglong), C.POINTER(C.c_float)], i),
         "canny_hip_selftest_div_fma_table": ([i, C.POINTER(C.c_float), C.POINTER(C.c_float)], i),
@@ -1209,6 +1211,14 @@
                     "selftest_sobel_pixel")
         return mags, bins
 
+    def selftest_sweep0_lists(self, d_img: int, sigma: float, min_val: int, max_val: int, h: int, w: int, n: int):
+        tpf = ((h + 63) // 64) * ((w + 63) // 64)
+        counts = np.zeros(n, np.uint32)
+        tiles = np.zeros((n, tpf), np.uint32)
+        self._check(self._L.canny_hip_selftest_sweep0_lists(self._h, C.c_void_p(d_img), sigma, min_val, max_val, h, w, n,
+                                                            _hp(counts), _hp(tiles)), "selftest_sweep0_lists")
+        return [tiles[f, :min(int(counts[f]), tpf)].copy() for f in range(n)], counts
+
     def selftest_div(self, divisor: float) -> Tuple[int, float]:
         bad, worst = C.c_ulonglong(0), C.c_float(0.0)
         self._check(self._L.canny_hip_selftest_div(self._h, divisor, C.byref(bad), C.byref(worst)), "selftest_div")
diff --git a/canny_edge_amd/csrc/canny_capi.hip b/canny_edge_amd/csrc/canny_capi.hip
--- a/canny_edge_amd/csrc/canny_capi.hip
+++ b/canny_edge_amd/csrc/canny_capi.hip
@@ -315,6 +315,7 @@
     int last_fused_gray = 0;
     int hyst_tail = 1;
     int hyst_tail_after = 2;
+    int hyst_sweep0_lists = 1;
     bool hyst_iters_async = false;
     int batch_workers = 0;
     int batch_chunk_mb = 0;
@@ -346,6 +347,7 @@
     DevBuf seg_ws, seg_lines, seg_work;
     DevBuf circ_accum, circ_ws;
     DevBuf plane_s, plane_c, stamps, flags;
+    DevBuf tile_flags;
     DevBuf io[4];
     std::string ws_name;
     unsigned *host_flags = nullptr;
@@ -585,6 +587,7 @@
     HIP_TRY(ctx, ctx->plane_c.ensure(g.words() * sizeof(uint64_t)));
     HIP_TRY(ctx, ctx->stamps.ensure((hyst_sched_words(g) + 4) * sizeof(unsigned)));
     HIP_TRY(ctx, ctx->flags.ensure(4 * sizeof(unsigned)));
+    HIP_TRY(ctx, ctx->tile_flags.ensure(2 * (size_t)g.tiles()));
     if (!ctx->host_flags) {
         HIP_TRY(ctx, hipHostMalloc((void **)&ctx->host_flags, 8 * sizeof(unsigned), hipHostMallocMapped));
         std::memset(ctx->host_flags, 0, 8 * sizeof(unsigned));
@@ -793,11 +796,13 @@
         pairs = out;
     }
     auto fused_sobel = [&](const short *smp, short *edges, uint64_t *S, uint64_t *C, const HystGeom &gg, int ev,
-                           const LaunchEvents &le, const int *pp) -> hipError_t {
+                           const LaunchEvents &le, const int *pp, uint8_t *tile_flags = nullptr,
+                           bool *flags_written = nullptr) -> hipError_t {
         return sm_u8 ? launch_sobel_nms_classify_march_u8in((const uint8_t *)smp, edges, S, C, gg, lo, hi, ev,
-                                                            ctx->stream, ctx->tune_sobel_seg, le, pp)
+                                                            ctx->stream, ctx->tune_sobel_seg, le, pp, tile_flags,
+                                                            flags_written)
                      : launch_sobel_nms_classify_march(smp, edges, S, C, gg, lo, hi, ev, ctx->stream,
-                                                       ctx->tune_sobel_seg, le, pp);
+                                                       ctx->tune_sobel_seg, le, pp, tile_flags, flags_written);
     };
     if (fused) {
         HystGeom g = make_hyst_geom(h, w, n);
@@ -844,18 +849,25 @@
             HIP_TRY(ctx, hipStreamWaitEvent(ctx->stream, A.event, 0));
             return CANNY_HIP_OK;
         }
-        if ((rc = prepare_hyst(ctx, g, true))) return rc;
+        const bool tail_route = ctx->hyst_tail && g.tiles_x * g.tiles_y <= kTailMaxTiles;
+        bool listed = false;
+        if (!tail_route && (rc = prepare_hyst(ctx, g, true))) return rc;
         {
             StageTimer tm(ctx, CANNY_HIP_STAGE_SOBEL_NMS, nullptr, true);
-            HIP_TRY(ctx, fused_sobel(sm, d_edges, S, C, g, edge_value, tm.launch_events(), pairs));
-        }
-        if (ctx->hyst_tail && g.tiles_x * g.tiles_y <= kTailMaxTiles) {
+            uint8_t *tf = (tail_route && ctx->hyst_sweep0_lists) ? (uint8_t *)ctx->tile_flags.p : nullptr;
+            HIP_TRY(ctx, fused_sobel(sm, d_edges, S, C, g, edge_value, tm.launch_events(), pairs, tf, &listed));
+        }
+        if (tail_route)
+            HIP_TRY(ctx, launch_hyst_prepare(S, C, g, true, (unsigned *)ctx->stamps.p,
+                                             (unsigned *)ctx->flags.p, ctx->stream, 1,
+                                             listed ? (const uint8_t *)ctx->tile_flags.p : nullptr));
+        if (tail_route) {
             StageTimer tm(ctx, CANNY_HIP_STAGE_HYST_PROPAGATE);
             unsigned *sched = (unsigned *)ctx->stamps.p, *flags = (unsigned *)ctx->flags.p;
             const int wide = ctx->hyst_tail_after;
             for (int k = 0; k < wide; k++)
                 HIP_TRY(ctx, launch_hyst_propagate(S, C, sched, flags, k, g, ctx->stream, d_edges, edge_value,
-                                                   true));
+                                                   true, listed));
             HIP_TRY(ctx, launch_hyst_tail(S, C, sched, flags, wide, g, ctx->stream, d_edges, edge_value));
             ctx->hyst_iters_async = true;
             return CANNY_HIP_OK;
@@ -1618,6 +1630,7 @@
     add("plane_c", c->plane_c, D);
     add("stamps", c->stamps, I);
     add("flags", c->flags, D);
+    add("tile_flags", c->tile_flags, D);
     for (int k = 0; k < 4; k++) add(("io" + std::to_string(k)).c_str(), c->io[k], I);
     for (size_t p = 0; p < c->batch_pool.size(); p++) {
         const canny_hip_ctx::BatchPipe *w = c->batch_pool[p];
@@ -1707,6 +1720,7 @@
     ctx->smoothed.release();
     ctx->plane_s.release();
     ctx->plane_c.release();
+    ctx->tile_flags.release();
     ctx->edges16.release();
     ctx->hist.release();
     ctx->thr.release();
@@ -1767,6 +1781,7 @@
     else if (!std::strcmp(name, "last_canny_fused_gray")) *value = ctx->last_fused_gray;
     else if (!std::strcmp(name, "fuse_classify")) *value = ctx->fuse_classify;
     else if (!std::strcmp(name, "hysteresis_tail")) *value = ctx->hyst_tail;
+    else if (!std::strcmp(name, "hysteresis_sweep0_lists")) *value = ctx->hyst_sweep0_lists;
     else if (!std::strcmp(name, "gaussian_path")) *value = ctx->gaussian_path;
     else if (!std::strcmp(name, "sobel_nms_path")) *value = ctx->sobel_nms_path;
     else if (!std::strcmp(name, "tune_batch_compact")) *value = ctx->batch_compact;
@@ -1789,6 +1804,8 @@
     else if (!std::strcmp(name, "fuse_gray") && value <= 1) ctx->fuse_gray = value;
     else if (!std::strcmp(name, "hysteresis_tail") && value <= 1) ctx->hyst_tail = value;
     else if (!std::strcmp(name, "tune_hyst_tail_after") && value >= 1 && value <= 4) ctx->hyst_tail_after = value;
+    else if (!std::strcmp(name, "hysteresis_sweep0_lists") && value <= 1) ctx->hyst_sweep0_lists = value;
+    else if (!std::strcmp(name, "tune_hyst_sweep0_div") && (value == 8 || value == 16 || value == 32 || value == 64 || value == 128)) hyst_set_sweep0_div(value);
     else if (!std::strcmp(name, "overlap_hysteresis") && value <= 1) ctx->overlap_hysteresis = value;
     else if (!std::strcmp(name, "tune_batch_workers") && value <= 16) ctx->batch_workers = value;
     else if (!std::strcmp(name, "tune_batch_chunk_mb") && value <= 1024) ctx->batch_chunk_mb = value;
@@ -4094,6 +4111,55 @@
     return d2h_sync(ctx, bins, d_bins, total);
 }
 
+int canny_hip_selftest_sweep0_lists(canny_hip_ctx *ctx, const unsigned char *d_img, float sigma, int min_val, int max_val,
+                                    int height, int width, int n_frames, unsigned int *counts, unsigned int *tiles)
+{
+    int rc = bind(ctx);
+    if (rc) return rc;
+    if (!d_img || !counts || !tiles) return CANNY_HIP_ERR_INVALID;
+    if ((rc = check_dims(height, width, n_frames))) return rc;
+    const int h = height, w = width, n = n_frames;
+    if (h < 2 || w < 2) return CANNY_HIP_ERR_UNSUPPORTED;
+    if (hysteresis_order_dependent(min_val, max_val)) return CANNY_HIP_ERR_DOMAIN;
+    const HystGeom g = make_hyst_geom(h, w, n);
+    if (!(ctx->fuse_classify && ctx->sobel_nms_path != 1 && sobel_nms_classify_supported(h, w, min_val)) ||
+        !(ctx->hyst_tail && g.tiles_x * g.tiles_y <= kTailMaxTiles) || !ctx->hyst_sweep0_lists)
+        return CANNY_HIP_ERR_UNSUPPORTED;
+    if ((rc = finish_pending(ctx))) return rc;
+    HIP_TRY(ctx, ctx->smoothed.ensure(npx(h, w, n) * sizeof(short)));
+    HIP_TRY(ctx, ctx->edges16.ensure(npx(h, w, n) * sizeof(short)));
+    short *sm = (short *)ctx->smoothed.p, *edges = (short *)ctx->edges16.p;
+    int sm_u8 = 0;
+    if (ctx->smoothed_u8) {
+        GaussTaps taps;
+        if ((rc = make_taps(sigma, taps))) return rc;
+        if (gaussian_u8_possible(ctx, taps, h, w)) sm_u8 = ctx->smoothed_u8;
+    }
+    if ((rc = dev_gaussian(ctx, d_img, sigma, h, w, n, sm, sm_u8)) || (rc = ensure_hyst(ctx, g))) return rc;
+    uint64_t *S = (uint64_t *)ctx->plane_s.p, *C = (uint64_t *)ctx->plane_c.p;
+    uint8_t *tf = (uint8_t *)ctx->tile_flags.p;
+    const int edge_value = 255 >= max_val ? 255 : 0;
+    bool listed = false;
+    HIP_TRY(ctx, sm_u8 ? launch_sobel_nms_classify_march_u8in((const uint8_t *)sm, edges, S, C, g, min_val, max_val,
+                                                              edge_value, ctx->stream, ctx->tune_sobel_seg, {}, nullptr,
+                                                              tf, &listed)
+                       : launch_sobel_nms_classify_march(sm, edges, S, C, g, min_val, max_val, edge_value, ctx->stream,
+                                                         ctx->tune_sobel_seg, {}, nullptr, tf, &listed));
+    if (!listed) {
+        HIP_TRY(ctx, hipStreamSynchronize(ctx->stream));
+        return CANNY_HIP_ERR_UNSUPPORTED;
+    }
+    unsigned *sched = (unsigned *)ctx->stamps.p;
+    HIP_TRY(ctx, launch_hyst_prepare(S, C, g, true, sched, (unsigned *)ctx->flags.p, ctx->stream, 1, tf));
+    const size_t tiles_all = (size_t)g.tiles();
+    std::vector<unsigned> fcount(4 * (size_t)n);
+    HIP_TRY(ctx, hipMemcpyAsync(fcount.data(), sched + 5 * tiles_all + 4, fcount.size() * sizeof(unsigned),
+                                hipMemcpyDeviceToHost, ctx->stream));
+    if ((rc = d2h_sync(ctx, tiles, sched + 3 * tiles_all + 4, tiles_all * sizeof(unsigned)))) return rc;
+    for (int f = 0; f < n; f++) counts[f] = fcount[4 * (size_t)f];
+    return CANNY_HIP_OK;
+}
+
 static int selftest_div_common(canny_hip_ctx *ctx, float divisor, int use_fma, float c,
                                unsigned long long *mismatches, float *largest_mismatching_dividend)
 {
diff --git a/canny_edge_amd/csrc/canny_kernels.h b/canny_edge_amd/csrc/canny_kernels.h
--- a/canny_edge_amd/csrc/canny_kernels.h
+++ b/canny_edge_amd/csrc/canny_kernels.h
@@ -132,7 +132,8 @@
 hipError_t launch_sobel_nms_classify_march(const int16_t *smoothed, int16_t *edges, uint64_t *strong, uint64_t *conn,
                                            const HystGeom &g, int min_val, int max_val, int edge_value,
                                            hipStream_t stream, int tune_seg = 0, const LaunchEvents &ev = {},
-                                           const int *pairs = nullptr);
+                                           const int *pairs = nullptr, uint8_t *tile_flags = nullptr,
+                                           bool *flags_written = nullptr);
 
 bool sobel_nms_u8_input_supported();
 hipError_t launch_sobel_nms_march_u8in(const uint8_t *smoothed, int16_t *out, int height, int width, int n_frames,
@@ -140,7 +141,8 @@
 hipError_t launch_sobel_nms_classify_march_u8in(const uint8_t *smoothed, int16_t *edges, uint64_t *strong,
                                                 uint64_t *conn, const HystGeom &g, int min_val, int max_val,
                                                 int edge_value, hipStream_t stream, int tune_seg = 0,
-                                                const LaunchEvents &ev = {}, const int *pairs = nullptr);
+                                                const LaunchEvents &ev = {}, const int *pairs = nullptr,
+                                                uint8_t *tile_flags = nullptr, bool *flags_written = nullptr);
 
 __host__ __device__ inline void clamp_thresholds(int &lo, int &hi)
 {
@@ -192,10 +194,12 @@
                                 int max_val, unsigned *domain_flag, hipStream_t stream, const int *pairs = nullptr);
 inline size_t hyst_sched_words(const HystGeom &g) { return 5 * (size_t)g.tiles() + 4 + 4 * (size_t)g.n_frames; }
 hipError_t launch_hyst_prepare(uint64_t *strong, uint64_t *conn, const HystGeom &g, bool zero_pad, unsigned *sched,
-                               unsigned *flags, hipStream_t stream, int n_lanes = 1);
+                               unsigned *flags, hipStream_t stream, int n_lanes = 1,
+                               const uint8_t *tile_flags = nullptr);
 hipError_t launch_hyst_propagate(uint64_t *strong, const uint64_t *conn, unsigned *sched, unsigned *last_change,
                                  int iter, const HystGeom &g, hipStream_t stream, int16_t *edges = nullptr,
-                                 int edge_value = 0, bool frame_queues = false);
+                                 int edge_value = 0, bool frame_queues = false, bool listed0 = false);
+void hyst_set_sweep0_div(int d);
 hipError_t launch_hyst_tail(uint64_t *strong, const uint64_t *conn, unsigned *sched, unsigned *last_change,
                             int first_iter, const HystGeom &g, hipStream_t stream, int16_t *edges = nullptr,
                             int edge_value = 0);
diff --git a/canny_edge_amd/csrc/canny_kernels.hip b/canny_edge_amd/csrc/canny_kernels.hip
--- a/canny_edge_amd/csrc/canny_kernels.hip
+++ b/canny_edge_amd/csrc/canny_kernels.hip
@@ -772,12 +772,12 @@
     process_tile(t, lane, strong, sch, last_change, iter, g, edges, edge_value, c, in, to_frame);
 }
 
-__global__ __launch_bounds__(256) void hyst_propagate_kernel(uint64_t *__restrict__ strong,
+__global__ __launch_bounds__(256) __attribute__((amdgpu_num_sgpr(80))) void hyst_propagate_kernel(uint64_t *__restrict__ strong,
                                                              const uint64_t *__restrict__ conn,
                                                              unsigned *__restrict__ sched_words,
                                                              unsigned *__restrict__ last_change, int iter, HystGeom g,
                                                              int16_t *__restrict__ edges, int edge_value,
-                                                             int frame_groups)
+                                                             int frame_groups, int listed0)
 {
     const int lane = threadIdx.x & 63;
     const int wave = __builtin_amdgcn_readfirstlane(blockIdx.x * 4 + (threadIdx.x >> 6));
@@ -785,7 +785,7 @@
     const int tiles = g.tiles();
     const HystSched sch = make_sched(sched_words, tiles);
     if (wave == 0 && lane == 0) sch.count[(iter + 2) % 3] = 0;
-    if (iter == 0) {
+    if (iter == 0 && !listed0) {
         for (int t0 = wave * kSweep0Tiles; t0 < tiles; t0 += n_waves * kSweep0Tiles) {
             uint64_t c[kSweep0Tiles];
 #pragma unroll
@@ -807,6 +807,24 @@
                                (unsigned)tpf);
         const unsigned *q = ((iter & 1) ? sch.fq1 : sch.fq0) + (size_t)f * tpf;
         const unsigned w = (unsigned)__builtin_amdgcn_readfirstlane(part * 4 + (int)(threadIdx.x >> 6));
+        if (listed0) {
+            const unsigned stride = (unsigned)frame_groups * 4u;
+            const unsigned mine = n > w ? (n - w + stride - 1u) / stride : 0u;
+            for (unsigned k0 = 0; k0 < mine; k0 += 64u) {
+                const unsigned m = min(64u, mine - k0);
+                const unsigned e = (unsigned)lane < m ? q[w + (k0 + (unsigned)lane) * stride] : 0u;
+                int t = __builtin_amdgcn_readlane((int)e, 0);
+                uint64_t c = conn[(size_t)t * kTile + lane];
+                for (unsigned k = 0; k < m; k++) {
+                    const int tn = __builtin_amdgcn_readlane((int)e, (int)min(k + 1u, m - 1u));
+                    const uint64_t cn = conn[(size_t)tn * kTile + lane];
+                    propagate_tile(t, lane, strong, conn, sch, last_change, iter, g, edges, edge_value, c, true);
+                    t = tn;
+                    c = cn;
+                }
+            }
+            return;
+        }
         for (unsigned i = w; i < n; i += (unsigned)frame_groups * 4u) {
             const int t = (int)q[i];
             propagate_tile(t, lane, strong, conn, sch, last_change, iter, g, edges, edge_value,
@@ -1090,9 +1108,48 @@
 __global__ __launch_bounds__(256) void hyst_prepare_kernel(uint64_t *__restrict__ strong, uint64_t *__restrict__ conn,
                                                            HystGeom g, int pad_waves, unsigned *__restrict__ sched,
                                                            unsigned n_sched, unsigned *__restrict__ flags,
-                                                           int n_flags)
+                                                           int n_flags, const uint8_t *__restrict__ tile_flags,
+                                                           int zero_blocks)
 {
     const int lane = (int)(threadIdx.x & 63);
+    const unsigned tiles = (unsigned)g.tiles();
+    if (tile_flags && (int)blockIdx.x >= zero_blocks) {
+        __shared__ unsigned s_wave[4];
+        const int f = (int)blockIdx.x - zero_blocks;
+        const unsigned tpf = (unsigned)(g.tiles_x * g.tiles_y), t_base = (unsigned)f * tpf;
+        const HystSched sch = make_sched(sched, (int)tiles);
+        const uint16_t *const pair = reinterpret_cast<const uint16_t *>(tile_flags) + t_base;
+        unsigned *const q = sch.fq0 + t_base;
+        constexpr int kTrips = kTailTiles / 256;
+        uint16_t mine[kTrips];
+#pragma unroll
+        for (int j = 0; j < kTrips; j++) {
+            const unsigned t = (unsigned)j * 256u + threadIdx.x;
+            mine[j] = t < tpf ? pair[t] : (uint16_t)0;
+        }
+        unsigned base = 0;
+#pragma unroll
+        for (int j = 0; j < kTrips; j++) {
+            const unsigned t0 = (unsigned)j * 256u;
+            if (t0 >= tpf) break;
+            const unsigned t = t0 + threadIdx.x;
+            const bool listed = mine[j] != 0;
+            const uint64_t votes = __ballot(listed);
+            if (lane == 0) s_wave[threadIdx.x >> 6] = (unsigned)__popcll(votes);
+            __syncthreads();
+            unsigned before = 0, all = 0;
+            for (unsigned w = 0; w < 4u; w++) {
+                const unsigned c = s_wave[w];
+                if (w < (threadIdx.x >> 6)) before += c;
+                all += c;
+            }
+            if (listed) q[base + before + (unsigned)__popcll(votes & ((1ull << lane) - 1ull))] = t_base + t;
+            base += all;
+            __syncthreads();
+        }
+        if (threadIdx.x == 0) sch.fcount[4 * (size_t)f] = base;
+        return;
+    }
     const int wave = (int)blockIdx.x * 4 + (int)(threadIdx.x >> 6);
     if (wave < pad_waves) {
         const int per_frame = g.tiles_x + g.tiles_y;
@@ -1112,22 +1169,29 @@
         return;
     }
     const size_t i0 = ((size_t)(wave - pad_waves) * 64 + lane) * 4;
-    for (int j = 0; j < 4; j++)
-        if (i0 + j < n_sched) sched[i0 + j] = 0u;
+    const size_t fq0_beg = 3 * (size_t)tiles + 4, fq0_end = 4 * (size_t)tiles + 4, fcount_beg = 5 * (size_t)tiles + 4;
+    for (int j = 0; j < 4; j++) {
+        const size_t i = i0 + j;
+        const bool listed = tile_flags && ((i >= fq0_beg && i < fq0_end) || (i >= fcount_beg && ((i - fcount_beg) & 3) == 0));
+        if (i < n_sched && !listed) sched[i] = 0u;
+    }
     if (wave == pad_waves && lane < n_flags) flags[lane] = 0u;
 }
 
 hipError_t launch_hyst_prepare(uint64_t *strong, uint64_t *conn, const HystGeom &g, bool zero_pad, unsigned *sched,
-                               unsigned *flags, hipStream_t stream, int n_lanes)
+                               unsigned *flags, hipStream_t stream, int n_lanes, const uint8_t *tile_flags)
 {
     if (n_lanes < 1 || n_lanes > 16) return hipErrorInvalidValue;
+    if (tile_flags && (n_lanes != 1 || g.n_frames < 1 || g.tiles_x * g.tiles_y > kTailTiles)) return hipErrorInvalidValue;
     const bool pad = zero_pad && (g.height % kTile != 0 || g.width % kTile != 0);
     const long long pad_waves = pad ? (long long)(g.tiles_x + g.tiles_y) * g.n_frames : 0;
     const size_t n_sched = 5 * (size_t)g.tiles() + 4 * (size_t)n_lanes + 4 * (size_t)g.n_frames;
     const long long waves = pad_waves + (long long)((n_sched + 255) / 256);
     if (pad_waves > 0x3fffffffLL || n_sched > 0xffffffffull) return hipErrorInvalidValue;
-    hipLaunchKernelGGL(hyst_prepare_kernel, dim3((unsigned)((waves + 3) / 4)), dim3(256), 0, stream, strong, conn, g,
-                       (int)pad_waves, sched, (unsigned)n_sched, flags, 2 * n_lanes);
+    const unsigned zero_blocks = (unsigned)((waves + 3) / 4);
+    hipLaunchKernelGGL(hyst_prepare_kernel, dim3(zero_blocks + (tile_flags ? (unsigned)g.n_frames : 0u)), dim3(256), 0,
+                       stream, strong, conn, g, (int)pad_waves, sched, (unsigned)n_sched, flags, 2 * n_lanes, tile_flags,
+                       (int)zero_blocks);
     return hipGetLastError();
 }
 
@@ -1222,11 +1286,15 @@
     return hipGetLastError();
 }
 
+static int sweep0_div = 64;
+void hyst_set_sweep0_div(int d) { sweep0_div = d; }
+
 hipError_t launch_hyst_propagate(uint64_t *strong, const uint64_t *conn, unsigned *stamp, unsigned *last_change,
                                  int iter, const HystGeom &g, hipStream_t stream, int16_t *edges, int edge_value,
-                                 bool frame_queues)
+                                 bool frame_queues, bool listed0)
 {
     if (frame_queues && (g.n_frames < 1 || g.tiles_x * g.tiles_y > kTailTiles)) return hipErrorInvalidValue;
+    if (listed0 && !frame_queues) return hipErrorInvalidValue;
     unsigned blocks = (unsigned)((g.tiles() + 4 * kSweep0Tiles - 1) / (4 * kSweep0Tiles));
     int frame_groups = frame_queues ? 1 : 0;
     if (iter > 0) {
@@ -1237,9 +1305,12 @@
             if (frame_groups < 1) frame_groups = 1;
             blocks = (unsigned)frame_groups * (unsigned)g.n_frames;
         }
+    } else if (listed0) {
+        frame_groups = (g.tiles_x * g.tiles_y + sweep0_div - 1) / sweep0_div;
+        blocks = (unsigned)frame_groups * (unsigned)g.n_frames;
     }
     hipLaunchKernelGGL(hyst_propagate_kernel, dim3(blocks), dim3(256), 0, stream, strong, conn, stamp, last_change,
-                       iter, g, edges, edge_value, frame_groups);
+                       iter, g, edges, edge_value, frame_groups, (iter == 0 && listed0) ? 1 : 0);
     return hipGetLastError();
 }
 __global__ __launch_bounds__(256) void hyst_finalize_rows_kernel(int16_t *__restrict__ cand,
diff --git a/canny_edge_amd/csrc/canny_sobel_nms_march.hip b/canny_edge_amd/csrc/canny_sobel_nms_march.hip
--- a/canny_edge_amd/csrc/canny_sobel_nms_march.hip
+++ b/canny_edge_amd/csrc/canny_sobel_nms_march.hip
@@ -87,6 +87,7 @@
     int H, W, ybeg, yend, x0, lane;
     uint8_t *pconn, *pstrong;
     int tiles_x, lo1, hi1;
+    uint8_t *pflags;
     int edge_value;
 };
 
@@ -121,6 +122,37 @@
     const int na = v_ge0 ? n0 : n45;
     const int nb = v_ge0 ? n135 : n90;
     return u_ge0 ? na : nb;
+}
+
+__device__ __forceinline__ void stage_flag_tiles(const StripJob &jb, const uint8_t *stage, unsigned plane_bytes,
+                                                 unsigned lrow, bool row_ok, int st_o, int st_e, int st_w0, int wf0,
+                                                 int wf1, int head_end, int tail_beg, unsigned weak_words)
+{
+    if (!jb.pflags) return;
+    auto weak = [&](int k, int lo, int hi) -> unsigned {
+        const uint64_t c = *reinterpret_cast<const uint64_t *>(stage + lrow + 8 * k);
+        const uint64_t s = *reinterpret_cast<const uint64_t *>(stage + plane_bytes + lrow + 8 * k);
+        const uint64_t mask = (hi >= 8 ? ~0ull : (1ull << (8 * hi)) - 1ull) & ~((1ull << (8 * lo)) - 1ull);
+        return __ballot(row_ok && (c & ~s & mask) != 0) != 0 ? 1u : 0u;
+    };
+    unsigned vals = 0;
+    int first = 2 * wf0, end = 2 * wf0;
+    if (st_o < head_end) {
+        first = 1;
+        end = 2;
+        vals = weak(0, st_o, head_end);
+    }
+    for (int k = wf0; k < wf1; k++) {
+        vals |= ((weak_words >> k) & 1u) << (2 * k - first);
+        end = 2 * k + 2;
+    }
+    if (tail_beg < st_e) {
+        vals |= weak(wf1, 0, st_e - 8 * wf1) << (2 * wf1 - first);
+        const bool image_ends = (st_w0 * 8 + st_e) * 8 >= jb.W;
+        end = 2 * wf1 + (image_ends ? 2 : 1);
+    }
+    uint8_t *const frow = jb.pflags + 2u * ((unsigned)(jb.ybeg >> 6) * (unsigned)jb.tiles_x + (unsigned)st_w0);
+    if (jb.lane < end - first) frow[first + jb.lane] = (uint8_t)((vals >> jb.lane) & 1u);
 }
 
 template <bool COL_EDGE, bool ROW_EDGE, bool PLANES, int NP, bool LDS_PLANES, bool IN_U8 = false>
@@ -212,13 +244,16 @@
         const unsigned grow = (unsigned)(y >> 6) * (unsigned)jb.tiles_x * 512u + (unsigned)(y & 63) * 8u;
         __builtin_amdgcn_fence(__ATOMIC_ACQ_REL, "wavefront");
         const int wf0 = (st_o + 7) >> 3, wf1 = st_e >> 3;
+        unsigned weak_words = 0;
         for (int k = wf0; k < wf1; k++) {
+            const uint64_t cw = *reinterpret_cast<const uint64_t *>(stage + lrow + 8 * k);
+            const uint64_t sw = *reinterpret_cast<const uint64_t *>(stage + kStagePlane + lrow + 8 * k);
             if (row_ok) {
                 const unsigned g = grow + (unsigned)(st_w0 + k) * 512u;
-                *reinterpret_cast<uint64_t *>(jb.pconn + g) = *reinterpret_cast<const uint64_t *>(stage + lrow + 8 * k);
-                *reinterpret_cast<uint64_t *>(jb.pstrong + g) =
-                    *reinterpret_cast<const uint64_t *>(stage + kStagePlane + lrow + 8 * k);
-            }
+                *reinterpret_cast<uint64_t *>(jb.pconn + g) = cw;
+                *reinterpret_cast<uint64_t *>(jb.pstrong + g) = sw;
+            }
+            if (jb.pflags) weak_words |= (__ballot(row_ok && (cw & ~sw) != 0) != 0 ? 1u : 0u) << k;
         }
         auto leftover = [&](int i) {
             if (!row_ok) return;
@@ -236,6 +271,7 @@
         const int head_end = min(8 * wf0, st_e), tail_beg = max(8 * wf1, head_end);
         for (int i = st_o; i < head_end; i += kStep) leftover(i);
         for (int i = tail_beg; i < st_e; i += kStep) leftover(i);
+        stage_flag_tiles(jb, stage, kStagePlane, lrow, row_ok, st_o, st_e, st_w0, wf0, wf1, head_end, tail_beg, weak_words);
         __builtin_amdgcn_fence(__ATOMIC_ACQ_REL, "wavefront");
     };
 
@@ -572,13 +608,16 @@
         const unsigned grow = (unsigned)(y >> 6) * (unsigned)jb.tiles_x * 512u + (unsigned)(y & 63) * 8u;
         __builtin_amdgcn_fence(__ATOMIC_ACQ_REL, "wavefront");
         const int wf0 = (st_o + 7) >> 3, wf1 = st_e >> 3;
+        unsigned weak_words = 0;
         for (int k = wf0; k < wf1; k++) {
+            const uint64_t cw = *reinterpret_cast<const uint64_t *>(stage + lrow + 8 * k);
+            const uint64_t sw = *reinterpret_cast<const uint64_t *>(stage + kStagePlane + lrow + 8 * k);
             if (row_ok) {
                 const unsigned g = grow + (unsigned)(st_w0 + k) * 512u;
-                *reinterpret_cast<uint64_t *>(jb.pconn + g) = *reinterpret_cast<const uint64_t *>(stage + lrow + 8 * k);
-                *reinterpret_cast<uint64_t *>(jb.pstrong + g) =
-                    *reinterpret_cast<const uint64_t *>(stage + kStagePlane + lrow + 8 * k);
-            }
+                *reinterpret_cast<uint64_t *>(jb.pconn + g) = cw;
+                *reinterpret_cast<uint64_t *>(jb.pstrong + g) = sw;
+            }
+            if (jb.pflags) weak_words |= (__ballot(row_ok && (cw & ~sw) != 0) != 0 ? 1u : 0u) << k;
         }
         auto leftover = [&](int i) {
             if (!row_ok) return;
@@ -596,6 +635,7 @@
         const int head_end = min(8 * wf0, st_e), tail_beg = max(8 * wf1, head_end);
         for (int i = st_o; i < head_end; i += kStep) leftover(i);
         for (int i = tail_beg; i < st_e; i += kStep) leftover(i);
+        stage_flag_tiles(jb, stage, kStagePlane, lrow, row_ok, st_o, st_e, st_w0, wf0, wf1, head_end, tail_beg, weak_words);
         __builtin_amdgcn_fence(__ATOMIC_ACQ_REL, "wavefront");
     };
 
@@ -836,6 +876,7 @@
     uint8_t *conn, *strong;
     int tiles_x, tiles_y, lo1, hi1, edge_value;
     const int *thr;
+    uint8_t *flags;
 };
 
 template <bool PLANES, int NP, bool LDS_PLANES, bool IN_U8 = false, bool FLT = false, bool THR = false>
@@ -885,6 +926,7 @@
         jb.pconn = pl.conn + (size_t)f * frame_bytes;
         jb.pstrong = pl.strong + (size_t)f * frame_bytes;
         jb.tiles_x = pl.tiles_x;
+        jb.pflags = (LDS_PLANES && pl.flags) ? pl.flags + (size_t)f * 2 * (size_t)(pl.tiles_y * pl.tiles_x) : nullptr;
         if constexpr (THR) {
             int lo = pl.thr[2 * f], hi = pl.thr[2 * f + 1];
             clamp_thresholds(lo, hi);
@@ -945,25 +987,36 @@
         hipLaunchKernelGGL(kernel, grid, block, 0, stream, args...);
 }
 
-template <bool THR = false>
-static hipError_t launch_march(const void *smoothed, int16_t *out, const PlaneArgs *planes, int height, int width,
-                               int n_frames, hipStream_t stream, int tune_seg, const LaunchEvents &ev,
-                               bool in_u8 = false)
-{
-    const int np = px_variant == 1 ? 2 : 4;
-    if (in_u8 && !(np == 4 && (!planes || plane_store_variant == 0))) return hipErrorNotSupported;
+static int march_segment_rows(bool planes, int np, int height, int width, int n_frames, int tune_seg)
+{
     const int sw = 62 * 2 * np;
-    int n_strips = (width + sw - 1) / sw;
+    const int n_strips = (width + sw - 1) / sw;
     int seg = 64;
     while (seg > 32 && (long long)n_frames * n_strips * ((height + seg - 1) / seg) < 16384) seg >>= 1;
     while (seg > 8 && (long long)n_frames * n_strips * ((height + seg - 1) / seg) < 2048) seg >>= 1;
     if (tune_seg >= 8) seg = tune_seg;
     if (planes && np == 4 && plane_store_variant == 0 && seg > SNM_STAGE_ROWS) seg = SNM_STAGE_ROWS;
+    return seg;
+}
+
+template <bool THR = false>
+static hipError_t launch_march(const void *smoothed, int16_t *out, const PlaneArgs *planes, int height, int width,
+                               int n_frames, hipStream_t stream, int tune_seg, const LaunchEvents &ev,
+                               bool in_u8 = false, bool *flags_written = nullptr)
+{
+    if (flags_written) *flags_written = false;
+    const int np = px_variant == 1 ? 2 : 4;
+    if (in_u8 && !(np == 4 && (!planes || plane_store_variant == 0))) return hipErrorNotSupported;
+    const int sw = 62 * 2 * np;
+    int n_strips = (width + sw - 1) / sw;
+    const int seg = march_segment_rows(planes != nullptr, np, height, width, n_frames, tune_seg);
     int n_segs = (height + seg - 1) / seg;
     long long waves = (long long)n_frames * n_strips * n_segs;
     if (waves > 0x7fffffffLL) return hipErrorInvalidValue;
     unsigned blocks = (unsigned)((waves + SNM_WPB - 1) / SNM_WPB);
-    const PlaneArgs pl = planes ? *planes : PlaneArgs{};
+    PlaneArgs pl = planes ? *planes : PlaneArgs{};
+    if (!(np == 4 && plane_store_variant == 0 && seg == SNM_STAGE_ROWS)) pl.flags = nullptr;
+    if (flags_written) *flags_written = pl.flags != nullptr;
     const dim3 grid(blocks), block(SNM_WPB * 64);
     const bool use_f32 = arith_variant == 2 || (arith_variant == 0 && planes != nullptr);
     if (use_f32 && np == 4) {
@@ -1024,29 +1077,34 @@
 
 static hipError_t classify_march_any(const void *smoothed, bool in_u8, int16_t *edges, uint64_t *strong, uint64_t *conn,
                                      const HystGeom &g, int min_val, int max_val, int edge_value, hipStream_t stream,
-                                     int tune_seg, const LaunchEvents &ev, const int *pairs);
+                                     int tune_seg, const LaunchEvents &ev, const int *pairs, uint8_t *tile_flags,
+                                     bool *flags_written);
 
 hipError_t launch_sobel_nms_classify_march(const int16_t *smoothed, int16_t *edges, uint64_t *strong, uint64_t *conn,
                                            const HystGeom &g, int min_val, int max_val, int edge_value,
-                                           hipStream_t stream, int tune_seg, const LaunchEvents &ev, const int *pairs)
+                                           hipStream_t stream, int tune_seg, const LaunchEvents &ev, const int *pairs,
+                                           uint8_t *tile_flags, bool *flags_written)
 {
     return classify_march_any(smoothed, false, edges, strong, conn, g, min_val, max_val, edge_value, stream, tune_seg, ev,
-                              pairs);
+                              pairs, tile_flags, flags_written);
 }
 
 hipError_t launch_sobel_nms_classify_march_u8in(const uint8_t *smoothed, int16_t *edges, uint64_t *strong,
                                                 uint64_t *conn, const HystGeom &g, int min_val, int max_val,
                                                 int edge_value, hipStream_t stream, int tune_seg,
-                                                const LaunchEvents &ev, const int *pairs)
+                                                const LaunchEvents &ev, const int *pairs, uint8_t *tile_flags,
+                                                bool *flags_written)
 {
     return classify_march_any(smoothed, true, edges, strong, conn, g, min_val, max_val, edge_value, stream, tune_seg, ev,
-                              pairs);
+                              pairs, tile_flags, flags_written);
 }
 
 static hipError_t classify_march_any(const void *smoothed, bool in_u8, int16_t *edges, uint64_t *strong, uint64_t *conn,
                                      const HystGeom &g, int min_val, int max_val, int edge_value, hipStream_t stream,
-                                     int tune_seg, const LaunchEvents &ev, const int *pairs)
-{
+                                     int tune_seg, const LaunchEvents &ev, const int *pairs, uint8_t *tile_flags,
+                                     bool *flags_written)
+{
+    if (flags_written) *flags_written = false;
     if (pairs) min_val = max_val = 255;
     if (!sobel_nms_classify_supported(g.height, g.width, min_val)) return hipErrorNotSupported;
     if (edge_value < 0 || edge_value > 32767) return hipErrorInvalidValue;
@@ -1061,11 +1119,13 @@
     pl.hi1 = (hi > lo ? hi : lo) - 1;
     pl.edge_value = edge_value;
     pl.thr = pairs;
+    pl.flags = tile_flags;
     if (pairs) {
         if (edge_value != 255) return hipErrorInvalidValue;
-        return launch_march<true>(smoothed, edges, &pl, g.height, g.width, g.n_frames, stream, tune_seg, ev, in_u8);
-    }
-    return launch_march(smoothed, edges, &pl, g.height, g.width, g.n_frames, stream, tune_seg, ev, in_u8);
-}
-
-}
+        return launch_march<true>(smoothed, edges, &pl, g.height, g.width, g.n_frames, stream, tune_seg, ev, in_u8,
+                                  flags_written);
+    }
+    return launch_march(smoothed, edges, &pl, g.height, g.width, g.n_frames, stream, tune_seg, ev, in_u8, flags_written);
+}
+
+}
diff --git a/include/canny_hip.h b/include/canny_hip.h
--- a/include/canny_hip.h
+++ b/include/canny_hip.h
@@ -7,7 +7,7 @@
 extern "C" {
 #endif
 
-#define CANNY_HIP_VERSION 1201
+#define CANNY_HIP_VERSION 1202
 #define CANNY_HIP_MAX_WINDOW 129
 
 typedef struct canny_hip_ctx canny_hip_ctx;
@@ -389,6 +389,8 @@
                                  int n_frames, unsigned int *d_hist);
 int canny_hip_selftest_select(canny_hip_ctx *ctx, const unsigned int *d_hist, int n_frames, int rule, float low, float high,
                               int *d_pairs);
+int canny_hip_selftest_sweep0_lists(canny_hip_ctx *ctx, const unsigned char *d_img, float sigma, int min_val, int max_val,
+                                    int height, int width, int n_frames, unsigned int *counts, unsigned int *tiles);
 enum canny_hip_workspace_kind { CANNY_HIP_WS_DATA = 0, CANNY_HIP_WS_INDEX = 1, CANNY_HIP_WS_CACHE = 2 };
 int canny_hip_selftest_workspace(canny_hip_ctx *ctx, int index, const char **name, void **d_ptr, size_t *bytes, int *kind);
 
```

Measured after the change: 590,700 Mpixels/s (median of 6 runs). +1.4%, better.
